# autonomousvision/unimatch

Measured on AMD Instinct MI355X. Metric: image_pairs_per_sec, higher is better.
Workload: dtype f16x2

## Files before the change

include/unimatch_hip.h:

```cpp
#ifndef UNIMATCH_HIP_H
#define UNIMATCH_HIP_H

#include <stddef.h>
#include <stdint.h>

#ifdef __cplusplus
extern "C" {
#endif

#define UM_VERSION 220

#define UM_MODE_EXACT 0
#define UM_MODE_FAST 1

#define UM_ERR_BAD_ARG (-1)
#define UM_ERR_BAD_GEOMETRY (-2)
#define UM_ERR_WORKSPACE (-3)
#define UM_ERR_UNSUPPORTED (-4)
#define UM_ERR_COLLECTIVE (-5)

int um_version(void);
const char* um_last_error_string(void);

#define UM_RANGE_PLANES 1u
#define UM_RANGE_ATTN_TOKENS 2u
#define UM_RANGE_ATTN_QUERY 4u
#define UM_RANGE_ATTN_OUTPUT 8u
#define UM_RANGE_FFN_TOKENS 16u
#define UM_RANGE_FFN_HIDDEN 32u
#define UM_RANGE_KV_TOKENS 64u
#define UM_RANGE_LINEAR 128u
int um_range_flags(unsigned* flags_out, int reset);

#define UM_K_WINDOW_ATTN 0
#define UM_K_GLOBAL_SOFTMAX 1
#define UM_K_SPLIT_PLANES 2
#define UM_K_LOCAL_CORR 3
#define UM_K_COST_VOLUME 4
#define UM_K_PROP_LOCAL 5
#define UM_K_DEPTH_CORR 6
#define UM_K_LINEAR 7
#define UM_K_INSTANCE_NORM 8
#define UM_K_CONVEX_UPSAMPLE 9
#define UM_K_FFN 10
#define UM_K_CONV 11
#define UM_K_COUNT 12
#define UM_V_WATTN_TILE 0
#define UM_V_WATTN_KSPLIT 1
#define UM_V_FFN_TILE 2
#define UM_V_FFN_HSPLIT 3
#define UM_V_GSV4 4
#define UM_V_GSV3 5
#define UM_V_K4_MFMA 6
#define UM_V_K4_VALU 7
#define UM_V_K3_MFMA 8
#define UM_V_K3_VALU 9
#define UM_V_CONV_PATCH 10
#define UM_V_CONV_ROWS 11
#define UM_V_CONV_GENERIC 12
#define UM_V_WATTN_W8 13
#define UM_V_CONV_PATCH_NORM 14
#define UM_V_COUNT 15
int um_census_enable(int on);
long um_census_count(int variant);
int um_window_attn_tile_census(int enable, unsigned long long* counts4);
double um_probe_mfma_flops(int iters);
int um_probe_mfma(float* sink, int iters, void* stream);
int um_probe_copy(const void* src, void* dst, size_t bytes, void* stream);
int um_probe_chase(const unsigned* ring, unsigned* out, int hops, void* stream);
int um_timing_enable(int kernel_mask);
int um_timing_collect(int kernel_id, double* total_ms, int* launches);

size_t um_window_attn_workspace_bytes(int streams, int tokens, int channels, int mode);
int um_window_attn_fwd(const float* q, const float* k, const float* v, float* out,
                       int streams, int h, int w, int channels,
                       int win_h, int win_w, int shift_h, int shift_w,
                       int mode, void* workspace, size_t workspace_bytes, void* stream);

int um_window_attn_planes_fwd(const void* q_planes, const void* k_planes, const void* v_planes, float* out,
                              int streams, int h, int w, int channels, int ldq, int ldkv,
                              long q_plane_stride, long kv_plane_stride,
                              int win_h, int win_w, int shift_h, int shift_w, int kv_rotate, int mode, void* stream);

int um_window_attn_merge_fwd(const void* q_planes, const void* k_planes, const void* v_planes, const void* wm_planes,
                             const float* gamma, const float* beta, const float* residual, float eps, int wshift, float* out,
                             int streams, int h, int w, int channels, int ldq, int ldkv, long q_plane_stride,
                             long kv_plane_stride, int win_h, int win_w, int shift_h, int shift_w, int kv_rotate, int mode,
                             void* stream);

size_t um_window_attn_ksplit_workspace_bytes(int streams, int h, int w, int win_h, int win_w);
int um_window_attn_plan(int streams, int h, int w, int win_h, int win_w, int* full_tiles, int* split_tiles, int* parts);
int um_window_attn_qproj_merge_fwd(const float* x, const void* wq_planes, const void* k_planes, const void* v_planes,
                                   const void* wm_planes, const float* gamma, const float* beta, const float* residual, float eps,
                                   int wshift, float* out, int streams, int h, int w, int channels, int ldkv,
                                   long kv_plane_stride, int win_h, int win_w, int shift_h, int shift_w, int kv_rotate, int mode,
                                   void* workspace, size_t workspace_bytes, void* stream);

#define UM_EPI_PLANES 0
#define UM_EPI_LN 1
#define UM_EPI_GELU_PLANES 2
size_t um_planes_bytes(long rows, int cols, int mode);
int um_weight_planes(const float* w, void* planes, int n, int k, int wshift, int mode, void* stream);
int um_linear_fwd(const float* a0, const float* a1, const void* a_planes, const void* w_planes,
                  int m, int n, int k, int wshift, int epilogue, void* out,
                  const float* gamma, const float* beta, const float* residual, float eps,
                  int mode, void* stream);

int um_linear_bias_fwd(const float* a0, const void* a_planes, const void* w_planes, const float* bias, int m, int n, int k,
                       int wshift, float out_mul, float bias_mul, void* out_planes, float* out_f32, int mode, void* stream);

int um_ffn_fwd(const float* x, const float* y, const void* w1_planes, const void* w2_planes, int m, int hidden,
               int wshift, const float* gamma, const float* beta, float eps, float* out, int mode, void* stream);
size_t um_ffn_split_workspace_bytes(int m, int hidden);
int um_ffn_ws_fwd(const float* x, const float* y, const void* w1_planes, const void* w2_planes, int m, int hidden,
                  int wshift, const float* gamma, const float* beta, float eps, float* out, int mode, void* workspace,
                  size_t workspace_bytes, void* stream);

int um_kv4_fwd(const float* x, const void* wc_planes, int m, int wshift, void* out_planes, int mode, void* stream);
int um_ffn_kv_fwd(const float* x, const float* y, const void* w1_planes, const void* w2_planes, int m, int hidden, int wshift,
                  const float* gamma, const float* beta, float eps, float* out, const void* wc_planes, void* kv_planes, int mode,
                  void* workspace, size_t workspace_bytes, void* stream);

int um_conv2d_fwd(const void* a_planes, const void* w_planes, const float* bias, float* out, float* stats_out, int batch,
                  int hi, int wi, int cin, int cout, int kh, int kw, int stride, int pad_h, int pad_w, int relu, int wshift,
                  int mode, void* stream);
int um_conv2d_ex(const void* a_planes, int a_ld, int a_coff, long a_rows, const void* w_planes, const float* bias, float* out,
                 int out_ld, int out_coff, void* out_planes, int outp_ld, int outp_coff, long outp_rows, float* stats_out,
                 int batch, int hi, int wi, int cin, int cout, int kh, int kw, int stride, int pad_h, int pad_w, int act,
                 int wshift, int mode, void* stream);
int um_conv2d_gru_fwd(int gate, const void* a_planes, int a_ld, int a_coff, long a_rows, const void* w_planes, const float* bias,
                      float* hidden, const float* z, int z_ld, float* z_out, int z_out_ld, void* out_planes, int outp_ld,
                      int outp_coff, long outp_rows, int batch, int hi, int wi, int cin, int channels, int kh, int kw, int pad_h,
                      int pad_w, int wshift, int mode, void* stream);
int um_conv2d_gru_add_fwd(int gate, const void* a_planes, int a_ld, int a_coff, long a_rows, const void* w_planes, const float* bias,
                          const float* addend, int addend_ld, float* hidden, const float* z, int z_ld, float* z_out, int z_out_ld,
                          void* out_planes, int outp_ld, int outp_coff, long outp_rows, int batch, int hi, int wi, int cin,
                          int channels, int kh, int kw, int pad_h, int pad_w, int wshift, int mode, void* stream);
int um_conv_stats_parts(int hi, int wi, int cout, int kh, int kw, int stride, int pad_h, int pad_w);
size_t um_conv_stats_bytes(int batch, int parts, int channels);

size_t um_stem_planes_bytes(int batch, int h, int w);
size_t um_conv7_planes_bytes(int batch, int h, int w, int stride);
int um_conv7_fwd(const float* image, int channels, int normalize, const float* mean3, const float* std3, void* image_planes,
                 const void* w_planes, const float* bias, float* out, int out_ld, int out_coff, void* out_planes, int outp_ld,
                 int outp_coff, long outp_rows, float* stats_out, int batch, int h, int w, int cout, int stride, int act,
                 int wshift, void* stream);
int um_stem_conv_fwd(const float* image, int normalize, const float* mean3, const float* std3, void* image_planes,
                     const void* w_planes, float* out, float* stats_out, int batch, int h, int w, int cout, int wshift,
                     void* stream);

size_t um_nhwc_norm_workspace_bytes(int batch, int pixels, int channels);
int um_nhwc_instance_norm(const float* x, const float* shortcut, const void* shortcut_planes, void* planes_out, float* f32_out,
                          int batch, int pixels, int channels, float eps, int normalize, int relu, const float* conv_stats,
                          int conv_stats_parts, void* workspace, size_t workspace_bytes, int mode, void* stream);

int um_nhwc_stats_finalize(const float* conv_stats, int conv_stats_parts, float* stats_out, int batch, int pixels, int channels,
                           float eps, void* stream);
int um_conv2d_norm_supported(int hi, int wi, int cin, int cout, int kh, int kw, int stride, int pad_h, int pad_w, int mode);
int um_conv2d_norm_fwd(const float* x, const float* norm_stats, int norm_relu, const void* w_planes, const float* bias, float* out,
                       float* stats_out, int batch, int hi, int wi, int cin, int cout, int kh, int kw, int stride, int pad_h,
                       int pad_w, int relu, int wshift, int mode, void* stream);

int um_nhwc_gate(int mode, const float* src, int src_ld, const float* zr, float* hbuf, void* planes_out, int ld, int coff,
                 long plane_rows, long rows, int channels, void* stream);

int um_nchw_to_nhwc(const float* x, void* planes_out, float* f32_out, int batch, int channels, int pixels, int mode,
                    void* stream);

size_t um_global_corr_workspace_bytes(int batch, int tokens, int channels, int mode);
int um_global_corr_softmax_flow(const float* f0, const float* f1, float* flow,
                                int batch, int h, int w, int channels, int bidir,
                                int mode, void* workspace, size_t workspace_bytes, void* stream);

int um_global_corr_softmax_stereo(const float* f0, const float* f1, float* disp,
                                  int batch, int h, int w, int channels,
                                  int mode, void* workspace, size_t workspace_bytes, void* stream);

int um_prop_global_attn(const float* q, const float* k, const float* value, float* out,
                        int batch, int h, int w, int channels, int value_channels,
                        int mode, void* workspace, size_t workspace_bytes, void* stream);
float um_global_corr_plane_scale(int channels);
int um_prop_global_attn_planes(const void* q_planes, const void* k_planes, const float* value, float* out, int batch, int h,
                               int w, int channels, int value_channels, int mode, void* workspace, size_t workspace_bytes,
                               void* stream);


int um_local_corr_softmax(const float* f0, const float* f1, float* out,
                          int batch, int h, int w, int channels, int radius, int one_d, void* stream);

int um_local_corr_with_flow(const float* f0, const float* f1, const float* flow, float* cost,
                            int batch, int h, int w, int channels, int radius, void* stream);
int um_local_corr_with_flow_dilated(const float* f0, const float* f1, const float* flow, float* cost,
                                    int batch, int h, int w, int channels, int radius, int dilation, void* stream);
int um_local_corr_with_flow_planes(const float* f0, const float* f1, const float* flow, void* planes_out, int ld, long plane_rows,
                                   int batch, int h, int w, int channels, int radius, void* stream);

size_t um_local_corr_feat_planes_bytes(int batch, int h, int w, int channels);
int um_local_corr_feat_planes(const float* f0, const float* f1, void* feat_planes, int batch, int h, int w, int channels,
                              void* stream);
int um_local_corr_with_flow_feat_supported(int h, int w, int channels, int radius);
int um_local_corr_softmax_mfma(const float* f0, const float* f1, float* out, int batch, int h, int w, int channels, int radius,
                               void* workspace, size_t workspace_bytes, void* stream);
int um_local_corr_with_flow_feat(const float* f0, const float* f1, const void* feat_planes, const float* flow, float* cost,
                                 void* planes_out, int ld, long plane_rows, int batch, int h, int w, int channels, int radius,
                                 int flags, unsigned* stats ,
                                 void* stream);

int um_prop_local_attn(const float* q, const float* k, const float* value, float* out,
                       int batch, int h, int w, int channels, int value_channels, int radius,
                       void* stream);

int um_depth_corr_softmax(const float* f0, const float* f1, const float* cam, const float* candidates,
                          float* out, int batch, int h, int w, int channels, int num_candidates,
                          int from_argmax, void* stream);

int um_convex_upsample(const float* flow, const float* mask, float* up, int batch, int channels, int h, int w,
                       int factor, int is_depth, int mask_nhwc, void* stream);

int um_flow_warp(const float* feature_tokens, const float* flow, float* out_tokens, int batch, int h, int w, int channels,
                 void* stream);

int um_fwd_bwd_occlusion(const float* fwd, const float* bwd, float* occ_fwd, float* occ_bwd, int batch, int h, int w, float alpha,
                         float beta, void* stream);
size_t um_flow_to_rgb_workspace_bytes(int batch, int h, int w);
int um_flow_to_rgb(const float* flow, unsigned char* rgb, int batch, int h, int w, void* workspace, size_t ws_bytes, void* stream);

#define UM_FLOW_METRICS_K 16
#define UM_DISP_METRICS_K 8
#define UM_DEPTH_METRICS_K 8
size_t um_flow_metrics_workspace_bytes(int batch, int h, int w);
int um_flow_metrics(const float* pred, const float* gt, const float* valid, const float* noc_valid, double* rows, int batch, int hp,
                    int wp, int h, int w, int top, int left, void* workspace, size_t ws_bytes, void* stream);
size_t um_disp_metrics_workspace_bytes(int batch, int h, int w);
int um_disp_metrics(const float* pred, const float* gt, double* rows, int batch, int hp, int wp, int h, int w, int top, int left,
                    float max_disp, void* workspace, size_t ws_bytes, void* stream);
size_t um_depth_metrics_workspace_bytes(int batch, int h, int w);
int um_depth_metrics(const float* pred, const float* gt, const float* valid, double* rows, int batch, int hp, int wp, int h, int w,
                     int top, int left, float lo, float hi, void* workspace, size_t ws_bytes, void* stream);

#define UM_PREPOST_MAX_DIM 262140
#define UM_IMG_F32_NCHW 0
#define UM_IMG_U8_NHWC 1
#define UM_SIZE_PAD 0
#define UM_SIZE_RESIZE 1
#define UM_PRED_FLOW 0
#define UM_PRED_DISPARITY 1
#define UM_PRED_DEPTH 2
int um_image_prepare(const void* src, int src_layout, float* dst, int batch, int h, int w, int transpose, const float* mean,
                     const float* std, int mode, int hp, int wp, int top, int left, void* stream);
int um_pred_restore(const float* pred, float* out, int batch, int channels, int hp, int wp, int mode, int top, int left, int h, int w,
                    int kind, int transpose, void* stream);

int um_flow_upsample2x(const float* flow, float* out, int batch, int channels, int h, int w, float mult, void* stream);
int um_depth_cam_pack(const float* intrinsics, const float* pose, float* cam, int batch, float stride_div, int bidir, void* stream);
int um_rigid_flow(const float* inv_depth, const float* cam, float* flow, int batch, int h, int w, void* stream);

int um_instance_norm_fwd(const float* x, const float* shortcut, float* y, long planes, int hw, float eps,
                         int relu, void* stream);

#define UM_COMM_ID_BYTES 128
int um_comm_unique_id(void* id_out );
int um_comm_init_rank(void** comm_out, const void* id , int rank, int world);
int um_comm_init_file(void** comm_out, const char* path, int rank, int world, int timeout_seconds);
int um_comm_init_file_nonce(void** comm_out, const char* path, int rank, int world, int timeout_seconds, int nonce);
int um_comm_world(void* comm);
int um_comm_destroy(void* comm);
int um_allgather_preds(void* comm, const float* send, float* recv, size_t count_per_rank, void* stream);

int um_swin_attn_fwd(const float* q, const float* k, const float* v, float* out, int streams, int h, int w, int channels,
                     int win_h, int win_w, int shift_h, int shift_w, int mode, void* workspace, size_t workspace_bytes,
                     void* stream);
int um_attn1d_fwd(const float* q, const float* k, const float* v, float* out, int streams, int h, int w, int channels,
                  int win_w, int shift_w, int mode, void* workspace, size_t workspace_bytes, void* stream);
int um_local_corr_softmax_1d(const float* f0, const float* f1, float* out, int batch, int h, int w, int channels, int radius,
                             void* stream);
size_t um_workspace_bytes_swin_attn_fwd(int streams, int h, int w, int channels, int mode);
size_t um_workspace_bytes_attn1d_fwd(int streams, int h, int w, int channels, int mode);
size_t um_workspace_bytes_global_corr_softmax_flow(int batch, int h, int w, int channels, int mode);
size_t um_workspace_bytes_global_corr_softmax_stereo(int batch, int h, int w, int channels, int mode);
size_t um_workspace_bytes_prop_global_attn(int batch, int h, int w, int channels, int mode);
size_t um_workspace_bytes_local_corr_softmax(int batch, int h, int w, int channels, int mode);
size_t um_workspace_bytes_local_corr_softmax_1d(int batch, int h, int w, int channels, int mode);
size_t um_workspace_bytes_local_corr_with_flow(int batch, int h, int w, int channels, int mode);
size_t um_workspace_bytes_prop_local_attn(int batch, int h, int w, int channels, int mode);
size_t um_workspace_bytes_depth_corr_softmax(int batch, int h, int w, int channels, int mode);
size_t um_workspace_bytes_allgather_preds(int batch, int h, int w, int channels, int mode);

#ifdef UM_DIAGNOSTIC_BUILD
int um_debug_mfma_peak(float* sink, int iters, int random_operands, void* stream);
int um_debug_mfma_ticks(unsigned long long* ticks, float* sink, int iters, int random_operands, int waves, int chain, void* stream);
int um_debug_mfma_lds(unsigned long long* ticks, float* sink, int tiles, int mode, void* stream);
#endif

#ifdef __cplusplus
}
#endif
#endif
```

unimatch_amd/_abi.py:

```python
import ctypes
import os

_HERE = os.path.dirname(os.path.abspath(__file__))
LIB_PATH = os.environ.get('UM_LIB') or os.path.join(_HERE, 'libunimatch_hip.so')

MODE_EXACT = 0
MODE_FAST = 1

CENSUS = {'wattn_tile': 0, 'wattn_ksplit': 1, 'ffn_tile': 2, 'ffn_hsplit': 3, 'gsv4': 4, 'gsv3': 5, 'k4_mfma': 6, 'k4_valu': 7,
          'k3_mfma': 8, 'k3_valu': 9, 'conv_patch': 10, 'conv_rows': 11, 'conv_generic': 12, 'wattn_w8': 13, 'conv_patch_norm': 14}

_c_int, _c_size_t, _c_void_p = ctypes.c_int, ctypes.c_size_t, ctypes.c_void_p

SIGNATURES = {
    'um_version': (_c_int, []),
    'um_last_error_string': (ctypes.c_char_p, []),
    'um_range_flags': (_c_int, [ctypes.POINTER(ctypes.c_uint), _c_int]),
    'um_timing_enable': (_c_int, [_c_int]),
    'um_timing_collect': (_c_int, [_c_int, ctypes.POINTER(ctypes.c_double), ctypes.POINTER(_c_int)]),
    'um_window_attn_workspace_bytes': (_c_size_t, [_c_int] * 4),
    'um_window_attn_fwd': (_c_int, [_c_void_p] * 4 + [_c_int] * 9 + [_c_void_p, _c_size_t, _c_void_p]),
    'um_window_attn_planes_fwd': (_c_int, [_c_void_p] * 4 + [_c_int] * 6 + [ctypes.c_long] * 2 + [_c_int] * 6 + [_c_void_p]),
    'um_window_attn_merge_fwd': (_c_int, [_c_void_p] * 7 + [ctypes.c_float, _c_int, _c_void_p] + [_c_int] * 6 + [ctypes.c_long] * 2 +
                                 [_c_int] * 6 + [_c_void_p]),
    'um_window_attn_qproj_merge_fwd': (_c_int, [_c_void_p] * 8 + [ctypes.c_float, _c_int, _c_void_p] + [_c_int] * 5 + [ctypes.c_long] +
                                       [_c_int] * 6 + [_c_void_p, _c_size_t, _c_void_p]),
    'um_window_attn_ksplit_workspace_bytes': (_c_size_t, [_c_int] * 5),
    'um_window_attn_plan': (_c_int, [_c_int] * 5 + [ctypes.POINTER(_c_int)] * 3),
    'um_planes_bytes': (_c_size_t, [ctypes.c_long, _c_int, _c_int]),
    'um_weight_planes': (_c_int, [_c_void_p] * 2 + [_c_int] * 4 + [_c_void_p]),
    'um_linear_fwd': (_c_int, [_c_void_p] * 4 + [_c_int] * 5 + [_c_void_p] * 4 + [ctypes.c_float, _c_int, _c_void_p]),
    'um_linear_bias_fwd': (_c_int, [_c_void_p] * 4 + [_c_int] * 4 + [ctypes.c_float] * 2 + [_c_void_p] * 2 + [_c_int, _c_void_p]),
    'um_ffn_fwd': (_c_int, [_c_void_p] * 4 + [_c_int] * 3 + [_c_void_p] * 2 + [ctypes.c_float, _c_void_p, _c_int, _c_void_p]),
    'um_ffn_ws_fwd': (_c_int, [_c_void_p] * 4 + [_c_int] * 3 + [_c_void_p] * 2 + [ctypes.c_float, _c_void_p, _c_int, _c_void_p, _c_size_t,
                                _c_void_p]),
    'um_ffn_split_workspace_bytes': (_c_size_t, [_c_int] * 2),
    'um_ffn_kv_fwd': (_c_int, [_c_void_p] * 4 + [_c_int] * 3 + [_c_void_p] * 2 + [ctypes.c_float, _c_void_p, _c_void_p, _c_void_p, _c_int, _c_void_p,
                                _c_size_t, _c_void_p]),
    'um_kv4_fwd': (_c_int, [_c_void_p, _c_void_p, _c_int, _c_int, _c_void_p, _c_int, _c_void_p]),
    'um_conv2d_fwd': (_c_int, [_c_void_p] * 5 + [_c_int] * 13 + [_c_void_p]),
    'um_conv2d_ex': (_c_int, [_c_void_p, _c_int, _c_int, ctypes.c_long, _c_void_p, _c_void_p, _c_void_p, _c_int, _c_int, _c_void_p,
                              _c_int, _c_int, ctypes.c_long, _c_void_p] + [_c_int] * 13 + [_c_void_p]),
    'um_nhwc_gate': (_c_int, [_c_int, _c_void_p, _c_int, _c_void_p, _c_void_p, _c_void_p, _c_int, _c_int, ctypes.c_long, ctypes.c_long,
                              _c_int, _c_void_p]),
    'um_local_corr_with_flow_planes': (_c_int, [_c_void_p] * 4 + [_c_int, ctypes.c_long] + [_c_int] * 5 + [_c_void_p]),
    'um_conv2d_gru_fwd': (_c_int, [_c_int, _c_void_p, _c_int, _c_int, ctypes.c_long, _c_void_p, _c_void_p, _c_void_p, _c_void_p, _c_int,
                                   _c_void_p, _c_int, _c_void_p, _c_int, _c_int, ctypes.c_long] + [_c_int] * 11 + [_c_void_p]),
    'um_conv2d_gru_add_fwd': (_c_int, [_c_int, _c_void_p, _c_int, _c_int, ctypes.c_long, _c_void_p, _c_void_p, _c_void_p, _c_int, _c_void_p, _c_void_p,
                                        _c_int, _c_void_p, _c_int, _c_void_p, _c_int, _c_int, ctypes.c_long] + [_c_int] * 11 + [_c_void_p]),
    'um_conv2d_norm_supported': (_c_int, [_c_int] * 10),
    'um_conv2d_norm_fwd': (_c_int, [_c_void_p, _c_void_p, _c_int] + [_c_void_p] * 4 + [_c_int] * 13 + [_c_void_p]),
    'um_nhwc_stats_finalize': (_c_int, [_c_void_p, _c_int, _c_void_p] + [_c_int] * 3 + [ctypes.c_float, _c_void_p]),
    'um_conv_stats_bytes': (_c_size_t, [_c_int] * 3),
    'um_conv_stats_parts': (_c_int, [_c_int] * 8),
    'um_stem_planes_bytes': (_c_size_t, [_c_int] * 3),
    'um_conv7_planes_bytes': (_c_size_t, [_c_int] * 4),
    'um_conv7_fwd': (_c_int, [_c_void_p, _c_int, _c_int] + [_c_void_p] * 6 + [_c_int, _c_int, _c_void_p, _c_int, _c_int, ctypes.c_long,
                              _c_void_p] + [_c_int] * 7 + [_c_void_p]),
    'um_stem_conv_fwd': (_c_int, [_c_void_p, _c_int] + [_c_void_p] * 6 + [_c_int] * 5 + [_c_void_p]),
    'um_nhwc_norm_workspace_bytes': (_c_size_t, [_c_int] * 3),
    'um_nhwc_instance_norm': (_c_int, [_c_void_p] * 5 + [_c_int] * 3 + [ctypes.c_float, _c_int, _c_int, _c_void_p, _c_int, _c_void_p,
                                       _c_size_t, _c_int, _c_void_p]),
    'um_nchw_to_nhwc': (_c_int, [_c_void_p] * 3 + [_c_int] * 4 + [_c_void_p]),
    'um_flow_warp': (_c_int, [_c_void_p] * 3 + [_c_int] * 4 + [_c_void_p]),
    'um_fwd_bwd_occlusion': (_c_int, [_c_void_p] * 4 + [_c_int] * 3 + [ctypes.c_float] * 2 + [_c_void_p]),
    'um_flow_to_rgb_workspace_bytes': (_c_size_t, [_c_int] * 3),
    'um_flow_to_rgb': (_c_int, [_c_void_p] * 2 + [_c_int] * 3 + [_c_void_p, _c_size_t, _c_void_p]),
    'um_flow_metrics_workspace_bytes': (_c_size_t, [_c_int] * 3),
    'um_flow_metrics': (_c_int, [_c_void_p] * 5 + [_c_int] * 7 + [_c_void_p, _c_size_t, _c_void_p]),
    'um_disp_metrics_workspace_bytes': (_c_size_t, [_c_int] * 3),
    'um_disp_metrics': (_c_int, [_c_void_p] * 3 + [_c_int] * 7 + [ctypes.c_float, _c_void_p, _c_size_t, _c_void_p]),
    'um_depth_metrics_workspace_bytes': (_c_size_t, [_c_int] * 3),
    'um_depth_metrics': (_c_int, [_c_void_p] * 4 + [_c_int] * 7 + [ctypes.c_float] * 2 + [_c_void_p, _c_size_t, _c_void_p]),
    'um_image_prepare': (_c_int, [_c_void_p, _c_int, _c_void_p] + [_c_int] * 4 + [ctypes.POINTER(ctypes.c_float)] * 2 + [_c_int] * 5 +
                         [_c_void_p]),
    'um_pred_restore': (_c_int, [_c_void_p] * 2 + [_c_int] * 11 + [_c_void_p]),
    'um_convex_upsample': (_c_int, [_c_void_p] * 3 + [_c_int] * 7 + [_c_void_p]),
    'um_flow_upsample2x': (_c_int, [_c_void_p] * 2 + [_c_int] * 4 + [ctypes.c_float, _c_void_p]),
    'um_depth_cam_pack': (_c_int, [_c_void_p] * 3 + [_c_int, ctypes.c_float, _c_int, _c_void_p]),
    'um_rigid_flow': (_c_int, [_c_void_p] * 3 + [_c_int] * 3 + [_c_void_p]),
    'um_instance_norm_fwd': (_c_int, [_c_void_p] * 3 + [ctypes.c_long, _c_int, ctypes.c_float, _c_int, _c_void_p]),
    'um_global_corr_workspace_bytes': (_c_size_t, [_c_int] * 4),
    'um_global_corr_softmax_flow': (_c_int, [_c_void_p] * 3 + [_c_int] * 6 + [_c_void_p, _c_size_t, _c_void_p]),
    'um_global_corr_softmax_stereo': (_c_int, [_c_void_p] * 3 + [_c_int] * 5 + [_c_void_p, _c_size_t, _c_void_p]),
    'um_prop_global_attn': (_c_int, [_c_void_p] * 4 + [_c_int] * 6 + [_c_void_p, _c_size_t, _c_void_p]),
    'um_global_corr_plane_scale': (ctypes.c_float, [_c_int]),
    'um_prop_global_attn_planes': (_c_int, [_c_void_p] * 4 + [_c_int] * 6 + [_c_void_p, _c_size_t, _c_void_p]),
    'um_local_corr_softmax': (_c_int, [_c_void_p] * 3 + [_c_int] * 6 + [_c_void_p]),
    'um_local_corr_with_flow': (_c_int, [_c_void_p] * 4 + [_c_int] * 5 + [_c_void_p]),
    'um_local_corr_with_flow_dilated': (_c_int, [_c_void_p] * 4 + [_c_int] * 6 + [_c_void_p]),
    'um_local_corr_feat_planes_bytes': (ctypes.c_size_t, [_c_int] * 4),
    'um_local_corr_feat_planes': (_c_int, [_c_void_p] * 3 + [_c_int] * 4 + [_c_void_p]),
    'um_local_corr_with_flow_feat_supported': (_c_int, [_c_int] * 4),
    'um_local_corr_softmax_mfma': (_c_int, [_c_void_p] * 3 + [_c_int] * 5 + [_c_void_p, ctypes.c_size_t, _c_void_p]),
    'um_local_corr_with_flow_feat': (_c_int, [_c_void_p] * 6 + [_c_int, ctypes.c_long] + [_c_int] * 6 + [_c_void_p, _c_void_p]),
    'um_prop_local_attn': (_c_int, [_c_void_p] * 4 + [_c_int] * 6 + [_c_void_p]),
    'um_depth_corr_softmax': (_c_int, [_c_void_p] * 5 + [_c_int] * 6 + [_c_void_p]),
    'um_census_enable': (_c_int, [_c_int]),
    'um_census_count': (ctypes.c_long, [_c_int]),
    'um_window_attn_tile_census': (_c_int, [_c_int, ctypes.POINTER(ctypes.c_ulonglong)]),
    'um_probe_mfma_flops': (ctypes.c_double, [_c_int]),
    'um_probe_mfma': (_c_int, [_c_void_p, _c_int, _c_void_p]),
    'um_probe_copy': (_c_int, [_c_void_p, _c_void_p, _c_size_t, _c_void_p]),
    'um_probe_chase': (_c_int, [_c_void_p, _c_void_p, _c_int, _c_void_p]),
    'um_swin_attn_fwd': (_c_int, [_c_void_p] * 4 + [_c_int] * 9 + [_c_void_p, _c_size_t, _c_void_p]),
    'um_attn1d_fwd': (_c_int, [_c_void_p] * 4 + [_c_int] * 7 + [_c_void_p, _c_size_t, _c_void_p]),
    'um_local_corr_softmax_1d': (_c_int, [_c_void_p] * 3 + [_c_int] * 5 + [_c_void_p]),
    **{f'um_workspace_bytes_{op}': (_c_size_t, [_c_int] * 5) for op in (
        'swin_attn_fwd', 'attn1d_fwd', 'global_corr_softmax_flow', 'global_corr_softmax_stereo', 'prop_global_attn',
        'local_corr_softmax', 'local_corr_softmax_1d', 'local_corr_with_flow', 'prop_local_attn', 'depth_corr_softmax',
        'allgather_preds')},
    'um_comm_unique_id': (_c_int, [_c_void_p]),
    'um_comm_init_rank': (_c_int, [ctypes.POINTER(_c_void_p), _c_void_p, _c_int, _c_int]),
    'um_comm_init_file': (_c_int, [ctypes.POINTER(_c_void_p), ctypes.c_char_p, _c_int, _c_int, _c_int]),
    'um_comm_init_file_nonce': (_c_int, [ctypes.POINTER(_c_void_p), ctypes.c_char_p, _c_int, _c_int, _c_int, _c_int]),
    'um_comm_world': (_c_int, [_c_void_p]),
    'um_comm_destroy': (_c_int, [_c_void_p]),
    'um_allgather_preds': (_c_int, [_c_void_p, _c_void_p, _c_void_p, _c_size_t, _c_void_p]),
}
COMM_ID_BYTES = 128
DIAG_SIGNATURES = {
    'um_debug_mfma_peak': (_c_int, [_c_void_p, _c_int, _c_int, _c_void_p]),
    'um_debug_mfma_lds': (_c_int, [_c_void_p, _c_void_p, _c_int, _c_int, _c_void_p]),
    'um_debug_mfma_ticks': (_c_int, [_c_void_p, _c_void_p, _c_int, _c_int, _c_int, _c_int, _c_void_p]),
}

RANGE_ROLES = {1: 'a tensor converted to operand planes (q / k / v / features)', 2: 'attention source tokens', 4: 'projected queries',
               8: 'attention output (input of the merge Linear)', 16: 'FFN input [x | y]', 32: 'FFN hidden activations',
               64: 'tokens / projected keys and values of the k | v projection', 128: 'inputs / plane outputs of a Linear'}

_lib = None


class HipExtensionError(RuntimeError):
    pass


def load():
    global _lib
    if _lib is not None:
        return _lib
    if not os.path.exists(LIB_PATH):
        raise HipExtensionError(
            f'{LIB_PATH} is missing: build it with `python -m unimatch_amd.build` '
            '(hipcc --offload-arch=gfx950).  There is no CPU / PyTorch fallback for the hot path.')
    try:
        lib = ctypes.CDLL(LIB_PATH)
    except OSError as exc:
        raise HipExtensionError(f'cannot load {LIB_PATH}: {exc}') from exc
    for name, (res, args) in SIGNATURES.items():
        try:
            fn = getattr(lib, name)
        except AttributeError as exc:
            raise HipExtensionError(f'{LIB_PATH} does not export {name}') from exc
        fn.restype = res
        fn.argtypes = args
    for name, (res, args) in DIAG_SIGNATURES.items():
        fn = getattr(lib, name, None)
        if fn is not None:
            fn.restype = res
            fn.argtypes = args
    _lib = lib
    return lib


def load_diagnostic():
    lib = load()
    if not hasattr(lib, 'um_debug_mfma_peak'):
        raise HipExtensionError('the shipped library carries no um_debug_* symbol: build a diagnostic variant '
                                '(`python -m unimatch_amd.build --variant diag`) and set UM_LIB=unimatch_amd/_variants/libdiag.so')
    return lib


def census(lib=None):
    lib = lib or load()
    return {k: int(lib.um_census_count(v)) for k, v in CENSUS.items()}


def attn_tile_census(enable):
    out = (ctypes.c_ulonglong * 4)()
    check(load().um_window_attn_tile_census(1 if enable else 0, out), 'um_window_attn_tile_census')
    return dict(zip(('full', 'probed', 'probed_then_computed', 'workgroups'), (int(v) for v in out)))


def check(code, what):
    if code == 0:
        return
    msg = load().um_last_error_string().decode('utf-8', 'replace')
    if code < 0:
        raise ValueError(f'{what}: {msg} (code {code})')
    raise RuntimeError(f'{what}: HIP error {code}')


class OperandRangeError(FloatingPointError):
    """An activation reached fp16's largest finite value (65504) on its way into an exact-mode MFMA operand."""


def range_flags(reset=False):
    out = ctypes.c_uint(0)
    check(load().um_range_flags(ctypes.byref(out), 1 if reset else 0), 'um_range_flags')
    return out.value


def check_operand_range(where=''):
# ... 8 lines not shown
```

unimatch_amd/build.py:

```python
import os
import shutil
import subprocess
import sys

HERE = os.path.dirname(os.path.abspath(__file__))
CSRC = os.path.join(HERE, 'csrc')
LIB = os.path.join(HERE, 'libunimatch_hip.so')
SOURCES = ['capi.hip', 'global_match.hip', 'window_attn.hip', 'local_ops.hip', 'linear.hip', 'ffn.hip', 'conv.hip', 'nhwc_ops.hip', 'norm_ops.hip', 'upsample.hip',
           'rccl_gather.hip', 'local_corr_mfma.hip', 'aliases.hip', 'probe.hip', 'video.hip', 'metrics.hip', 'prepost.hip']
DIAG_SOURCES = ['microbench.hip']
HEADERS = ['common.h', 'planes.h', 'timing.h', os.path.join('..', '..', 'include', 'unimatch_hip.h')]
EXTRA_FLAGS = {'ffn.hip': ['-fno-slp-vectorize'], 'global_match.hip': ['-fno-slp-vectorize', '-mllvm', '-amdgpu-mfma-vgpr-form', '-Wno-inline-asm'], 'window_attn.hip': ['-fno-slp-vectorize'],
               'linear.hip': ['-fno-slp-vectorize'],
               'video.hip': ['-ffp-contract=off'],
               'metrics.hip': ['-ffp-contract=off', '-fhip-fp32-correctly-rounded-divide-sqrt'],
               'prepost.hip': ['-ffp-contract=off', '-fhip-fp32-correctly-rounded-divide-sqrt']}
FLAGS = ['--offload-arch=gfx950', '-O3', '-std=c++17', '-fPIC', '-fno-gpu-rdc', '-Wno-unused-result']


def find_hipcc():
    for cand in (os.environ.get('HIPCC'), shutil.which('hipcc'), '/opt/rocm/bin/hipcc'):
        if cand and os.path.exists(cand):
            return cand
    raise RuntimeError('hipcc not found: the HIP extension cannot be built')


def _stale(target, deps):
    if not os.path.exists(target):
        return True
    t = os.path.getmtime(target)
    return any(os.path.getmtime(d) > t for d in deps)


def build(force=False, verbose=False):
    hipcc = find_hipcc()
    objdir = os.path.join(HERE, '_obj')
    os.makedirs(objdir, exist_ok=True)
    hdrs = [os.path.normpath(os.path.join(CSRC, h)) for h in HEADERS] + [os.path.abspath(__file__)]
    objs = []
    for src in SOURCES:
        s = os.path.join(CSRC, src)
        o = os.path.join(objdir, src.replace('.hip', '.o'))
        if force or _stale(o, [s] + hdrs):
            cmd = [hipcc] + FLAGS + EXTRA_FLAGS.get(src, []) + ['-c', s, '-o', o]
            if verbose:
                print(' '.join(cmd))
            subprocess.run(cmd, check=True, cwd=CSRC)
        objs.append(o)
    if force or _stale(LIB, objs):
        cmd = [hipcc, '--offload-arch=gfx950', '-shared', '-fPIC', '-o', LIB] + objs + ['-ldl']
        if verbose:
            print(' '.join(cmd))
        subprocess.run(cmd, check=True)
    return LIB


def build_variant(name, defines, verbose=False, only=None):
    hipcc = find_hipcc()
    objdir = os.path.join(HERE, '_variants', '_obj_' + name)
    os.makedirs(objdir, exist_ok=True)
    objs = []
    defines = list(defines) + ['-DUM_DIAGNOSTIC_BUILD']
    if only:
        build(verbose=verbose)
    for src in SOURCES + DIAG_SOURCES:
        if only and src not in only and src not in DIAG_SOURCES:
            objs.append(os.path.join(HERE, '_obj', src.replace('.hip', '.o')))
            continue
        o = os.path.join(objdir, src.replace('.hip', '.o'))
        cmd = [hipcc] + FLAGS + EXTRA_FLAGS.get(src, []) + list(defines) + ['-c', os.path.join(CSRC, src), '-o', o]
        if verbose:
            print(' '.join(cmd))
        subprocess.run(cmd, check=True, cwd=CSRC)
        objs.append(o)
    lib = os.path.join(HERE, '_variants', f'lib{name}.so')
    subprocess.run([hipcc, '--offload-arch=gfx950', '-shared', '-fPIC', '-o', lib] + objs + ['-ldl'], check=True)
    shutil.rmtree(objdir, ignore_errors=True)
    return lib


if __name__ == '__main__':
    if '--variant' in sys.argv:
        i = sys.argv.index('--variant')
        only = sys.argv[sys.argv.index('--only') + 1].split(',') if '--only' in sys.argv else None
        print(build_variant(sys.argv[i + 1], [a for a in sys.argv[i + 2:] if a.startswith('-D')], verbose=True, only=only))
    else:
        print(build(force='--force' in sys.argv, verbose=True))
```

unimatch_amd/csrc/conv.hip:

```cpp
#include <cstdlib>
#include <cstring>
#ifndef UM_CONV_2P
#define UM_CONV_2P 0
#endif
#include "common.h"
#include "planes.h"

struct ConvArgs {
    const unsigned short* ap;
    long a_plane_stride;
    unsigned row_stride;
    unsigned zero_row;
    const unsigned short* wp;
    long w_plane_stride;
    const float* bias;
    float* out;
    unsigned short* outp;
    long outp_plane_stride;
    int out_ld, out_coff, outp_ld, outp_coff;
    int act;
    int gate, gate_c, gate_zld;
    float* gate_h;
    const float* gate_z;
    float* gate_hout;
// ... 89 lines not shown
    };
    auto to_lds_b = [&](auto act_tag) {
        if (a.bias) to_lds(act_tag, IntC<1>{});
        else to_lds(act_tag, IntC<0>{});
    };
    switch (a.addend ? 0 : a.act) {
        case 0: to_lds_b(IntC<0>{}); break;
        case 1: to_lds_b(IntC<1>{}); break;
        case 2: to_lds_b(IntC<2>{}); break;
        default: to_lds_b(IntC<3>{}); break;
    }
    __builtin_amdgcn_wave_barrier();
    if (a.stats) {
        constexpr int RG = 64 / CPR >= 8 ? 8 : 64 / CPR >= 4 ? 4 : 2;
        constexpr int RPG = 32 / RG;
        const int nv = nvalid;
        const int c = lane % CPR, rg = lane / CPR;
        const f32x4 k = *reinterpret_cast<const f32x4*>(stg + (c << 4));
        f32x4 s1 = {0.f, 0.f, 0.f, 0.f}, s2 = {0.f, 0.f, 0.f, 0.f};
        if (rg < RG) {
            if (nv == 32) {
#pragma unroll
                for (int j = 0; j < RPG; ++j) {
                    const int r = rg * RPG + j;
                    const f32x4 d = *reinterpret_cast<const f32x4*>(stg + r * ROWB + ((c ^ (r & 7)) << 4)) - k;
                    s1 = s1 + d;
                    s2 = s2 + d * d;
                }
            } else {
#pragma unroll
                for (int j = 0; j < RPG; ++j) {
                    const int r = rg * RPG + j;
                    f32x4 d = *reinterpret_cast<const f32x4*>(stg + r * ROWB + ((c ^ (r & 7)) << 4)) - k;
                    if (r >= nv) d = f32x4{0.f, 0.f, 0.f, 0.f};
                    s1 = s1 + d;
                    s2 = s2 + d * d;
                }
            }
        }
#pragma unroll
        for (int step = CPR * RG / 2; step >= CPR; step >>= 1)
#pragma unroll
            for (int i = 0; i < 4; ++i) {
                s1[i] += __shfl_down(s1[i], step, 64);
                s2[i] += __shfl_down(s2[i], step, 64);
            }
        float* ws = reinterpret_cast<float*>(scratch) + wave * (2 * 32 * NT) + 32 * NT0;
        float* cnt = reinterpret_cast<float*>(scratch) + 8 * (2 * 32 * NT);
        if (lane == 0) cnt[wave] = (float)nv;
        if (lane < CPR) {
            const float inv = nv > 0 ? 1.0f / (float)nv : 0.f;
            *reinterpret_cast<f32x4*>(ws + 4 * c) = k + s1 * inv;
            *reinterpret_cast<f32x4*>(ws + 32 * NT + 4 * c) = s2 - s1 * s1 * inv;
        }
        __syncthreads();
        const int grp = tid >> 8, gt = tid & 255;
        if (gt < 32 * NTP && nb + gt < a.Cout && (cnt[4 * grp] > 0.f || dense_parts)) {
            const float* w0 = reinterpret_cast<const float*>(scratch) + grp * 4 * (2 * 32 * NT) + 32 * NT0;
            float mean = w0[gt], m2 = w0[32 * NT + gt];
            float n = cnt[4 * grp];
#pragma unroll
            for (int wv = 1; wv < 4; ++wv) {
                const float nw = cnt[4 * grp + wv];
                if (nw > 0.f) {
                    const float mw = w0[wv * (2 * 32 * NT) + gt], m2w = w0[wv * (2 * 32 * NT) + 32 * NT + gt];
                    const float delta = mw - mean, nn = n + nw;
                    mean += delta * (nw / nn);
                    m2 += m2w + delta * delta * (n * nw / nn);
                    n = nn;
                }
            }
            float* pr = a.stats + ((long)(part0 + grp) * 3) * a.Cout + nb + gt;
            pr[0] = n > 0.f ? mean : 0.f;
            pr[a.Cout] = n;
            pr[2 * a.Cout] = n > 0.f ? m2 : 0.f;
        }
    }
    auto store_rows = [&](auto gate_tag, auto add_tag) {
        constexpr int GATE = decltype(gate_tag)::value;
        constexpr bool ADD = decltype(add_tag)::value != 0;
        float* obase = a.out ? a.out + rowbase * a.out_ld + a.out_coff : nullptr;
        unsigned short* pbase = a.outp ? a.outp + rowbase * a.outp_ld + a.outp_coff : nullptr;
#pragma unroll
        for (int b = 0; b < NBATCH; ++b) {
            const int slot = NSIDE == 2 ? (b & 1) : 0;
            if ((ADD || GATE != 0) && NSIDE == 2 && b + 1 < NBATCH) preload(b + 1, (b + 1) & 1);
            if ((ADD || GATE != 0) && NSIDE == 1 && b > 0) preload(b, 0);
#pragma unroll
            for (int j = 0; j < BATCH; ++j) {
                const int idx = (b * BATCH + j) * 64 + lane;
                const int r = idx / CPR, c = idx - r * CPR;
                f32x4 d = *reinterpret_cast<const f32x4*>(stg + r * ROWB + ((c ^ (r & 7)) << 4));
                int col = nb + 4 * c;
                if (r < nrows && col < a.Cout) {
                    if (ADD) {
                        d = d + ad[slot][j];
#pragma unroll
                        for (int i = 0; i < 4; ++i) {
                            if (a.act == 1) d[i] = fmaxf(d[i], 0.f);
                            else if (a.act == 2) d[i] = 1.0f / (1.0f + __expf(-d[i]));
                            else if (a.act == 3) d[i] = tanhf(d[i]);
                        }
                    }
                    bool to_out = obase != nullptr, to_planes = pbase != nullptr;
                    if (GATE == 1) {
                        if (col >= a.gate_c) {
                            col -= a.gate_c;
                            d = d * gh[slot][j];
                            to_out = false;
                        } else {
                            to_planes = false;
                        }
                    } else if (GATE == 2) {
#pragma unroll
                        for (int i = 0; i < 4; ++i) d[i] = (1.0f - gz[slot][j][i]) * gh[slot][j][i] + gz[slot][j][i] * d[i];
                        *reinterpret_cast<f32x4*>(hobase + (unsigned)(r * a.gate_hout_ld + col)) = d;
                    }
                    if (to_out) __builtin_nontemporal_store(d, reinterpret_cast<f32x4*>(obase + (unsigned)(r * a.out_ld + col)));
                    if (to_planes) {
                        unsigned short* dst = pbase + (unsigned)(r * a.outp_ld + col);
                        const unsigned h0 = T::pack2(d[0], d[1]), h1 = T::pack2(d[2], d[3]);
                        *reinterpret_cast<u32x2*>(dst) = u32x2{h0, h1};
                        if (NS == 2) {
                            const f32x2 u0 = T::unpack2(h0), u1 = T::unpack2(h1);
                            const u32x2 lo = u32x2{T::pack2(d[0] - u0[0], d[1] - u0[1]), T::pack2(d[2] - u1[0], d[3] - u1[1])};
                            *reinterpret_cast<u32x2*>(dst + a.outp_plane_stride) = lo;
                        }
                    }
                }
            }
        }
    };
    auto store_rows_g = [&](auto gate_tag) {
        if (a.addend) store_rows(gate_tag, IntC<1>{});
        else store_rows(gate_tag, IntC<0>{});
    };
    if (a.gate == 0) store_rows_g(IntC<0>{});
    else if (a.gate == 1) store_rows_g(IntC<1>{});
    else store_rows_g(IntC<2>{});
}

template <typename T, int NS, int NT, int NTE = NT>
__device__ __forceinline__ void conv_epilogue(const ConvArgs& a, f32x16 (&acc)[NT], unsigned char* lds, unsigned char* scratch,
                                              int bt, int rloc0, int nvalid, int part0, bool dense_parts, int n0, int tid, int wave,
                                              int lane, int half) {
    constexpr int NP = NTE < NT ? NTE : NT;
    constexpr int WSTRIDE = 32 * (32 * NP * 4);
    conv_epilogue_pass<T, NS, NT, 0, NP, WSTRIDE>(a, acc, lds, scratch, bt, rloc0, nvalid, part0, dense_parts, n0, tid, wave, lane, half);
    if constexpr (NTE < NT)
        conv_epilogue_pass<T, NS, NT, NTE, NT - NTE, WSTRIDE>(a, acc, lds, scratch, bt, rloc0, nvalid, part0, dense_parts, n0, tid, wave,
                                                              lane, half);
}

template <typename T, int NS, int NT>
__global__ __launch_bounds__(256, 2) void conv_kernel(ConvArgs a) {
    constexpr int TILE = 128 * 64;
    constexpr int WTILE = 32 * NT * 64;
    constexpr int STAGE = NS * (TILE + WTILE);
    constexpr int EPI = 4 * 32 * (32 * NT * 4);
    constexpr int RING = (2 * STAGE > EPI) ? 2 * STAGE : EPI;
    __shared__ __attribute__((aligned(16))) unsigned char lds[RING + 8 * 2 * 32 * NT * 4 + 64];

    const int tid = threadIdx.x, lane = tid & 63;
    const int wave = __builtin_amdgcn_readfirstlane(tid >> 6);
    const int half = lane >> 5;
    const int P = a.Ho * a.Wo, tpi = (P + 127) / 128;
    const int ny = (a.Cout + 32 * NT - 1) / (32 * NT);
    const int wg = a.xcd ? xcd_remap(blockIdx.x, gridDim.x) : blockIdx.x;
    const int tile = wg / ny;
    const int bt = tile / tpi, pl0 = (tile - bt * tpi) * 128;
    const int n0 = (wg - tile * ny) * (32 * NT);
    const int cpt = a.Cin >> 5;
    const int nstage = a.KH * a.KW * cpt;
    const int ktot = a.KH * a.KW * a.Cin;

    const int dcp = lane & 3;
    int py[2], px[2], pbase[2];
    bool pok[2];
#pragma unroll
    for (int i = 0; i < 2; ++i) {
        const int p = pl0 + 32 * wave + 16 * i + (lane >> 2);
        pok[i] = p < P;
        const int rem = pok[i] ? p : 0;
        const int y = rem / a.Wo, x = rem - y * a.Wo;
        py[i] = y * a.stride - a.pad_h;
        px[i] = x * a.stride - a.pad_w;
        pbase[i] = bt * a.Hi * a.Wi;
    }
    const unsigned zero_row = a.zero_row;
    unsigned rowoff[2];
    auto set_tap = [&](int ky, int kx) {
#pragma unroll
        for (int i = 0; i < 2; ++i) {
            const int iy = py[i] + ky, ix = px[i] + kx;
            const bool ok = pok[i] && (unsigned)iy < (unsigned)a.Hi && (unsigned)ix < (unsigned)a.Wi;
            const unsigned row = ok ? (unsigned)(pbase[i] + iy * a.Wi + ix) : zero_row;
            rowoff[i] = row * a.row_stride;
        }
    };
    int ky = 0, kx = 0, cc = 0;
    auto stage_async = [&](int c0, int kglob, unsigned char* buf) {
#pragma unroll
        for (int i = 0; i < 2; ++i) {
            const int r = 32 * wave + 16 * i + (lane >> 2);
            const int sc = dcp ^ ((r >> 2) & 3);
            const unsigned off = rowoff[i] + (unsigned)((c0 + 8 * sc) * 2);
#pragma unroll
            for (int pl = 0; pl < NS; ++pl) conv_dma16(a.ap + pl * a.a_plane_stride, off, buf + pl * TILE + (32 * wave + 16 * i) * 64);
        }
#pragma unroll
        for (int i = 0; i < (2 * NT + 3) / 4; ++i) {
            const int j = wave + 4 * i;
            if (j < 2 * NT) {
                const int r = 16 * j + (lane >> 2);
                const int sc = dcp ^ ((r >> 2) & 3);
                const int n = min(n0 + r, a.Cout - 1);
                const unsigned off = (unsigned)(((long)n * ktot + kglob + 8 * sc) * 2);
#pragma unroll
                for (int pl = 0; pl < NS; ++pl)
                    conv_dma16(a.wp + pl * a.w_plane_stride, off, buf + NS * TILE + pl * WTILE + (16 * j) * 64);
            }
        }
    };

    f32x16 acc[NT];
#pragma unroll
    for (int nt = 0; nt < NT; ++nt)
#pragma unroll
        for (int r = 0; r < 16; ++r) acc[nt][r] = 0.f;

    const int fr = lane & 31;
    int foff[2];
#pragma unroll
    for (int ks = 0; ks < 2; ++ks) foff[ks] = fr * 64 + (((2 * ks + half) ^ ((fr >> 2) & 3)) << 4);

    set_tap(0, 0);
    stage_async(0, 0, lds);
    auto advance = [&]() {
        if (++cc == cpt) {
            cc = 0;
            if (++kx == a.KW) {
                kx = 0;
                ++ky;
            }
            set_tap(ky, kx);
        }
    };
    advance();
    asm volatile("s_waitcnt vmcnt(0)" ::: "memory");
    __syncthreads();

    for (int s = 0; s < nstage; ++s) {
        unsigned char* cur = lds + (s & 1) * STAGE;
        unsigned char* nxt = lds + ((s & 1) ^ 1) * STAGE;
        if (s + 1 < nstage) {
            stage_async(cc * 32, (s + 1) * 32, nxt);
            advance();
        }
        const unsigned char* at = cur + 32 * wave * 64;
        const unsigned char* wt = cur + NS * TILE;
        __builtin_amdgcn_s_setprio(1);
#pragma unroll
        for (int ks = 0; ks < 2; ++ks) {
            const i16x8 bh = *reinterpret_cast<const i16x8*>(at + foff[ks]);
            i16x8 bl;
            if (NS == 2) bl = *reinterpret_cast<const i16x8*>(at + TILE + foff[ks]);
#pragma unroll
            for (int nt = 0; nt < NT; ++nt) {
                const i16x8 wh = *reinterpret_cast<const i16x8*>(wt + nt * 32 * 64 + foff[ks]);
                if (NS == 2) {
                    const i16x8 wl = *reinterpret_cast<const i16x8*>(wt + WTILE + nt * 32 * 64 + foff[ks]);
                    if (UM_CONV_2P != 1) acc[nt] = T::mfma(wl, bh, acc[nt]);
                    if (UM_CONV_2P != 2) acc[nt] = T::mfma(wh, bl, acc[nt]);
                }
                acc[nt] = T::mfma(wh, bh, acc[nt]);
            }
        }
        __builtin_amdgcn_s_setprio(0);
        asm volatile("s_waitcnt vmcnt(0)" ::: "memory");
        __syncthreads();
    }

    {
        const int rloc0 = pl0 + 32 * wave;
        conv_epilogue<T, NS, NT>(a, acc, lds, lds + RING, bt, rloc0, min(32, max(0, P - rloc0)), bt * ((P + 127) / 128) + pl0 / 128, false,
                                 n0, tid, wave, lane, half);
    }
}

template <int NS, int NT, int KW, int NSLOT>
struct ConvRowsLds {
    static constexpr int NTE = NT < 2 ? NT : 2;
    static constexpr int ATILE = 288 * 32;
    static constexpr int WTILE = 32 * NT * 32;
    static constexpr int STAGE = NS * (ATILE + KW * WTILE);
    static constexpr int EPI = 8 * 32 * (32 * NTE * 4);
    static constexpr int RING = (NSLOT * STAGE > EPI) ? NSLOT * STAGE : EPI;
    static constexpr int TOTAL = RING + 8 * 2 * 32 * NT * 4 + 64;
};

__device__ __forceinline__ void conv_wait_vm(int n) {
    switch (n) {
        case 0: asm volatile("s_waitcnt vmcnt(0)" ::: "memory"); break;
        case 1: asm volatile("s_waitcnt vmcnt(1)" ::: "memory"); break;
        case 2: asm volatile("s_waitcnt vmcnt(2)" ::: "memory"); break;
        case 3: asm volatile("s_waitcnt vmcnt(3)" ::: "memory"); break;
        case 4: asm volatile("s_waitcnt vmcnt(4)" ::: "memory"); break;
        case 6: asm volatile("s_waitcnt vmcnt(6)" ::: "memory"); break;
        case 8: asm volatile("s_waitcnt vmcnt(8)" ::: "memory"); break;
        case 9: asm volatile("s_waitcnt vmcnt(9)" ::: "memory"); break;
        case 12: asm volatile("s_waitcnt vmcnt(12)" ::: "memory"); break;
        case 16: asm volatile("s_waitcnt vmcnt(16)" ::: "memory"); break;
        case 18: asm volatile("s_waitcnt vmcnt(18)" ::: "memory"); break;
        case 24: asm volatile("s_waitcnt vmcnt(24)" ::: "memory"); break;
        default: asm volatile("s_waitcnt vmcnt(0)" ::: "memory"); break;
    }
}

template <typename T, int NS, int NT, int KW, int NSLOT>
__global__ __launch_bounds__(512, (NSLOT == 2 && NT < 4 ? 2 : 1)) void conv_rows_kernel(ConvArgs a) {
    using L = ConvRowsLds<NS, NT, KW, NSLOT>;
    constexpr int ATILE = L::ATILE, WTILE = L::WTILE, STAGE = L::STAGE, RING = L::RING;
    extern __shared__ __attribute__((aligned(16))) unsigned char lds[];

    const int tid = threadIdx.x, lane = tid & 63;
    const int wave = __builtin_amdgcn_readfirstlane(tid >> 6);
    const int half = lane >> 5, fr = lane & 31;
    const int P = a.Ho * a.Wo, tpi = (P + 255) / 256;
    const int ny = (a.Cout + 32 * NT - 1) / (32 * NT);
    const int wg = a.xcd ? xcd_remap(blockIdx.x, gridDim.x) : blockIdx.x;
    const int tile = wg / ny;
    const int bt = tile / tpi, pl0 = (tile - bt * tpi) * 256;
    const int n0 = (wg - tile * ny) * (32 * NT);
    const int cpt = a.Cin >> 4;
    const int nstage = a.KH * cpt;
    const int ktot = a.KH * KW * a.Cin;

    const int dcp = lane & 1;
    int wy[2];
    long wflat[2];
    bool wok[2];
#pragma unroll
    for (int i = 0; i < 2; ++i) {
        const int jr = i == 0 ? wave : 8;
        const int j = 32 * jr + (lane >> 1);
        const int p = pl0 + j - a.pad_w;
        wok[i] = (i == 0 || wave == 7) && p >= 0 && p < P;
        const int rem = wok[i] ? p : 0;
        wy[i] = rem / a.Wo - a.pad_h;
        wflat[i] = (long)bt * P + rem - (long)a.pad_h * a.Wi;
    }
    unsigned rowoff[2];
    auto set_ky = [&](int ky) {
#pragma unroll
        for (int i = 0; i < 2; ++i) {
            const int iy = wy[i] + ky;
            const bool ok = wok[i] && (unsigned)iy < (unsigned)a.Hi;
            const unsigned row = ok ? (unsigned)(wflat[i] + (long)ky * a.Wi) : a.zero_row;
            rowoff[i] = row * a.row_stride;
        }
    };
    constexpr int NPIECE = 2 + (KW * NT + 7) / 8;
    auto stage_piece = [&](int k, int ky, int cc, unsigned char* buf) {
        if (k < 2) {
            const int jr = k == 0 ? wave : 8;
            if (k == 0 || wave == 7) {
                const int r = 32 * jr + (lane >> 1);
                const int sc = dcp ^ ((r >> 3) & 1);
                const unsigned off = rowoff[k] + (unsigned)((cc * 16 + 8 * sc) * 2);
#pragma unroll
                for (int pl = 0; pl < NS; ++pl) conv_dma16(a.ap + pl * a.a_plane_stride, off, buf + pl * ATILE + (32 * jr) * 32);
            }
        } else {
            const int q = wave + 8 * (k - 2);
            if (q < KW * NT) {
                const int kx = q / NT, jb = q - kx * NT;
                const int r = 32 * jb + (lane >> 1);
                const int sc = dcp ^ ((r >> 3) & 1);
                const int n = min(n0 + r, a.Cout - 1);
                const unsigned off = (unsigned)(((long)n * ktot + (ky * KW + kx) * a.Cin + cc * 16 + 8 * sc) * 2);
#pragma unroll
                for (int pl = 0; pl < NS; ++pl)
                    conv_dma16(a.wp + pl * a.w_plane_stride, off, buf + NS * ATILE + (kx * NS + pl) * WTILE + (32 * jb) * 32);
            }
        }
    };

    bool tap_ok[KW];
    bool any_masked = false;
    {
        const int p = pl0 + 32 * wave + fr;
        const bool pok = p < P;
        const int x = (pok ? p : 0) % a.Wo;
#pragma unroll
        for (int kx = 0; kx < KW; ++kx) {
            tap_ok[kx] = pok && (unsigned)(x + kx - a.pad_w) < (unsigned)a.Wi;
            any_masked |= !tap_ok[kx];
        }
    }
    const bool wave_masked = __any(any_masked);

    f32x16 acc[NT];
#pragma unroll
    for (int nt = 0; nt < NT; ++nt)
#pragma unroll
        for (int r = 0; r < 16; ++r) acc[nt][r] = 0.f;

    const int foffw = fr * 32 + ((half ^ ((fr >> 3) & 1)) << 4);
    int foffa[KW];
#pragma unroll
    for (int kx = 0; kx < KW; ++kx) {
        const int r = 32 * wave + fr + kx;
        foffa[kx] = r * 32 + ((half ^ ((r >> 3) & 1)) << 4);
    }

    int cnt = NS * (1 + (wave == 7 ? 1 : 0));
#pragma unroll
    for (int k = 2; k < NPIECE; ++k) cnt += (wave + 8 * (k - 2) < KW * NT) ? NS : 0;
    constexpr int D = NSLOT - 1;

    int ky = 0, cc = 0;
    set_ky(0);
    auto advance = [&]() {
        if (++cc == cpt) {
            cc = 0;
            ++ky;
            set_ky(ky);
        }
    };
#pragma unroll
    for (int d = 0; d < D; ++d)
        if (d < nstage) {
#pragma unroll
            for (int k = 0; k < NPIECE; ++k) stage_piece(k, ky, cc, lds + d * STAGE);
            advance();
        }
    conv_wait_vm(nstage >= D ? cnt * (D - 1) : 0);
    __syncthreads();

    int cur_off = 0, nxt_off = D * STAGE;
// ... 123 lines not shown
        float v[8];
#pragma unroll
        for (int k = 0; k < 8; ++k) {
            const float m = nsc ? mu[8 + k] : mu[k], r = nsc ? rs[8 + k] : rs[k];
            v[k] = ((k < 4 ? nx0[k & 3] : nx1[k & 3]) - m) * r;
        }
        if (a.norm_relu) {
#pragma unroll
            for (int k = 0; k < 8; ++k) v[k] = fmaxf(v[k], 0.f);
        }
        const bool ok = rowoff[i] != ~0u;
        u32x4 h = {T::pack2(v[0], v[1]), T::pack2(v[2], v[3]), T::pack2(v[4], v[5]), T::pack2(v[6], v[7])};
        unsigned char* dst = buf + (32 * (wave + 8 * i)) * 32 + lane * 16;
        if (NS == 2) {
            u32x4 l;
#pragma unroll
            for (int k = 0; k < 4; ++k) {
                const f32x2 u = T::unpack2(h[k]);
                l[k] = ok ? T::pack2(v[2 * k] - u[0], v[2 * k + 1] - u[1]) : 0u;
            }
            *reinterpret_cast<u32x4*>(dst + ATILE) = l;
        }
#pragma unroll
        for (int k = 0; k < 4; ++k) h[k] = ok ? h[k] : 0u;
        *reinterpret_cast<u32x4*>(dst) = h;
    };
    auto stage_w = [&](int cc, int ky, unsigned char* buf) {
#pragma unroll
        for (int k = 0; k < (3 * NT + 7) / 8; ++k) {
            const int q = wave + 8 * k;
            if (q < 3 * NT) {
                const int kx = q / NT, jb = q - kx * NT;
                const int r = 32 * jb + (lane >> 1);
                const int sc = dcp ^ ((r >> 3) & 1);
                const int n = min(n0 + r, a.Cout - 1);
                const unsigned off = (unsigned)(((long)n * ktot + (ky * 3 + kx) * a.Cin + cc * 16 + 8 * sc) * 2);
#pragma unroll
                for (int pl = 0; pl < NS; ++pl)
                    conv_dma16(a.wp + pl * a.w_plane_stride, off, buf + (kx * NS + pl) * WTILE + (32 * jb) * 32);
            }
        }
    };

    f32x16 acc[NT];
#pragma unroll
    for (int nt = 0; nt < NT; ++nt)
#pragma unroll
        for (int r = 0; r < 16; ++r) acc[nt][r] = 0.f;

    const int foffw = fr * 32 + ((half ^ ((fr >> 3) & 1)) << 4);
    int foffa[3][3];
#pragma unroll
    for (int ky = 0; ky < 3; ++ky)
#pragma unroll
        for (int kx = 0; kx < 3; ++kx) {
            const int r = (wave + ky) * PW + kx + fr;
            foffa[ky][kx] = r * 32 + ((half ^ ((r >> 3) & 1)) << 4);
        }

    if constexpr (NORM) {
        stage_w(0, 0, lds + WBASE);
        norm_load(0, 0);
        norm_store(0, 0, lds);
        if (wave < 3) {
            norm_load(0, 1);
            norm_store(0, 1, lds);
        }
    } else {
        stage_patch(0, lds);
        stage_w(0, 0, lds + WBASE);
    }
    asm volatile("s_waitcnt vmcnt(0)" ::: "memory");
    __syncthreads();

    for (int cc = 0; cc < cpt; ++cc) {
        const int a_cur = (cc & 1) * ASLOT, a_nxt = ASLOT - a_cur;
#pragma unroll
        for (int ky = 0; ky < 3; ++ky) {
            const int w_par = (cc + ky) & 1;
            const int w_cur = WBASE + w_par * WSLOT, w_nxt = WBASE + (w_par ^ 1) * WSLOT;
            const bool last = ky == 2 && cc + 1 == cpt;
            __builtin_amdgcn_s_setprio(1);
#pragma unroll
            for (int kx = 0; kx < 3; ++kx) {
                if (kx == 0 && !last) stage_w(ky == 2 ? cc + 1 : cc, ky == 2 ? 0 : ky + 1, lds + w_nxt);
                if constexpr (NORM) {
                    if (kx == 1 && cc + 1 < cpt) {
                        if (ky == 0) norm_load(cc + 1, 0);
                        if (ky == 1) {
                            norm_store(cc + 1, 0, lds + a_nxt);
                            if (wave < 3) norm_load(cc + 1, 1);
                        }
                        if (ky == 2 && wave < 3) norm_store(cc + 1, 1, lds + a_nxt);
                    }
                } else {
                    if (kx == 1 && ky == 0 && cc + 1 < cpt) stage_patch(cc + 1, lds + a_nxt);
                }
                const i16x8 bh = *reinterpret_cast<const i16x8*>(lds + a_cur + foffa[ky][kx]);
                i16x8 bl;
                if (NS == 2) bl = *reinterpret_cast<const i16x8*>(lds + a_cur + ATILE + foffa[ky][kx]);
                const unsigned char* wt = lds + w_cur + kx * NS * WTILE;
#pragma unroll
                for (int nt = 0; nt < NT; ++nt) {
                    const i16x8 wh = *reinterpret_cast<const i16x8*>(wt + nt * 32 * 32 + foffw);
                    if (NS == 2) {
                        const i16x8 wl = *reinterpret_cast<const i16x8*>(wt + WTILE + nt * 32 * 32 + foffw);
                        if (UM_CONV_2P != 1) acc[nt] = T::mfma(wl, bh, acc[nt]);
                        if (UM_CONV_2P != 2) acc[nt] = T::mfma(wh, bl, acc[nt]);
                    }
                    acc[nt] = T::mfma(wh, bh, acc[nt]);
                }
            }
            __builtin_amdgcn_s_setprio(0);
            asm volatile("s_waitcnt vmcnt(0)" ::: "memory");
            __syncthreads();
        }
    }
    const int nvalid = y0 + wave < a.Ho ? min(32, a.Wo - x0) : 0;
    conv_epilogue<T, NS, NT, L::NTE>(a, acc, lds, lds + L::EPI, bt, (y0 + wave) * a.Wo + x0, nvalid, (bt * tpi + tt) * 2, true, n0, tid,
                                     wave, lane, half);
}

template <typename T, int NS, int NT>
__global__ __launch_bounds__(512, (NT < 4 ? 2 : 1)) void conv_patch_kernel(ConvArgs a) {
    extern __shared__ __attribute__((aligned(16))) unsigned char lds[];
    conv_patch_body<T, NS, NT, false>(a, lds);
}

template <typename T, int NS, int NT>
__global__ __launch_bounds__(512, (NT < 4 ? 2 : 1)) void conv_patch_norm_kernel(ConvArgs a) {
    extern __shared__ __attribute__((aligned(16))) unsigned char lds[];
    conv_patch_body<T, NS, NT, true>(a, lds);
}

extern void um_set_error(const char* fmt, ...);

static int conv_xcd_enabled() {
    static const int on = um_debug_env("UM_CONV_NO_XCD") == nullptr;
    return on;
}

template <int NT>
static hipError_t launch_conv(const ConvArgs& a, int mode, hipStream_t stream) {
    dim3 grid(a.B * ((a.Ho * a.Wo + 127) / 128) * ((a.Cout + 32 * NT - 1) / (32 * NT))), block(256);
    ScopedKernelTimer timer(UM_K_CONV, stream);
    um_census_hit(UM_V_CONV_GENERIC);
    if (mode == 0)
        hipLaunchKernelGGL((conv_kernel<Fp16, 2, NT>), grid, block, 0, stream, a);
    else
        hipLaunchKernelGGL((conv_kernel<Bf16, 1, NT>), grid, block, 0, stream, a);
    return hipGetLastError();
}

template <int NT, int KW, int NSLOT>
static hipError_t launch_conv_rows(const ConvArgs& a, int mode, hipStream_t stream) {
    static bool configured[2] = {false, false};
    dim3 grid(a.B * ((a.Ho * a.Wo + 255) / 256) * ((a.Cout + 32 * NT - 1) / (32 * NT))), block(512);
    constexpr int LDS2 = ConvRowsLds<2, NT, KW, NSLOT>::TOTAL, LDS1 = ConvRowsLds<1, NT, KW, NSLOT>::TOTAL;
    static_assert(LDS2 <= 160 * 1024 && LDS1 <= 160 * 1024, "ring beyond the CU's LDS");
    ScopedKernelTimer timer(UM_K_CONV, stream);
    um_census_hit(UM_V_CONV_ROWS);
    if (mode == 0) {
        if (!configured[0]) {
            hipError_t e = hipFuncSetAttribute(reinterpret_cast<const void*>(&conv_rows_kernel<Fp16, 2, NT, KW, NSLOT>),
                                               hipFuncAttributeMaxDynamicSharedMemorySize, LDS2);
            if (e != hipSuccess) return e;
            configured[0] = true;
        }
        hipLaunchKernelGGL((conv_rows_kernel<Fp16, 2, NT, KW, NSLOT>), grid, block, LDS2, stream, a);
    } else {
        if (!configured[1]) {
            hipError_t e = hipFuncSetAttribute(reinterpret_cast<const void*>(&conv_rows_kernel<Bf16, 1, NT, KW, NSLOT>),
                                               hipFuncAttributeMaxDynamicSharedMemorySize, LDS1);
            if (e != hipSuccess) return e;
            configured[1] = true;
        }
        hipLaunchKernelGGL((conv_rows_kernel<Bf16, 1, NT, KW, NSLOT>), grid, block, LDS1, stream, a);
    }
    return hipGetLastError();
}

template <int NT, bool NORM = false>
static hipError_t launch_conv_patch(const ConvArgs& a, int mode, hipStream_t stream) {
    static bool configured[2] = {false, false};
    dim3 grid(a.B * ((a.Ho + 7) / 8) * ((a.Wo + 31) / 32) * ((a.Cout + 32 * NT - 1) / (32 * NT))), block(512);
    constexpr int LDS2 = ConvPatchLds<2, NT>::TOTAL, LDS1 = ConvPatchLds<1, NT>::TOTAL;
    static_assert(LDS2 <= 160 * 1024 && LDS1 <= 160 * 1024, "ring beyond the CU's LDS");
    ScopedKernelTimer timer(UM_K_CONV, stream);
    um_census_hit(UM_V_CONV_PATCH);
    if (NORM) um_census_hit(UM_V_CONV_PATCH_NORM);
    void (*k2)(ConvArgs), (*k1)(ConvArgs);
    if constexpr (NORM) {
        k2 = conv_patch_norm_kernel<Fp16, 2, NT>;
        k1 = conv_patch_norm_kernel<Bf16, 1, NT>;
    } else {
        k2 = conv_patch_kernel<Fp16, 2, NT>;
        k1 = conv_patch_kernel<Bf16, 1, NT>;
    }
    if (mode == 0) {
        if (!configured[0]) {
            hipError_t e = hipFuncSetAttribute(reinterpret_cast<const void*>(k2), hipFuncAttributeMaxDynamicSharedMemorySize, LDS2);
            if (e != hipSuccess) return e;
            configured[0] = true;
        }
        hipLaunchKernelGGL(k2, grid, block, LDS2, stream, a);
    } else {
        if (!configured[1]) {
            hipError_t e = hipFuncSetAttribute(reinterpret_cast<const void*>(k1), hipFuncAttributeMaxDynamicSharedMemorySize, LDS1);
            if (e != hipSuccess) return e;
            configured[1] = true;
        }
        hipLaunchKernelGGL(k1, grid, block, LDS1, stream, a);
    }
    return hipGetLastError();
}

enum ConvKind { CONV_GENERIC = 0, CONV_ROWS = 1, CONV_PATCH = 2 };

static ConvKind conv_pick(int hi, int wi, int ho, int wo, int cout, int kh, int kw, int stride, int pad_h, int pad_w, int* nt_out) {
    const int nt = (cout % 128 == 0 || cout > 192) ? 4 : (cout % 96 == 0) ? 3 : (cout <= 64 || cout % 64 == 0) ? 2 : 4;
    *nt_out = nt;
    static const bool rows_enabled = um_debug_env("UM_CONV_NO_ROWS") == nullptr;
    static const char* patch_env = um_debug_env("UM_CONV_PATCH");
    static const char* patch_nts = patch_env ? patch_env : "234";
    const bool same = stride == 1 && ho == hi && wo == wi && (long)ho * wo >= 256 && rows_enabled;
    const bool rows3 = same && kw == 3 && pad_w == 1, rows5 = same && kw == 5 && pad_w == 2 && nt == 4;
    const long tiled = (long)((ho + 7) / 8 * 8) * ((wo + 31) / 32 * 32);
    if (rows3 && kh == 3 && pad_h == 1 && 4L * ho * wo >= 3 * tiled && strchr(patch_nts, '0' + nt) != nullptr) {
        if (cout <= 32) *nt_out = 1;
        return CONV_PATCH;
    }
    return rows3 || rows5 ? CONV_ROWS : CONV_GENERIC;
}

static constexpr bool kNormOnLoad[5] = {false, false, true, true, true};

extern "C" int um_conv2d_norm_supported(int hi, int wi, int cin, int cout, int kh, int kw, int stride, int pad_h, int pad_w, int mode) {
    if (hi <= 0 || wi <= 0 || cin <= 0 || cin % 32 != 0 || cout <= 0 || cout % 4 != 0 || kh <= 0 || kw <= 0 || stride <= 0 || pad_h < 0 ||
        pad_w < 0 || (mode != 0 && mode != 1))
        return 0;
    const int ho = (hi + 2 * pad_h - kh) / stride + 1, wo = (wi + 2 * pad_w - kw) / stride + 1;
    if (ho <= 0 || wo <= 0) return 0;
    int nt;
    if (conv_pick(hi, wi, ho, wo, cout, kh, kw, stride, pad_h, pad_w, &nt) != CONV_PATCH) return 0;
    return nt >= 2 && nt <= 4 && kNormOnLoad[nt] ? 1 : 0;
}

extern "C" int um_conv_stats_parts(int hi, int wi, int cout, int kh, int kw, int stride, int pad_h, int pad_w) {
    if (hi <= 0 || wi <= 0 || cout <= 0 || kh <= 0 || kw <= 0 || stride <= 0 || pad_h < 0 || pad_w < 0) return -1;
    const int ho = (hi + 2 * pad_h - kh) / stride + 1, wo = (wi + 2 * pad_w - kw) / stride + 1;
    if (ho <= 0 || wo <= 0) return -1;
    int nt;
    if (conv_pick(hi, wi, ho, wo, cout, kh, kw, stride, pad_h, pad_w, &nt) == CONV_PATCH) return 2 * ((ho + 7) / 8) * ((wo + 31) / 32);
    return (int)(((long)ho * wo + 127) / 128);
}

static int conv2d_impl(const void* a_planes, int a_ld, int a_coff, long a_rows, const void* w_planes, const float* bias,
                       float* out, int out_ld, int out_coff, void* out_planes, int outp_ld, int outp_coff, long outp_rows,
                       float* stats_out, int batch, int hi, int wi, int cin, int cout, int kh, int kw, int stride,
                       int pad_h, int pad_w, int act, int wshift, int mode, void* stream_, int gate, float* gate_h,
                       const float* gate_z, int gate_zld, const float* addend = nullptr, int addend_ld = 0, float* gate_hout = nullptr,
                       int gate_hout_ld = 0, const float* norm_x = nullptr, const float* norm_stats = nullptr, int norm_relu = 0) {
    const bool norm = norm_x != nullptr;
    if (gate_hout && (gate != 2 || gate_hout_ld < cout || gate_hout_ld % 4 != 0 || ((unsigned long)gate_hout & 15) != 0)) {
        um_set_error("um_conv2d: a separate new-state tensor goes with gate 2 only: 16-byte aligned fp32 [M][ld >= channels, ld %% 4 == 0]");
        return -1;
    }
    if (addend && (addend_ld < cout || addend_ld % 4 != 0 || ((unsigned long)addend & 15) != 0 || stats_out)) {
        um_set_error("um_conv2d: the addend must be 16-byte aligned fp32 [M][ld >= cout, ld %% 4 == 0] (and excludes fused statistics)");
        return -1;
    }
    if ((!a_planes && !norm) || !w_planes || (!out && !out_planes) || batch <= 0 || hi <= 0 || wi <= 0 || cin <= 0 || cin % 32 != 0 ||
        cout <= 0 || cout % 4 != 0 || kh <= 0 || kw <= 0 || stride <= 0 || pad_h < 0 || pad_w < 0 || (mode != 0 && mode != 1) ||
        wshift < 0 || wshift > 14 || act < 0 || act > 3) {
        um_set_error("um_conv2d: bad argument (batch=%d hi=%d wi=%d cin=%d cout=%d k=%dx%d stride=%d pad=%d,%d act=%d; cin must "
                     "be a multiple of 32, cout of 4)", batch, hi, wi, cin, cout, kh, kw, stride, pad_h, pad_w, act);
        return -1;
    }
    const int ho = (hi + 2 * pad_h - kh) / stride + 1, wo = (wi + 2 * pad_w - kw) / stride + 1;
    if (ho <= 0 || wo <= 0) {
        um_set_error("um_conv2d: empty output (%d x %d)", ho, wo);
        return -1;
    }
    const long rows_in = (long)batch * hi * wi, m = (long)batch * ho * wo;
    if (a_ld < a_coff + cin || a_ld % 8 != 0 || a_coff % 8 != 0 || a_rows < rows_in + 1 ||
        (out && (out_ld < out_coff + cout || out_ld % 4 != 0 || out_coff % 4 != 0)) ||
        (out_planes && (outp_ld < outp_coff + (gate == 1 ? cout / 2 : cout) || outp_ld % 4 != 0 || outp_coff % 4 != 0 ||
                        outp_rows < m))) {
        um_set_error("um_conv2d: inconsistent leading dimensions / offsets / row counts");
        return -1;
    }
    if (stats_out && !out) {
        um_set_error("um_conv2d: fused statistics need the fp32 output");
        return -1;
    }
    if (bias && ((unsigned long)bias & 15) != 0) {
        um_set_error("um_conv2d: bias must be 16-byte aligned");
        return -1;
    }
    if (a_rows * a_ld * 2 >= (1L << 32) || (long)cout * kh * kw * cin * 2 >= (1L << 32) || m >= (1L << 31)) {
        um_set_error("um_conv2d: operand planes beyond 4 GiB are not addressable by this kernel");
        return -4;
    }
    if (norm) {
        if (!norm_stats || ((unsigned long)norm_x & 15) != 0 || ((unsigned long)norm_stats & 3) != 0) {
            um_set_error("um_conv2d_norm_fwd: the fp32 input must be 16-byte aligned and comes with its statistics [batch][2][cin]");
            return -1;
        }
        if (!um_conv2d_norm_supported(hi, wi, cin, cout, kh, kw, stride, pad_h, pad_w, mode)) {
            um_set_error("um_conv2d_norm_fwd: no on-load kernel for this geometry (hi=%d wi=%d cin=%d cout=%d k=%dx%d stride=%d pad=%d,%d): "
                         "ask um_conv2d_norm_supported() first", hi, wi, cin, cout, kh, kw, stride, pad_h, pad_w);
            return -2;
        }
        if (rows_in * cin * 4 >= (1L << 32) - 1) {
            um_set_error("um_conv2d_norm_fwd: an fp32 input beyond 4 GiB is not addressable by this kernel");
            return -4;
        }
    }
    ConvArgs a;
    a.xf = norm_x;
    a.nstats = norm_stats;
    a.norm_relu = norm_relu;
    a.ap = (const unsigned short*)a_planes + a_coff;
    a.a_plane_stride = a_rows * a_ld;
    a.row_stride = (unsigned)a_ld * 2;
    a.zero_row = (unsigned)(a_rows - 1);
    a.wp = (const unsigned short*)w_planes;
    a.w_plane_stride = (long)cout * kh * kw * cin;
    a.bias = bias;
    a.out = out;
    a.out_ld = out_ld;
    a.out_coff = out_coff;
    a.outp = (unsigned short*)out_planes;
    a.outp_ld = outp_ld;
    a.outp_coff = outp_coff;
    a.outp_plane_stride = outp_rows * outp_ld;
    a.stats = stats_out;
    a.addend = addend;
    a.addend_ld = addend_ld;
    a.B = batch;
    a.Hi = hi;
    a.Wi = wi;
    a.Cin = cin;
    a.Ho = ho;
    a.Wo = wo;
    a.Cout = cout;
    a.KH = kh;
    a.KW = kw;
    a.stride = stride;
    a.pad_h = pad_h;
    a.pad_w = pad_w;
    a.M = (int)m;
    a.act = act;
    a.gate = gate;
    a.gate_c = gate == 1 ? cout / 2 : cout;
    a.gate_h = gate_h;
    a.gate_z = gate_z;
    a.gate_zld = gate_zld;
    a.gate_hout = gate_hout ? gate_hout : gate_h;
    a.gate_hout_ld = gate_hout ? gate_hout_ld : a.gate_c;
    a.out_scale = ldexpf(1.f, -wshift);
    a.xcd = conv_xcd_enabled();
    hipError_t e;
    int nt;
    const ConvKind kind = conv_pick(hi, wi, ho, wo, cout, kh, kw, stride, pad_h, pad_w, &nt);
    hipStream_t st = (hipStream_t)stream_;
    if (norm)
        e = nt == 2 ? launch_conv_patch<2, true>(a, mode, st) : nt == 3 ? launch_conv_patch<3, true>(a, mode, st) : launch_conv_patch<4, true>(a, mode, st);
    else if (kind == CONV_PATCH)
        e = nt == 1 ? launch_conv_patch<1>(a, mode, st) : nt == 2 ? launch_conv_patch<2>(a, mode, st) : nt == 3 ? launch_conv_patch<3>(a, mode, st)
                                                                                                          : launch_conv_patch<4>(a, mode, st);
    else if (kind == CONV_ROWS && kw == 5) e = launch_conv_rows<4, 5, 2>(a, mode, st);
    else if (kind == CONV_ROWS) e = nt == 2 ? launch_conv_rows<2, 3, 2>(a, mode, st) : nt == 3 ? launch_conv_rows<3, 3, 2>(a, mode, st) : launch_conv_rows<4, 3, 2>(a, mode, st);
    else e = nt == 2 ? launch_conv<2>(a, mode, st) : nt == 3 ? launch_conv<3>(a, mode, st) : launch_conv<4>(a, mode, st);
    if (e != hipSuccess) {
        um_set_error("um_conv2d: launch failed: %s", hipGetErrorString(e));
        return (int)e;
    }
    return 0;
}

extern "C" int um_conv2d_ex(const void* a_planes, int a_ld, int a_coff, long a_rows, const void* w_planes, const float* bias,
                            float* out, int out_ld, int out_coff, void* out_planes, int outp_ld, int outp_coff, long outp_rows,
                            float* stats_out, int batch, int hi, int wi, int cin, int cout, int kh, int kw, int stride,
                            int pad_h, int pad_w, int act, int wshift, int mode, void* stream_) {
    return conv2d_impl(a_planes, a_ld, a_coff, a_rows, w_planes, bias, out, out_ld, out_coff, out_planes, outp_ld, outp_coff,
                       outp_rows, stats_out, batch, hi, wi, cin, cout, kh, kw, stride, pad_h, pad_w, act, wshift, mode, stream_, 0,
                       nullptr, nullptr, 0);
}

extern "C" int um_conv2d_gru_fwd(int gate, const void* a_planes, int a_ld, int a_coff, long a_rows, const void* w_planes,
                                 const float* bias, float* hidden, const float* z, int z_ld, float* z_out, int z_out_ld,
                                 void* out_planes, int outp_ld, int outp_coff, long outp_rows, int batch, int hi, int wi, int cin,
                                 int channels, int kh, int kw, int pad_h, int pad_w, int wshift, int mode, void* stream_) {
    if ((gate != 1 && gate != 2) || !hidden || !out_planes || channels <= 0 || channels % 4 != 0 || (gate == 1 && !z_out) ||
        (gate == 2 && !z)) {
        um_set_error("um_conv2d_gru_fwd: bad argument (gate=%d channels=%d)", gate, channels);
        return -1;
    }
    if (gate == 1)
        return conv2d_impl(a_planes, a_ld, a_coff, a_rows, w_planes, bias, z_out, z_out_ld, 0, out_planes, outp_ld, outp_coff,
                           outp_rows, nullptr, batch, hi, wi, cin, 2 * channels, kh, kw, 1, pad_h, pad_w, 2, wshift, mode, stream_,
                           1, hidden, nullptr, 0);
    return conv2d_impl(a_planes, a_ld, a_coff, a_rows, w_planes, bias, nullptr, 0, 0, out_planes, outp_ld, outp_coff, outp_rows,
                       nullptr, batch, hi, wi, cin, channels, kh, kw, 1, pad_h, pad_w, 3, wshift, mode, stream_, 2, hidden, z, z_ld);
}

extern "C" int um_conv2d_gru_add_fwd(int gate, const void* a_planes, int a_ld, int a_coff, long a_rows, const void* w_planes,
                                     const float* bias, const float* addend, int addend_ld, float* hidden, const float* z, int z_ld,
                                     float* z_out, int z_out_ld, void* out_planes, int outp_ld, int outp_coff, long outp_rows,
                                     int batch, int hi, int wi, int cin, int channels, int kh, int kw, int pad_h, int pad_w,
                                     int wshift, int mode, void* stream_) {
    if ((gate != 1 && gate != 2) || !hidden || !out_planes || !addend || channels <= 0 || channels % 4 != 0 || (gate == 1 && !z_out) ||
        (gate == 2 && !z)) {
        um_set_error("um_conv2d_gru_add_fwd: bad argument (gate=%d channels=%d)", gate, channels);
        return -1;
    }
    if (gate == 1)
        return conv2d_impl(a_planes, a_ld, a_coff, a_rows, w_planes, bias, z_out, z_out_ld, 0, out_planes, outp_ld, outp_coff,
                           outp_rows, nullptr, batch, hi, wi, cin, 2 * channels, kh, kw, 1, pad_h, pad_w, 2, wshift, mode, stream_,
                           1, hidden, nullptr, 0, addend, addend_ld);
    return conv2d_impl(a_planes, a_ld, a_coff, a_rows, w_planes, bias, nullptr, 0, 0, out_planes, outp_ld, outp_coff, outp_rows,
                       nullptr, batch, hi, wi, cin, channels, kh, kw, 1, pad_h, pad_w, 3, wshift, mode, stream_, 2, hidden, z, z_ld,
                       addend, addend_ld, z_out, z_out_ld);
}

extern "C" int um_conv2d_fwd(const void* a_planes, const void* w_planes, const float* bias, float* out, float* stats_out,
                             int batch, int hi, int wi, int cin, int cout, int kh, int kw, int stride, int pad_h, int pad_w,
                             int relu, int wshift, int mode, void* stream_) {
    const long rows_in = (long)batch * hi * wi;
    return um_conv2d_ex(a_planes, cin, 0, rows_in + 1, w_planes, bias, out, cout, 0, nullptr, 0, 0, 0, stats_out, batch, hi, wi,
                        cin, cout, kh, kw, stride, pad_h, pad_w, relu ? 1 : 0, wshift, mode, stream_);
}

extern "C" int um_conv2d_norm_fwd(const float* x, const float* norm_stats, int norm_relu, const void* w_planes, const float* bias, float* out,
                                  float* stats_out, int batch, int hi, int wi, int cin, int cout, int kh, int kw, int stride, int pad_h,
                                  int pad_w, int relu, int wshift, int mode, void* stream_) {
    if (!x) {
        um_set_error("um_conv2d_norm_fwd: no input");
        return -1;
    }
    const long rows_in = (long)batch * hi * wi;
    return conv2d_impl(nullptr, cin, 0, rows_in + 1, w_planes, bias, out, cout, 0, nullptr, 0, 0, 0, stats_out, batch, hi, wi, cin, cout, kh,
                       kw, stride, pad_h, pad_w, relu ? 1 : 0, wshift, mode, stream_, 0, nullptr, nullptr, 0, nullptr, 0, nullptr, 0, x,
                       norm_stats, norm_relu ? 1 : 0);
}

template <int CPP>
__global__ __launch_bounds__(256) void pack7_kernel(const float* img, unsigned short* planes, long plane_stride, int B, int C,
                                                    int H, int W, int Hp, int Wp, int normalize, float m0, float m1, float m2,
                                                    float s0, float s1, float s2) {
    const long idx = (long)blockIdx.x * 256 + threadIdx.x;
    const long total = (long)B * Hp * Wp;
    if (idx >= total) return;
    const int xp = (int)(idx % Wp);
    const long t = idx / Wp;
    const int yp = (int)(t % Hp), b = (int)(t / Hp);
    const int y = yp - 3, x = xp - 3;
    float v[CPP];
#pragma unroll
    for (int c = 0; c < CPP; ++c) v[c] = 0.f;
    if ((unsigned)y < (unsigned)H && (unsigned)x < (unsigned)W) {
        const float mean[3] = {m0, m1, m2}, sd[3] = {s0, s1, s2};
#pragma unroll
        for (int c = 0; c < CPP; ++c) {
            if (c < C) {
                float p = img[(((long)b * C + c) * H + y) * W + x];
                if (normalize && c < 3) p = (p / 255.0f - mean[c]) / sd[c];
                v[c] = p;
            }
        }
    }
#pragma unroll
    for (int c = 0; c < CPP; c += 4) {
        const unsigned h0 = Fp16::pack2(v[c], v[c + 1]), h1 = Fp16::pack2(v[c + 2], v[c + 3]);
        *reinterpret_cast<u32x2*>(planes + idx * CPP + c) = u32x2{h0, h1};
        const f32x2 u0 = Fp16::unpack2(h0), u1 = Fp16::unpack2(h1);
        *reinterpret_cast<u32x2*>(planes + plane_stride + idx * CPP + c) =
            u32x2{Fp16::pack2(v[c] - u0[0], v[c + 1] - u0[1]), Fp16::pack2(v[c + 2] - u1[0], v[c + 3] - u1[1])};
    }
}

static int conv7_wp(int w) { return (w + 8 + 1) & ~1; }

extern "C" size_t um_conv7_planes_bytes(int batch, int h, int w, int stride) {
    if (batch <= 0 || h <= 0 || w <= 0 || (stride != 1 && stride != 2)) return 0;
    const long cpp = stride == 2 ? 4 : 8;
    return (size_t)(2 * ((long)batch * (h + 6) * conv7_wp(w) + 8) * cpp * 2);
}

extern "C" int um_conv7_fwd(const float* image, int channels, int normalize, const float* mean3, const float* std3,
                            void* image_planes, const void* w_planes, const float* bias, float* out, int out_ld, int out_coff,
                            void* out_planes, int outp_ld, int outp_coff, long outp_rows, float* stats_out, int batch, int h,
                            int w, int cout, int stride, int act, int wshift, void* stream_) {
    hipStream_t stream = (hipStream_t)stream_;
    const int cpp = stride == 2 ? 4 : 8;
    if (!image || !image_planes || !w_planes || (!out && !out_planes) || batch <= 0 || h < 7 || w < 7 || cout <= 0 || cout % 4 != 0 ||
        wshift < 0 || wshift > 14 || (stride != 1 && stride != 2) || channels <= 0 || channels > (stride == 2 ? 3 : 8) ||
        (normalize && (!mean3 || !std3)) || act < 0 || act > 3) {
        um_set_error("um_conv7_fwd: bad argument (batch=%d channels=%d h=%d w=%d cout=%d stride=%d)", batch, channels, h, w, cout, stride);
        return -1;
    }
    const int hp = h + 6, wp = conv7_wp(w);
    const int ho = (h - 1) / stride + 1, wo = (w - 1) / stride + 1;
    const long rows = (long)batch * hp * wp, m = (long)batch * ho * wo;
    if ((out && (out_ld < out_coff + cout || out_ld % 4 != 0 || out_coff % 4 != 0)) ||
        (out_planes && (outp_ld < outp_coff + cout || outp_ld % 4 != 0 || outp_coff % 4 != 0 || outp_rows < m))) {
        um_set_error("um_conv7_fwd: inconsistent leading dimensions / offsets / row counts");
        return -1;
    }
    if (stats_out && !out) {
        um_set_error("um_conv7_fwd: fused statistics need the fp32 output");
        return -1;
    }
    if (bias && ((unsigned long)bias & 15) != 0) {
        um_set_error("um_conv7_fwd: bias must be 16-byte aligned");
        return -1;
    }
    if ((rows + 8) * cpp * 2 >= (1L << 32) || m >= (1L << 31)) {
        um_set_error("um_conv7_fwd: image batch beyond the 32-bit addressing of this kernel");
        return -4;
    }
    const long plane_stride = (rows + 8) * cpp;
    {
        ScopedKernelTimer timer(UM_K_CONV, stream);
        const float mm[3] = {normalize ? mean3[0] : 0.f, normalize ? mean3[1] : 0.f, normalize ? mean3[2] : 0.f};
        const float ss[3] = {normalize ? std3[0] : 1.f, normalize ? std3[1] : 1.f, normalize ? std3[2] : 1.f};
        const dim3 grid((unsigned)((rows + 255) / 256));
        if (cpp == 4)
            hipLaunchKernelGGL((pack7_kernel<4>), grid, dim3(256), 0, stream, image, (unsigned short*)image_planes, plane_stride,
                               batch, channels, h, w, hp, wp, normalize, mm[0], mm[1], mm[2], ss[0], ss[1], ss[2]);
        else
            hipLaunchKernelGGL((pack7_kernel<8>), grid, dim3(256), 0, stream, image, (unsigned short*)image_planes, plane_stride,
                               batch, channels, h, w, hp, wp, normalize, mm[0], mm[1], mm[2], ss[0], ss[1], ss[2]);
    }
    ConvArgs a;
    a.ap = (const unsigned short*)image_planes;
    a.a_plane_stride = plane_stride;
    a.row_stride = (unsigned)cpp * 2;
    a.zero_row = 0;
    a.wp = (const unsigned short*)w_planes;
    a.w_plane_stride = (long)cout * 7 * 8 * cpp;
    a.bias = bias;
    a.out = out;
    a.out_ld = out_ld;
    a.out_coff = out_coff;
    a.outp = (unsigned short*)out_planes;
    a.outp_ld = outp_ld;
    a.outp_coff = outp_coff;
    a.outp_plane_stride = outp_rows * outp_ld;
    a.stats = stats_out;
    a.addend = nullptr;
    a.addend_ld = 0;
    a.B = batch;
    a.Hi = hp;
    a.Wi = wp;
    a.Cin = 8 * cpp;
    a.Ho = ho;
    a.Wo = wo;
    a.Cout = cout;
    a.KH = 7;
    a.KW = 1;
    a.stride = stride;
    a.pad_h = 0;
    a.pad_w = 0;
    a.M = (int)m;
    a.act = act;
    a.gate = 0;
    a.gate_c = a.gate_zld = 0;
    a.gate_h = nullptr;
    a.gate_z = nullptr;
    a.out_scale = ldexpf(1.f, -wshift);
    a.xcd = conv_xcd_enabled();
    a.xf = a.nstats = nullptr;
    a.norm_relu = 0;
    hipError_t e;
    if (cout % 128 == 0 || cout > 192) e = launch_conv<4>(a, 0, stream);
    else if (cout % 96 == 0) e = launch_conv<3>(a, 0, stream);
    else e = launch_conv<2>(a, 0, stream);
    if (e != hipSuccess) {
        um_set_error("um_conv7_fwd: launch failed: %s", hipGetErrorString(e));
        return (int)e;
    }
    return 0;
}

extern "C" size_t um_stem_planes_bytes(int batch, int h, int w) { return um_conv7_planes_bytes(batch, h, w, 2); }

extern "C" int um_stem_conv_fwd(const float* image, int normalize, const float* mean3, const float* std3, void* image_planes,
                                const void* w_planes, float* out, float* stats_out, int batch, int h, int w, int cout,
                                int wshift, void* stream_) {
    return um_conv7_fwd(image, 3, normalize, mean3, std3, image_planes, w_planes, nullptr, out, cout, 0, nullptr, 0, 0, 0, stats_out,
                        batch, h, w, cout, 2, 0, wshift, stream_);
}
```

unimatch_amd/csrc/nhwc_ops.hip:

```cpp
#include "common.h"
#include "planes.h"

#define NHWC_CHUNK_ROWS 256

__global__ __launch_bounds__(256) void nhwc_stats_kernel(const float* x, float* partial, int P, int C, int nchunk) {
    __shared__ float red[2][256 * 4];
    const int b = blockIdx.y, ch = blockIdx.x;
    const int quads = C >> 2, rl_n = 256 / quads;
    const int q = threadIdx.x % quads, rl = threadIdx.x / quads;
    const int r0 = ch * NHWC_CHUNK_ROWS, r1 = min(P, r0 + NHWC_CHUNK_ROWS);
    const float* xb = x + ((long)b * P) * C + 4 * q;
    f32x4 s1 = {0.f, 0.f, 0.f, 0.f}, s2 = s1;
    if (rl < rl_n) {
        const f32x4 k = *reinterpret_cast<const f32x4*>(xb + (long)r0 * C);
        for (int r = r0 + rl; r < r1; r += rl_n) {
            const f32x4 v = *reinterpret_cast<const f32x4*>(xb + (long)r * C) - k;
            s1 += v;
            s2 += v * v;
        }
    }
#pragma unroll
    for (int i = 0; i < 4; ++i) {
        red[0][threadIdx.x * 4 + i] = s1[i];
        red[1][threadIdx.x * 4 + i] = s2[i];
    }
    __syncthreads();
    if ((int)threadIdx.x < C) {
        const int c = threadIdx.x, cq = c >> 2, ci = c & 3;
        float a1 = 0.f, a2 = 0.f;
        for (int l = 0; l < rl_n; ++l) {
            a1 += red[0][(l * quads + cq) * 4 + ci];
            a2 += red[1][(l * quads + cq) * 4 + ci];
        }
        float* pr = partial + (((long)b * nchunk + ch) * 3) * C;
        pr[c] = x[((long)b * P + r0) * C + c];
        pr[C + c] = a1;
        pr[2 * C + c] = a2;
    }
}

__global__ __launch_bounds__(256) void nhwc_stats_finalize_kernel(const float* partial, float* stats, int P, int C, int nparts,
                                                                  int rpp, float eps) {
    __shared__ double red[256];
    __shared__ double bc[8];
    const int b = blockIdx.y;
    const int ch = threadIdx.x & 7, c = blockIdx.x * 8 + ch, ln = threadIdx.x >> 3;
    const bool counted = rpp == 0;
    const int tail = counted ? 1 : P - (nparts - 1) * rpp;
    const double inv_full = counted ? 0.0 : 1.0 / (double)rpp, inv_tail = 1.0 / (double)tail;
    const float* base = partial + ((long)b * nparts * 3) * C + c;
    constexpr int NB = 32;
    const bool in_regs = nparts <= 32 * NB;
    float rk[NB], r1[NB], r2[NB];
    double sx = 0.0;
    if (in_regs) {
#pragma unroll
        for (int j = 0; j < NB; ++j) {
            const int pt = ln + 32 * j;
            rk[j] = r1[j] = r2[j] = 0.f;
            if (pt < nparts) {
                const float* pr = base + (long)pt * 3 * C;
                rk[j] = pr[0];
                r1[j] = pr[C];
                r2[j] = pr[2 * C];
            }
        }
#pragma unroll
        for (int j = 0; j < NB; ++j) {
            const int pt = ln + 32 * j;
            if (pt < nparts)
                sx += counted ? (double)r1[j] * (double)rk[j]
                              : (pt == nparts - 1 ? (double)tail : (double)rpp) * (double)rk[j] + (double)r1[j];
        }
    } else {
#pragma unroll 8
        for (int pt = ln; pt < nparts; pt += 32) {
            const float* pr = base + (long)pt * 3 * C;
            sx += counted ? (double)pr[C] * (double)pr[0]
                          : (pt == nparts - 1 ? (double)tail : (double)rpp) * (double)pr[0] + (double)pr[C];
        }
    }
    red[threadIdx.x] = sx;
    __syncthreads();
    if (ln == 0) {
        double t = 0.0;
        for (int l = 0; l < 32; ++l) t += red[l * 8 + ch];
        bc[ch] = t / (double)P;
    }
    __syncthreads();
    const double mean = bc[ch];
    double m2 = 0.0;
    auto add_part = [&](int pt, double k, double s1, double s2) {
        if (counted) {
            const double d = k - mean;
            m2 += s2 + s1 * d * d;
            return;
        }
        const bool last = pt == nparts - 1;
        const double n = last ? (double)tail : (double)rpp, inv = last ? inv_tail : inv_full;
        const double d = k + s1 * inv - mean;
        m2 += (s2 - s1 * s1 * inv) + n * d * d;
    };
    if (in_regs) {
#pragma unroll
        for (int j = 0; j < NB; ++j) {
            const int pt = ln + 32 * j;
            if (pt < nparts) add_part(pt, rk[j], r1[j], r2[j]);
        }
    } else {
#pragma unroll 8
        for (int pt = ln; pt < nparts; pt += 32) {
            const float* pr = base + (long)pt * 3 * C;
            add_part(pt, pr[0], pr[C], pr[2 * C]);
        }
    }
    red[threadIdx.x] = m2;
    __syncthreads();
    if (ln == 0) {
        double t = 0.0;
        for (int l = 0; l < 32; ++l) t += red[l * 8 + ch];
        const double var = t / (double)P;
        stats[((long)b * 2) * C + c] = (float)mean;
        stats[((long)b * 2 + 1) * C + c] = (float)(1.0 / sqrt((var > 0.0 ? var : 0.0) + (double)eps));
    }
}

template <typename T, int NS>
__global__ __launch_bounds__(256) void nhwc_apply_kernel(const float* x, const float* stats, const float* shortcut,
                                                         const unsigned short* shortcut_planes, unsigned short* planes,
                                                         float* outf, long rows, int P, int C, int relu) {
    const int c8n = C >> 3;
    const long idx = (long)blockIdx.x * 256 + threadIdx.x;
    const long total = (rows + (planes ? 1 : 0)) * c8n;
    if (idx >= total) return;
    const long row = idx / c8n;
    const int c = (int)(idx - row * c8n) * 8;
    const long plane_stride = (rows + 1) * C;
    if (row == rows) {
        const u32x4 z = {0u, 0u, 0u, 0u};
#pragma unroll
        for (int pl = 0; pl < NS; ++pl) *reinterpret_cast<u32x4*>(planes + pl * plane_stride + row * C + c) = z;
        return;
    }
    float v[8];
    {
        const f32x4 a0 = __builtin_nontemporal_load(reinterpret_cast<const f32x4*>(x + row * C + c));
        const f32x4 a1 = __builtin_nontemporal_load(reinterpret_cast<const f32x4*>(x + row * C + c + 4));
#pragma unroll
        for (int i = 0; i < 4; ++i) {
            v[i] = a0[i];
            v[4 + i] = a1[i];
        }
    }
    if (stats) {
        const int b = (int)(row / P);
        const float* mu = stats + ((long)b * 2) * C + c;
        const float* rs = mu + C;
#pragma unroll
        for (int i = 0; i < 8; ++i) v[i] = (v[i] - mu[i]) * rs[i];
    }
    if (relu) {
#pragma unroll
        for (int i = 0; i < 8; ++i) v[i] = fmaxf(v[i], 0.f);
    }
    if (shortcut) {
        const f32x4 s0 = *reinterpret_cast<const f32x4*>(shortcut + row * C + c);
        const f32x4 s1 = *reinterpret_cast<const f32x4*>(shortcut + row * C + c + 4);
#pragma unroll
        for (int i = 0; i < 4; ++i) {
            v[i] = fmaxf(v[i] + s0[i], 0.f);
            v[4 + i] = fmaxf(v[4 + i] + s1[i], 0.f);
        }
    } else if (shortcut_planes) {
        const u32x4 sh = *reinterpret_cast<const u32x4*>(shortcut_planes + row * C + c);
        u32x4 sl = {0u, 0u, 0u, 0u};
        if (NS == 2) sl = *reinterpret_cast<const u32x4*>(shortcut_planes + plane_stride + row * C + c);
#pragma unroll
        for (int i = 0; i < 4; ++i) {
            const f32x2 uh = T::unpack2(sh[i]);
            f32x2 ul = {0.f, 0.f};
            if (NS == 2) ul = T::unpack2(sl[i]);
            v[2 * i] = fmaxf(v[2 * i] + (uh[0] + ul[0]), 0.f);
            v[2 * i + 1] = fmaxf(v[2 * i + 1] + (uh[1] + ul[1]), 0.f);
        }
    }
    if (outf) {
        *reinterpret_cast<f32x4*>(outf + row * C + c) = f32x4{v[0], v[1], v[2], v[3]};
        *reinterpret_cast<f32x4*>(outf + row * C + c + 4) = f32x4{v[4], v[5], v[6], v[7]};
    }
    if (planes) {
        const u32x4 h = {T::pack2(v[0], v[1]), T::pack2(v[2], v[3]), T::pack2(v[4], v[5]), T::pack2(v[6], v[7])};
        *reinterpret_cast<u32x4*>(planes + row * C + c) = h;
        if (NS == 2) {
            u32x4 l;
#pragma unroll
            for (int i = 0; i < 4; ++i) {
                const f32x2 u = T::unpack2(h[i]);
                l[i] = T::pack2(v[2 * i] - u[0], v[2 * i + 1] - u[1]);
            }
            *reinterpret_cast<u32x4*>(planes + plane_stride + row * C + c) = l;
        }
    }
}

template <typename T, int NS>
__global__ __launch_bounds__(256) void nchw_to_nhwc_kernel(const float* x, unsigned short* planes, float* outf, int P, int C,
                                                           long rows) {
    __shared__ float tile[256 * 65];
    const int b = blockIdx.y, p0 = blockIdx.x * 64;
    const int px = threadIdx.x & 63;
    for (int c = threadIdx.x >> 6; c < C; c += 4) {
        const int p = min(p0 + px, P - 1);
        tile[c * 65 + px] = x[((long)b * C + c) * P + p];
    }
    __syncthreads();
    const int c8n = C >> 3;
    const long plane_stride = (rows + 1) * C;
    for (int it = threadIdx.x; it < 64 * c8n; it += 256) {
        const int pl_px = it / c8n, c = (it - pl_px * c8n) * 8;
        if (p0 + pl_px >= P) continue;
        const long row = (long)b * P + p0 + pl_px;
        float v[8];
#pragma unroll
        for (int i = 0; i < 8; ++i) v[i] = tile[(c + i) * 65 + pl_px];
        if (outf) {
            *reinterpret_cast<f32x4*>(outf + row * C + c) = f32x4{v[0], v[1], v[2], v[3]};
            *reinterpret_cast<f32x4*>(outf + row * C + c + 4) = f32x4{v[4], v[5], v[6], v[7]};
        }
        if (planes) {
            const u32x4 h = {T::pack2(v[0], v[1]), T::pack2(v[2], v[3]), T::pack2(v[4], v[5]), T::pack2(v[6], v[7])};
            *reinterpret_cast<u32x4*>(planes + row * C + c) = h;
            if (NS == 2) {
                u32x4 l;
#pragma unroll
                for (int i = 0; i < 4; ++i) {
                    const f32x2 u = T::unpack2(h[i]);
                    l[i] = T::pack2(v[2 * i] - u[0], v[2 * i + 1] - u[1]);
                }
                *reinterpret_cast<u32x4*>(planes + plane_stride + row * C + c) = l;
            }
        }
    }
    if (planes && blockIdx.x == 0 && b == 0) {
        for (int c = threadIdx.x; c < C; c += 256)
#pragma unroll
            for (int pl = 0; pl < NS; ++pl) planes[pl * plane_stride + rows * C + c] = 0;
    }
}

__global__ __launch_bounds__(256) void nhwc_gate_kernel(int mode, const float* src, int src_ld, const float* zr, float* hbuf,
                                                        unsigned short* planes, long plane_stride, int ld, int coff, long rows,
                                                        int C) {
    const int c4n = (C + 3) >> 2;
    const long idx = (long)blockIdx.x * 256 + threadIdx.x;
    if (idx >= rows * c4n) return;
    const long row = idx / c4n;
    const int c = (int)(idx - row * c4n) * 4;
    float v[4];
#pragma unroll
    for (int i = 0; i < 4; ++i) {
        const int ci = c + i;
        float x = 0.f;
        if (ci < C) {
            if (mode == 0) x = src[row * src_ld + ci];
            else if (mode == 1) x = zr[row * (2 * C) + C + ci] * hbuf[row * C + ci];
            else {
                const float z = zr[row * (2 * C) + ci];
                x = (1.0f - z) * hbuf[row * C + ci] + z * src[row * src_ld + ci];
                hbuf[row * C + ci] = x;
            }
        }
        v[i] = x;
    }
    if (!planes) return;
    const unsigned h0 = Fp16::pack2(v[0], v[1]), h1 = Fp16::pack2(v[2], v[3]);
    const f32x2 u0 = Fp16::unpack2(h0), u1 = Fp16::unpack2(h1);
    const unsigned l0 = Fp16::pack2(v[0] - u0[0], v[1] - u0[1]), l1 = Fp16::pack2(v[2] - u1[0], v[3] - u1[1]);
    unsigned short* d = planes + row * ld + coff + c;
    if (c + 4 <= C) {
        *reinterpret_cast<u32x2*>(d) = u32x2{h0, h1};
        *reinterpret_cast<u32x2*>(d + plane_stride) = u32x2{l0, l1};
    } else {
        const unsigned hh[2] = {h0, h1}, ll[2] = {l0, l1};
        for (int i = 0; c + i < C; ++i) {
            d[i] = (unsigned short)(hh[i >> 1] >> (16 * (i & 1)));
            d[plane_stride + i] = (unsigned short)(ll[i >> 1] >> (16 * (i & 1)));
        }
    }
}

extern void um_set_error(const char* fmt, ...);

extern "C" size_t um_nhwc_norm_workspace_bytes(int batch, int pixels, int channels) {
    if (batch <= 0 || pixels <= 0 || channels <= 0) return 0;
    const long nchunk = (pixels + NHWC_CHUNK_ROWS - 1) / NHWC_CHUNK_ROWS;
    return (size_t)((long)batch * nchunk * 3 * channels + (long)batch * 2 * channels) * sizeof(float);
}

extern "C" size_t um_conv_stats_bytes(int batch, int parts, int channels) {
    if (batch <= 0 || parts <= 0 || channels <= 0) return 0;
    return (size_t)((long)batch * parts * 3 * channels) * sizeof(float);
}

static bool nhwc_channels_ok(int c) { return c > 0 && c % 8 == 0 && c <= 256; }

extern "C" int um_nhwc_instance_norm(const float* x, const float* shortcut, const void* shortcut_planes, void* planes_out, float* f32_out, int batch,
                                     int pixels, int channels, float eps, int normalize, int relu, const float* conv_stats, int conv_stats_parts,
                                     void* workspace, size_t workspace_bytes, int mode, void* stream_) {
    hipStream_t stream = (hipStream_t)stream_;
    if (!x || (!planes_out && !f32_out) || batch <= 0 || pixels <= 0 || !nhwc_channels_ok(channels) || (mode != 0 && mode != 1)) {
        um_set_error("um_nhwc_instance_norm: bad argument (batch=%d pixels=%d channels=%d: channels must be a multiple of 8, <= 256)",
                     batch, pixels, channels);
        return -1;
    }
    const long rows = (long)batch * pixels;
    const int nchunk = (pixels + NHWC_CHUNK_ROWS - 1) / NHWC_CHUNK_ROWS;
    float* partial = (float*)workspace;
    float* stats = nullptr;
    ScopedKernelTimer timer(UM_K_INSTANCE_NORM, stream);
    if (normalize) {
        if (!workspace || workspace_bytes < um_nhwc_norm_workspace_bytes(batch, pixels, channels)) {
            um_set_error("um_nhwc_instance_norm: workspace too small");
            return -3;
        }
        stats = partial + (long)batch * nchunk * 3 * channels;
        if (conv_stats) {
            if (conv_stats_parts <= 0) {
                um_set_error("um_nhwc_instance_norm: conv_stats needs conv_stats_parts = um_conv_stats_parts() of the convolution");
                return -1;
            }
            hipLaunchKernelGGL(nhwc_stats_finalize_kernel, dim3(channels / 8, batch), dim3(256), 0, stream, conv_stats, stats, pixels, channels,
                               conv_stats_parts, 0, eps);
        } else {
            hipLaunchKernelGGL(nhwc_stats_kernel, dim3(nchunk, batch), dim3(256), 0, stream, x, partial, pixels, channels, nchunk);
            hipLaunchKernelGGL(nhwc_stats_finalize_kernel, dim3(channels / 8, batch), dim3(256), 0, stream, partial, stats, pixels, channels,
                               nchunk, NHWC_CHUNK_ROWS, eps);
        }
    }
    const long total = (rows + (planes_out ? 1 : 0)) * (channels / 8);
    const dim3 grid((unsigned)((total + 255) / 256));
    if (mode == 0)
        hipLaunchKernelGGL((nhwc_apply_kernel<Fp16, 2>), grid, dim3(256), 0, stream, x, stats, shortcut,
                           (const unsigned short*)shortcut_planes, (unsigned short*)planes_out, f32_out, rows, pixels, channels, relu);
    else
        hipLaunchKernelGGL((nhwc_apply_kernel<Bf16, 1>), grid, dim3(256), 0, stream, x, stats, shortcut,
                           (const unsigned short*)shortcut_planes, (unsigned short*)planes_out, f32_out, rows, pixels, channels, relu);
    const hipError_t e = hipGetLastError();
    if (e != hipSuccess) {
        um_set_error("um_nhwc_instance_norm: launch failed: %s", hipGetErrorString(e));
        return (int)e;
    }
    return 0;
}

extern "C" int um_nhwc_stats_finalize(const float* conv_stats, int conv_stats_parts, float* stats_out, int batch, int pixels, int channels,
                                      float eps, void* stream_) {
    hipStream_t stream = (hipStream_t)stream_;
    if (!conv_stats || conv_stats_parts <= 0 || !stats_out || batch <= 0 || pixels <= 0 || !nhwc_channels_ok(channels)) {
        um_set_error("um_nhwc_stats_finalize: bad argument (parts=%d batch=%d pixels=%d channels=%d: channels must be a multiple of 8, "
                     "<= 256)", conv_stats_parts, batch, pixels, channels);
        return -1;
    }
    ScopedKernelTimer timer(UM_K_INSTANCE_NORM, stream);
    hipLaunchKernelGGL(nhwc_stats_finalize_kernel, dim3(channels / 8, batch), dim3(256), 0, stream, conv_stats, stats_out, pixels, channels,
                       conv_stats_parts, 0, eps);
    const hipError_t e = hipGetLastError();
    if (e != hipSuccess) {
        um_set_error("um_nhwc_stats_finalize: launch failed: %s", hipGetErrorString(e));
        return (int)e;
    }
    return 0;
}

extern "C" int um_nchw_to_nhwc(const float* x, void* planes_out, float* f32_out, int batch, int channels, int pixels, int mode,
                               void* stream_) {
    hipStream_t stream = (hipStream_t)stream_;
    if (!x || (!planes_out && !f32_out) || batch <= 0 || pixels <= 0 || channels <= 0 || channels % 8 != 0 || channels > 256 ||
        (mode != 0 && mode != 1)) {
        um_set_error("um_nchw_to_nhwc: bad argument (batch=%d channels=%d pixels=%d: channels must be a multiple of 8, <= 256)",
                     batch, channels, pixels);
        return -1;
    }
    const long rows = (long)batch * pixels;
    const dim3 grid((pixels + 63) / 64, batch);
    ScopedKernelTimer timer(UM_K_INSTANCE_NORM, stream);
    if (mode == 0)
        hipLaunchKernelGGL((nchw_to_nhwc_kernel<Fp16, 2>), grid, dim3(256), 0, stream, x, (unsigned short*)planes_out, f32_out,
                           pixels, channels, rows);
    else
        hipLaunchKernelGGL((nchw_to_nhwc_kernel<Bf16, 1>), grid, dim3(256), 0, stream, x, (unsigned short*)planes_out, f32_out,
                           pixels, channels, rows);
    const hipError_t e = hipGetLastError();
    if (e != hipSuccess) {
        um_set_error("um_nchw_to_nhwc: launch failed: %s", hipGetErrorString(e));
        return (int)e;
    }
    return 0;
}

extern "C" int um_nhwc_gate(int mode, const float* src, int src_ld, const float* zr, float* hbuf, void* planes_out, int ld, int coff,
                            long plane_rows, long rows, int channels, void* stream_) {
    hipStream_t stream = (hipStream_t)stream_;
    const bool ok = rows > 0 && channels > 0 && mode >= 0 && mode <= 2 && (mode == 1 || src) && (mode == 0 || (zr && hbuf)) &&
                    (mode == 2 || planes_out) &&
                    (!planes_out || (ld >= coff + channels && plane_rows >= rows && (channels % 4 != 0 || coff % 4 == 0)));
    if (!ok) {
        um_set_error("um_nhwc_gate: bad argument (mode=%d rows=%ld channels=%d ld=%d coff=%d)", mode, rows, channels, ld, coff);
        return -1;
    }
    const long total = rows * ((channels + 3) / 4);
    ScopedKernelTimer timer(UM_K_INSTANCE_NORM, stream);
    hipLaunchKernelGGL(nhwc_gate_kernel, dim3((unsigned)((total + 255) / 256)), dim3(256), 0, stream, mode, src, src_ld, zr, hbuf,
                       (unsigned short*)planes_out, plane_rows * ld, ld, coff, rows, channels);
    const hipError_t e = hipGetLastError();
    if (e != hipSuccess) {
        um_set_error("um_nhwc_gate: launch failed: %s", hipGetErrorString(e));
        return (int)e;
    }
    return 0;
}
```

unimatch_amd/csrc/planes.h:

```cpp
#pragma once
#include "common.h"
#include "timing.h"

template <class T, int NS>
__global__ __launch_bounds__(256) void split_planes_kernel(const float* __restrict__ src,
                                                           unsigned short* __restrict__ dst,
                                                           long n8, float scale, long plane_stride, unsigned* range_flag) {
    long i = (long)blockIdx.x * blockDim.x + threadIdx.x;
    const long step = (long)gridDim.x * blockDim.x;
    float mx = 0.f;
    for (; i < n8; i += step) {
        const f32x4* s4 = reinterpret_cast<const f32x4*>(src) + 2 * i;
        f32x4 a = s4[0], b = s4[1];
        float x[8] = {a[0], a[1], a[2], a[3], b[0], b[1], b[2], b[3]};
        float y[8];
        u32x4 hi;
#pragma unroll
        for (int j = 0; j < 8; ++j) {
            y[j] = x[j] * scale;
            mx = fmaxf(mx, __builtin_fabsf(y[j]));
        }
#pragma unroll
        for (int j = 0; j < 4; ++j) hi[j] = T::pack2(y[2 * j], y[2 * j + 1]);
        *reinterpret_cast<u32x4*>(dst + 8 * i) = hi;
        if (NS == 2) {
            u32x4 lo;
#pragma unroll
            for (int j = 0; j < 4; ++j) {
                f32x2 h = T::unpack2(hi[j]);
                lo[j] = T::pack2(y[2 * j] - h[0], y[2 * j + 1] - h[1]);
            }
            *reinterpret_cast<u32x4*>(dst + plane_stride + 8 * i) = lo;
        }
    }
    um_range_note<T>(range_flag, mx, UM_RANGE_PLANES);
}

static inline hipError_t launch_split_elems(const float* src, unsigned short* dst, long n_elems, float scale,
                                            int mode, hipStream_t stream);

static inline hipError_t launch_split_planes(const float* src, unsigned short* dst, long rows, float scale,
                                             int mode, hipStream_t stream) {
    return launch_split_elems(src, dst, rows * UM_CHANNELS, scale, mode, stream);
}

static inline hipError_t launch_split_elems(const float* src, unsigned short* dst, long n_elems, float scale,
                                            int mode, hipStream_t stream) {
    const long n8 = n_elems / 8;
    long blocks = (n8 + 255) / 256;
    if (blocks > 8192) blocks = 8192;
    if (blocks < 1) blocks = 1;
    const long plane_stride = n_elems;
    ScopedKernelTimer timer(UM_K_SPLIT_PLANES, stream);
    if (mode == 0)
        hipLaunchKernelGGL((split_planes_kernel<Fp16, 2>), dim3((unsigned)blocks), dim3(256), 0, stream, src, dst, n8,
                           scale, plane_stride, um_range_flag_dev());
    else
        hipLaunchKernelGGL((split_planes_kernel<Bf16, 1>), dim3((unsigned)blocks), dim3(256), 0, stream, src, dst, n8,
                           scale, plane_stride, (unsigned*)nullptr);
    return hipGetLastError();
}

static inline size_t planes_bytes(long rows, int mode) {
    return (size_t)rows * UM_CHANNELS * 2 * (mode == 0 ? 2 : 1);
}
```

unimatch_amd/encoder.py:

```python

import torch
import torch.nn as nn
import torch.nn.functional as F


def _conv3(cin, cout, stride=1):
    return nn.Conv2d(cin, cout, 3, stride=stride, padding=1, bias=False)


class _Residual(nn.Module):

    def __init__(self, cin, cout, stride):
        super().__init__()
        self.conv1, self.conv2 = _conv3(cin, cout, stride), _conv3(cout, cout)
        self.norm1, self.norm2 = nn.InstanceNorm2d(cout), nn.InstanceNorm2d(cout)
        self.downsample = None
        if stride != 1 or cin != cout:
            self.norm3 = nn.InstanceNorm2d(cout)
            self.downsample = nn.Sequential(nn.Conv2d(cin, cout, 1, stride=stride), self.norm3)

    def forward(self, x, ops=None):
        if ops is not None:
            y = ops.instance_norm(self.conv1(x), relu=True)
            sc = x if self.downsample is None else ops.instance_norm(self.downsample[0](x), relu=False)
            return ops.instance_norm(self.conv2(y), relu=True, shortcut=sc.contiguous())
        y = F.relu(self.norm1(self.conv1(x)))
        y = F.relu(self.norm2(self.conv2(y)))
        return F.relu((x if self.downsample is None else self.downsample(x)) + y)


    def forward_nhwc(self, act, ops, want_f32):
        planes, f32, b, h, w, c = act
        stride = self.conv1.stride[0]
        cout = self.conv1.out_channels
        t, ho, wo = ops.conv2d_nhwc((planes, b, h, w, c), self.conv1.weight, None, stride, (1, 1), stats=True)
        if getattr(ops, 'norm_on_load', False) and ops.conv2d_norm_supported(ho, wo, cout, self.conv2.weight):
            u, _, _ = ops.conv2d_nhwc_normed(t, ops.last_conv_stats, (b, ho, wo, cout), self.conv2.weight, stats=True)
        else:
            tp, _ = ops.nhwc_norm(t, b, ho * wo, relu=True, want_planes=True, conv_stats=ops.last_conv_stats)
            u, _, _ = ops.conv2d_nhwc((tp, b, ho, wo, cout), self.conv2.weight, None, 1, (1, 1), stats=True)
        ustats = ops.last_conv_stats
        sc = scp = None
        if self.downsample is None:
            sc, scp = (f32, None) if f32 is not None else (None, planes)
        else:
            proj = self.downsample[0]
            d, _, _ = ops.conv2d_nhwc((planes, b, h, w, c), proj.weight, proj.bias, stride, (0, 0), stats=True)
            _, sc = ops.nhwc_norm(d, b, ho * wo, relu=False, want_planes=False, want_f32=True, conv_stats=ops.last_conv_stats)
        op, of = ops.nhwc_norm(u, b, ho * wo, relu=True, shortcut=sc, shortcut_planes=scp, want_planes=True, want_f32=want_f32,
                               conv_stats=ustats)
        return op, of, b, ho, wo, cout


class _SharedStridedConv(nn.Module):

    def __init__(self, channels, num_branch):
        super().__init__()
        self.num_branch = num_branch
        self.weight = nn.Parameter(torch.empty(channels, channels, 3, 3))
        nn.init.kaiming_uniform_(self.weight, nonlinearity='relu')

    def forward(self, x):
        return [F.conv2d(x, self.weight, None, stride=2 ** i, padding=1) for i in range(self.num_branch)]

    def forward_nhwc(self, act, ops):
        planes, _, b, h, w, c = act
        outs = []
        for i in range(self.num_branch):
            o, ho, wo = ops.conv2d_nhwc((planes, b, h, w, c), self.weight, None, 2 ** i, (1, 1))
            outs.append(o.view(b, ho, wo, -1).permute(0, 3, 1, 2))
        return outs


class CNNEncoder(nn.Module):

    def __init__(self, output_dim=128, num_output_scales=1):
        super().__init__()
        self.num_branch = num_output_scales
        d0, d1, d2 = 64, 96, 128
        self.conv1 = nn.Conv2d(3, d0, 7, stride=2, padding=3, bias=False)
        self.norm1 = nn.InstanceNorm2d(d0)
        self.layer1 = nn.Sequential(_Residual(d0, d0, 1), _Residual(d0, d0, 1))
        self.layer2 = nn.Sequential(_Residual(d0, d1, 2), _Residual(d1, d1, 1))
        self.layer3 = nn.Sequential(_Residual(d1, d2, 2 if num_output_scales == 1 else 1), _Residual(d2, d2, 1))
        self.conv2 = nn.Conv2d(d2, output_dim, 1)
        if num_output_scales > 1:
            if num_output_scales > 4:
                raise ValueError('at most 4 output scales')
            self.trident_conv = _SharedStridedConv(output_dim, num_output_scales)
        for m in self.modules():
            if isinstance(m, nn.Conv2d):
                nn.init.kaiming_normal_(m.weight, mode='fan_out', nonlinearity='relu')

    @staticmethod
    def takes_raw_images(ops, x):
        return ops is not None and getattr(ops, 'fused_conv', False) and x.is_cuda

    def forward(self, x, ops=None, input_norm=None):
        if self.takes_raw_images(ops, x):
            return self._forward_nhwc(x, ops, input_norm)
        assert input_norm is None
        if ops is not None and getattr(ops, 'fused_tail', False) and x.is_cuda:
            x = ops.instance_norm(self.conv1(x), relu=True)
            for layer in (self.layer1, self.layer2, self.layer3):
                for block in layer:
                    x = block(x, ops)
            x = self.conv2(x)
        else:
            x = F.relu(self.norm1(self.conv1(x)))
            x = self.conv2(self.layer3(self.layer2(self.layer1(x))))
        return self.trident_conv(x) if self.num_branch > 1 else [x]


    shortcut_f32 = False

    def _forward_nhwc(self, x, ops, input_norm=None):
        b = x.shape[0]
        y, h, w = ops.stem_conv(x.contiguous(), self.conv1.weight, input_norm, stats=True)
        c = y.shape[1]
        keep_f32 = self.shortcut_f32
        planes, f32 = ops.nhwc_norm(y, b, h * w, relu=True, want_planes=True, want_f32=keep_f32, conv_stats=ops.last_conv_stats)
        act = (planes, f32, b, h, w, c)
        blocks = [blk for layer in (self.layer1, self.layer2, self.layer3) for blk in layer]
        for i, blk in enumerate(blocks):
            nxt = blocks[i + 1] if i + 1 < len(blocks) else None
            act = blk.forward_nhwc(act, ops, want_f32=keep_f32 and nxt is not None and nxt.downsample is None)
        planes, _, b, h, w, c = act
        out, _, _ = ops.conv2d_nhwc((planes, b, h, w, c), self.conv2.weight, self.conv2.bias, 1, (0, 0))
        if self.num_branch == 1:
            return [out.view(b, h, w, -1).permute(0, 3, 1, 2)]
        tp, _ = ops.nhwc_norm(out, b, h * w, normalize=False, relu=False, want_planes=True)
        return self.trident_conv.forward_nhwc((tp, None, b, h, w, out.shape[1]), ops)
```

unimatch_amd/ops.py:

```python
import contextlib
import ctypes
import threading
import weakref
from collections import namedtuple

import torch

from . import _abi

PRECISIONS = {'exact': _abi.MODE_EXACT, 'fast': _abi.MODE_FAST}


class KernelTimer:

    def __init__(self):
        self.records = []

    def summary(self):
        torch.cuda.synchronize()
        out = {}
        for name, s, e, meta in self.records:
            d = out.setdefault(name, {'calls': 0, 'ms': 0.0, 'meta': meta})
            d['calls'] += 1
            d['ms'] += s.elapsed_time(e)
        return out


def _ptr(t):
    return t.data_ptr()


def _stream():
    return torch.cuda.current_stream().cuda_stream


def _check_tokens(name, t, n=None, tokens=None):
    if not (t.is_cuda and t.dtype == torch.float32 and t.dim() == 3 and t.is_contiguous()):
        raise ValueError(f'{name}: expected a contiguous CUDA float32 [N, L, C] tensor, got '
                         f'{tuple(t.shape)} {t.dtype} {t.device} contiguous={t.is_contiguous()}')
    if n is not None and t.shape[0] != n or tokens is not None and t.shape[1] != tokens:
        raise ValueError(f'{name}: shape {tuple(t.shape)} does not match N={n}, L={tokens}')


def _check_map(name, t, n, h, w):
    if not (t.is_cuda and t.dtype == torch.float32 and t.dim() == 4 and t.is_contiguous()
            and t.shape[0] == n and t.shape[2] == h and t.shape[3] == w):
        raise ValueError(f'{name}: expected a contiguous CUDA float32 [{n}, V, {h}, {w}] tensor, got '
                         f'{tuple(t.shape)} {t.dtype}')


def pack_kv4_weights(weights):
    w4 = torch.cat([w.detach().float() for w in weights], 0)
    perm = torch.arange(32, device=w4.device) ^ 16
    cross = w4[256:].view(8, 32, 128)[:, perm].reshape(256, 128)
    return torch.cat([w4[:256], cross], 1).contiguous()


WorkspaceKey = namedtuple('WorkspaceKey', 'kind geometry device owner')


class _Scope(threading.local):
    token = None
    lane = 0


class WorkspaceRegistry:

    GEOMETRIES = 8

    def __init__(self, stream=None, capturing=None):
        self._entries = {}
        self._scope = _Scope()
        self._stream_handle = stream or _stream
        self._capturing = capturing or torch.cuda.is_current_stream_capturing

    @contextlib.contextmanager
    def graph_scope(self, token):
        prev, self._scope.token = self._scope.token, token
        owned = {}
        try:
            yield owned
        finally:
            self._scope.token = prev
            for k in [k for k in self._entries if isinstance(k.owner, tuple) and k.owner[0] is token]:
                owned[k] = self._entries.pop(k)

    @contextlib.contextmanager
    def part_scope(self, lane):
        prev, self._scope.lane = self._scope.lane, lane
        try:
            yield
        finally:
            self._scope.lane = prev

    def workspace_scope(self):
        return self._scope.token, self._scope.lane

    def workspace_entries(self):
        return list(self._entries.items())

    def _workspace(self, kind, geometry, nbytes, device, keep):
        scope = self._scope
        owner = self._stream_handle() if scope.token is None else (scope.token, scope.lane)
        buf = self._entries.get((kind, geometry, device, owner))
        if buf is None:
            if self._capturing():
                return torch.zeros(nbytes, dtype=torch.uint8, device=device)
            group = [k for k in self._entries if (k.kind, k.device, k.owner) == (kind, device, owner)]
            for k in group[:max(0, len(group) + 1 - keep)]:
                del self._entries[k]
            buf = self._entries[WorkspaceKey(kind, geometry, device, owner)] = torch.zeros(nbytes, dtype=torch.uint8, device=device)
        return buf

    def release_cached_planes(self):
        for k in [k for k in self._entries if isinstance(k.kind, tuple)]:
            del self._entries[k]


class HipOps(WorkspaceRegistry):

    fused_tail = True
    fused_ffn = True
    fused_merge = True
    fused_qproj = True
    block_kv = True
    refine_hoist = True
    fused_kv = True
    fused_conv = True
    norm_on_load = True
    CONV_MODE = 0
    WSHIFT = 10

    def __init__(self, precision='exact'):
        if precision not in PRECISIONS:
            raise ValueError(f'precision must be one of {sorted(PRECISIONS)}')
        self.lib = _abi.load()
        if not torch.cuda.is_available():
            raise _abi.HipExtensionError('no GPU visible: the UniMatch hot path only runs on the HIP extension')
        self.precision = precision
        self.mode = PRECISIONS[precision]
        self.timer = None
        self.nplanes = 2 if precision == 'exact' else 1
        self._wcache = {}
        self.cache_generation = 0
        WorkspaceRegistry.__init__(self)

    def _ws(self, nbytes, device):
        return torch.empty(max(int(nbytes), 256), dtype=torch.uint8, device=device)

    def _launch(self, name, fn, meta=None):
        if self.timer is None:
            return fn()
        s, e = torch.cuda.Event(enable_timing=True), torch.cuda.Event(enable_timing=True)
        s.record()
        r = fn()
        e.record()
        self.timer.records.append((name, s, e, meta))
        return r

    def window_attention(self, q, k, v, h, w, win_h, win_w, shift_h=0, shift_w=0):
        s, l, c = q.shape
        _check_tokens('q', q, tokens=h * w)
        _check_tokens('k', k, s, l)
        _check_tokens('v', v, s, l)
        out = torch.empty_like(q)
        nbytes = self.lib.um_window_attn_workspace_bytes(s, l, c, self.mode)
        ws = self._ws(nbytes, q.device)
        n = win_h * win_w
        meta = {'flops': 4.0 * s * l * n * c, 'bytes': 4.0 * 4 * s * l * c}
        code = self._launch('window_attn', lambda: self.lib.um_window_attn_fwd(
            _ptr(q), _ptr(k), _ptr(v), _ptr(out), s, h, w, c, win_h, win_w, shift_h, shift_w,
            self.mode, _ptr(ws), ws.numel(), _stream()), meta)
        _abi.check(code, 'um_window_attn_fwd')
        return out

    def _cache_get(self, tag, tensors):
        key = (tag,) + tuple((id(t), t._version, t.data_ptr(), str(t.device), t.dtype) for t in tensors)
        hit = self._wcache.get(key)
        if hit is not None and all(r() is t for r, t in zip(hit[0], tensors)):
            return key, hit[1]
        return key, None

    def invalidate_weights(self):
        self._wcache.clear()
        self._entries.clear()
        self.cache_generation += 1

    def _cache_put(self, key, tensors, value):
        if len(self._wcache) > 256:
            self._wcache = {k: v for k, v in self._wcache.items() if all(r() is not None for r in v[0])}
            if len(self._wcache) > 256:
                self._wcache.clear()
        self._wcache[key] = (tuple(weakref.ref(t) for t in tensors), value)
        self.cache_generation += 1
        return value

    def weight_planes(self, weights):
        key, hit = self._cache_get('lin', weights)
        if hit is not None:
            return hit
        w = (weights[0] if len(weights) == 1 else torch.cat(list(weights), 0)).detach().float().contiguous()
        n, k = w.shape
        self._check_weight_range(w, self.WSHIFT if self.mode == 0 else 0, 'Linear weight')
        planes = torch.empty(self.lib.um_planes_bytes(n, k, self.mode), dtype=torch.uint8, device=w.device)
        _abi.check(self.lib.um_weight_planes(_ptr(w), _ptr(planes), n, k, self.WSHIFT, self.mode, _stream()),
                   'um_weight_planes')
        return self._cache_put(key, weights, (planes, n, k))

    @staticmethod
    def _check_weight_range(w, shift, what):
        limit = 65504.0 / float(1 << shift)
        amax = float(w.abs().max()) if w.numel() else 0.0
        if not amax < limit:
            raise ValueError(f'{what}: max |w| = {amax:.4g} does not fit the fp16 operand planes (|w| < {limit:.4g} at the '
                             f'2^{shift} pre-scale; see include/unimatch_hip.h, "Operand range")')

    def _check_rows(self, name, t, k):
        if not (t.is_cuda and t.dtype == torch.float32 and t.dim() == 2 and t.is_contiguous() and t.shape[1] == k):
            raise ValueError(f'{name}: expected a contiguous CUDA float32 [M, {k}] tensor, got {tuple(t.shape)} {t.dtype}')

    def linear_planes(self, a, weights, a1=None, gelu=False, a_planes_k=None):
        wp, n, k = self.weight_planes(weights)
        if a_planes_k is not None:
            m = a.numel() // (2 * self.nplanes * a_planes_k)
            args = (None, None, _ptr(a))
        else:
            m = a.shape[0]
            self._check_rows('a', a, k // 2 if a1 is not None else k)
            if a1 is not None:
                self._check_rows('a1', a1, k // 2)
            args = (_ptr(a), _ptr(a1) if a1 is not None else None, None)
        out = torch.empty(self.lib.um_planes_bytes(m, n, self.mode), dtype=torch.uint8, device=a.device)
        meta = {'flops': 2.0 * m * n * k}
        code = self._launch('linear', lambda: self.lib.um_linear_fwd(
            args[0], args[1], args[2], _ptr(wp), m, n, k, self.WSHIFT, 2 if gelu else 0, _ptr(out),
            None, None, None, 0.0, self.mode, _stream()), meta)
        _abi.check(code, 'um_linear_fwd')
        return out, m, n

    def linear_ln(self, a, weights, norm, residual=None, a_planes_k=None):
        wp, n, k = self.weight_planes(weights)
        if a_planes_k is not None:
            m = a.numel() // (2 * self.nplanes * a_planes_k)
            args = (None, None, _ptr(a))
        else:
            m = a.shape[0]
            self._check_rows('a', a, k)
            args = (_ptr(a), None, None)
        if residual is not None:
            self._check_rows('residual', residual, n)
        out = torch.empty((m, n), dtype=torch.float32, device=a.device)
        code = self._launch('linear', lambda: self.lib.um_linear_fwd(
            args[0], args[1], args[2], _ptr(wp), m, n, k, self.WSHIFT, 1, _ptr(out),
            _ptr(norm.weight), _ptr(norm.bias), _ptr(residual) if residual is not None else None,
            float(norm.eps), self.mode, _stream()), {'flops': 2.0 * m * n * k})
        _abi.check(code, 'um_linear_fwd')
        return out

    def ffn_ln(self, x, y, w1, w2, norm):
        w1p, hid, k1 = self.weight_planes((w1,))
        w2p, n2, k2 = self.weight_planes((w2,))
        if (k1, n2, k2) != (256, 128, hid):
            raise ValueError(f'ffn_ln: expected W1 [hidden, 256] and W2 [128, hidden], got {tuple(w1.shape)} {tuple(w2.shape)}')
        self._check_rows('x', x, 128)
        self._check_rows('y', y, 128)
        m = x.shape[0]
        if y.shape[0] != m:
            raise ValueError('ffn_ln: x and y must have the same number of rows')
        out = torch.empty((m, 128), dtype=torch.float32, device=x.device)
        ws = self._split_workspace('ffn_hsplit', (m, hid), x.device)
        code = self._launch('ffn', lambda: self.lib.um_ffn_ws_fwd(
            _ptr(x), _ptr(y), _ptr(w1p), _ptr(w2p), m, hid, self.WSHIFT, _ptr(norm.weight), _ptr(norm.bias),
            float(norm.eps), _ptr(out), self.mode, _ptr(ws) if ws is not None else None, ws.numel() if ws is not None else 0,
            _stream()), {'flops': 2.0 * m * hid * (256 + 128)})
        _abi.check(code, 'um_ffn_ws_fwd')
        return out

    def ffn_ln_kv(self, x, y, w1, w2, norm, kv_weights):
        w1p, hid, k1 = self.weight_planes((w1,))
        w2p, n2, k2 = self.weight_planes((w2,))
        if (k1, n2, k2) != (256, 128, hid):
            raise ValueError(f'ffn_ln_kv: expected W1 [hidden, 256] and W2 [128, hidden], got {tuple(w1.shape)} {tuple(w2.shape)}')
# ... 211 lines not shown
              and pred.dim() == want and gt.dim() == want and gt.shape[0] == pred.shape[0]
              and (not channels or (pred.shape[1] == channels and gt.shape[1] == channels)))
        if not ok:
            raise ValueError(f'{name}: expected CUDA float32 pred / gt of {want} dimensions and one batch, got {tuple(pred.shape)} '
                             f'{pred.dtype} and {tuple(gt.shape)} {gt.dtype}')
        b, (hp, wp), (h, w) = pred.shape[0], pred.shape[-2:], gt.shape[-2:]
        top, left = (int(crop[0]), int(crop[1])) if crop is not None else (0, 0)
        if top < 0 or left < 0 or top + h > hp or left + w > wp:
            raise ValueError(f'{name}: the crop {h}x{w} at ({top}, {left}) leaves the prediction {hp}x{wp}')
        out = []
        for m in masks:
            if m is not None:
                if not (m.is_cuda and m.device == pred.device and tuple(m.shape) == (b, h, w)):
                    raise ValueError(f'{name}: expected a CUDA mask [{b}, {h}, {w}], got {tuple(m.shape)} on {m.device}')
                m = m.float().contiguous()
            out.append(m)
        return pred.contiguous(), gt.contiguous(), out, (b, hp, wp, h, w, top, left)

    def flow_metrics(self, pred, gt, valid=None, noc_valid=None, crop=None):
        pred, gt, (valid, noc_valid), (b, hp, wp, h, w, top, left) = self._metric_args('flow_metrics', pred, gt, 2, crop, (valid, noc_valid))
        rows = torch.empty((b, 16), dtype=torch.float64, device=pred.device)
        ws = self._ws(self.lib.um_flow_metrics_workspace_bytes(b, h, w), pred.device)
        code = self._launch('flow_metrics', lambda: self.lib.um_flow_metrics(
            _ptr(pred), _ptr(gt), _ptr(valid) if valid is not None else None, _ptr(noc_valid) if noc_valid is not None else None,
            _ptr(rows), b, hp, wp, h, w, top, left, _ptr(ws), ws.numel(), _stream()))
        _abi.check(code, 'um_flow_metrics')
        return rows

    def disp_metrics(self, pred, gt, max_disp=0.0, crop=None):
        pred, gt, _, (b, hp, wp, h, w, top, left) = self._metric_args('disp_metrics', pred, gt, 0, crop, ())
        rows = torch.empty((b, 8), dtype=torch.float64, device=pred.device)
        ws = self._ws(self.lib.um_disp_metrics_workspace_bytes(b, h, w), pred.device)
        code = self._launch('disp_metrics', lambda: self.lib.um_disp_metrics(
            _ptr(pred), _ptr(gt), _ptr(rows), b, hp, wp, h, w, top, left, float(max_disp), _ptr(ws), ws.numel(), _stream()))
        _abi.check(code, 'um_disp_metrics')
        return rows

    def depth_metrics(self, pred, gt, valid=None, lo=0.0, hi=float('inf'), crop=None):
        pred, gt, (valid,), (b, hp, wp, h, w, top, left) = self._metric_args('depth_metrics', pred, gt, 0, crop, (valid,))
        rows = torch.empty((b, 8), dtype=torch.float64, device=pred.device)
        ws = self._ws(self.lib.um_depth_metrics_workspace_bytes(b, h, w), pred.device)
        code = self._launch('depth_metrics', lambda: self.lib.um_depth_metrics(
            _ptr(pred), _ptr(gt), _ptr(valid) if valid is not None else None, _ptr(rows), b, hp, wp, h, w, top, left, float(lo),
            float(hi), _ptr(ws), ws.numel(), _stream()))
        _abi.check(code, 'um_depth_metrics')
        return rows

    def flow_upsample2x(self, flow, mult=2.0):
        if not (flow.is_cuda and flow.dtype == torch.float32 and flow.dim() == 4):
            raise ValueError('flow_upsample2x: expected a CUDA float32 [B, V, h, w] tensor')
        flow = flow.contiguous()
        b, v, h, w = flow.shape
        out = torch.empty((b, v, 2 * h, 2 * w), dtype=torch.float32, device=flow.device)
        _abi.check(self.lib.um_flow_upsample2x(_ptr(flow), _ptr(out), b, v, h, w, float(mult), _stream()), 'um_flow_upsample2x')
        return out

    def depth_cam(self, intrinsics, pose, stride_div, bidir=False):
        b = intrinsics.shape[0]
        if not (tuple(intrinsics.shape) == (b, 3, 3) and tuple(pose.shape) == (b, 4, 4) and intrinsics.is_cuda and pose.is_cuda):
            raise ValueError('depth_cam: expected CUDA intrinsics [B,3,3] and pose [B,4,4]')
        k, p = intrinsics.float().contiguous(), pose.float().contiguous()
        cam = torch.empty((2 * b if bidir else b, 30), dtype=torch.float32, device=k.device)
        _abi.check(self.lib.um_depth_cam_pack(_ptr(k), _ptr(p), _ptr(cam), b, float(stride_div), int(bool(bidir)), _stream()),
                   'um_depth_cam_pack')
        return cam

    def rigid_flow(self, inv_depth, cam):
        b, _, h, w = inv_depth.shape
        if not (inv_depth.is_cuda and inv_depth.dtype == torch.float32 and tuple(cam.shape) == (b, 30)):
            raise ValueError('rigid_flow: expected CUDA float32 inv_depth [B,1,h,w] and cam [B,30]')
        inv_depth = inv_depth.contiguous()
        out = torch.empty((b, 2, h, w), dtype=torch.float32, device=inv_depth.device)
        _abi.check(self.lib.um_rigid_flow(_ptr(inv_depth), _ptr(cam), _ptr(out), b, h, w, _stream()), 'um_rigid_flow')
        return out

    def instance_norm(self, x, relu=True, shortcut=None, eps=1e-5):
        if not (x.is_cuda and x.dtype == torch.float32 and x.dim() == 4 and x.is_contiguous()):
            raise ValueError('instance_norm: expected a contiguous CUDA float32 NCHW tensor')
        if shortcut is not None and not (shortcut.shape == x.shape and shortcut.is_contiguous()
                                         and shortcut.dtype == torch.float32):
            raise ValueError('instance_norm: shortcut must match x')
        n, c, h, w = x.shape
        y = torch.empty_like(x)
        code = self._launch('instance_norm', lambda: self.lib.um_instance_norm_fwd(
            _ptr(x), _ptr(shortcut) if shortcut is not None else None, _ptr(y), n * c, h * w, float(eps),
            int(bool(relu)), _stream()))
        _abi.check(code, 'um_instance_norm_fwd')
        return y

    def conv_weight_planes(self, weight):
        key, hit = self._cache_get('conv', (weight,))
        if hit is not None:
            return hit
        cout, cin, kh, kw = weight.shape
        w2 = weight.detach().float().permute(0, 2, 3, 1).reshape(cout, kh * kw * cin).contiguous()
        planes = torch.empty(self.lib.um_planes_bytes(cout, kh * kw * cin, self.CONV_MODE), dtype=torch.uint8, device=w2.device)
        self._check_weight_range(w2, self.WSHIFT, 'convolution weight')
        _abi.check(self.lib.um_weight_planes(_ptr(w2), _ptr(planes), cout, kh * kw * cin, self.WSHIFT, self.CONV_MODE, _stream()),
                   'um_weight_planes')
        return self._cache_put(key, (weight,), (planes, cout, cin, kh, kw))

    def conv2d_nhwc(self, act, weight, bias=None, stride=1, padding=(1, 1), relu=False, stats=False):
        planes, b, h, w, cin = act
        wp, cout, wcin, kh, kw = self.conv_weight_planes(weight)
        if wcin != cin:
            raise ValueError(f'conv2d_nhwc: weight expects {wcin} input channels, activation has {cin}')
        ph, pw = (padding, padding) if isinstance(padding, int) else padding
        ho, wo = (h + 2 * ph - kh) // stride + 1, (w + 2 * pw - kw) // stride + 1
        out = torch.empty((b * ho * wo, cout), dtype=torch.float32, device=planes.device)
        self.last_conv_stats = None
        if stats:
            parts = self.lib.um_conv_stats_parts(h, w, cout, kh, kw, stride, ph, pw)
            self.last_conv_stats = (torch.empty(self.lib.um_conv_stats_bytes(b, parts, cout) // 4, dtype=torch.float32,
                                                device=planes.device), parts)
        st = self.last_conv_stats[0] if self.last_conv_stats is not None else None
        meta = {'flops': 2.0 * b * ho * wo * cout * kh * kw * cin}
        code = self._launch('conv', lambda: self.lib.um_conv2d_fwd(
            _ptr(planes), _ptr(wp), _ptr(bias) if bias is not None else None, _ptr(out), _ptr(st) if st is not None else None,
            b, h, w, cin, cout, kh, kw,
            stride, ph, pw, int(bool(relu)), self.WSHIFT, self.CONV_MODE, _stream()), meta)
        _abi.check(code, 'um_conv2d_fwd')
        return out, ho, wo

    def conv2d_norm_supported(self, h, w, cin, weight, stride=1, padding=(1, 1)):
        cout, wcin, kh, kw = weight.shape
        ph, pw = (padding, padding) if isinstance(padding, int) else padding
        return wcin == cin and bool(self.lib.um_conv2d_norm_supported(h, w, cin, cout, kh, kw, stride, ph, pw, self.CONV_MODE))

    def conv2d_nhwc_normed(self, x, conv_stats, geom, weight, bias=None, norm_relu=True, relu=False, stats=False, eps=1e-5):
        b, h, w, cin = geom
        self._check_rows('x', x, cin)
        if x.shape[0] != b * h * w:
            raise ValueError('conv2d_nhwc_normed: x must have b * h * w rows')
        wp, cout, wcin, kh, kw = self.conv_weight_planes(weight)
        if wcin != cin:
            raise ValueError(f'conv2d_nhwc_normed: weight expects {wcin} input channels, activation has {cin}')
        nstats = torch.empty((b, 2, cin), dtype=torch.float32, device=x.device)
        _abi.check(self._launch('instance_norm', lambda: self.lib.um_nhwc_stats_finalize(
            _ptr(conv_stats[0]), conv_stats[1], _ptr(nstats), b, h * w, cin, float(eps), _stream())), 'um_nhwc_stats_finalize')
        out = torch.empty((b * h * w, cout), dtype=torch.float32, device=x.device)
        self.last_conv_stats = None
        if stats:
            parts = self.lib.um_conv_stats_parts(h, w, cout, kh, kw, 1, 1, 1)
            self.last_conv_stats = (torch.empty(self.lib.um_conv_stats_bytes(b, parts, cout) // 4, dtype=torch.float32,
                                                device=x.device), parts)
        st = self.last_conv_stats[0] if self.last_conv_stats is not None else None
        meta = {'flops': 2.0 * b * h * w * cout * kh * kw * cin}
        code = self._launch('conv', lambda: self.lib.um_conv2d_norm_fwd(
            _ptr(x), _ptr(nstats), int(bool(norm_relu)), _ptr(wp), _ptr(bias) if bias is not None else None, _ptr(out),
            _ptr(st) if st is not None else None, b, h, w, cin, cout, kh, kw, 1, 1, 1, int(bool(relu)), self.WSHIFT, self.CONV_MODE,
            _stream()), meta)
        _abi.check(code, 'um_conv2d_norm_fwd')
        return out, h, w

    def nhwc_planes_from(self, pieces, pad_to=32):
        rows = pieces[0].shape[0]
        c = sum(p.shape[1] for p in pieces)
        cp = (c + pad_to - 1) // pad_to * pad_to
        if cp != c:
            pieces = list(pieces) + [torch.zeros((rows, cp - c), dtype=torch.float32, device=pieces[0].device)]
        x = pieces[0].contiguous() if len(pieces) == 1 else torch.cat(list(pieces), 1)
        planes, _ = self.nhwc_norm(x, 1, rows, normalize=False, relu=False, want_planes=True)
        return planes, cp

    def conv_weight_padded(self, weight, cin_to):
        key, hit = self._cache_get(('padw', cin_to), (weight,))
        if hit is None:
            cout, cin, kh, kw = weight.shape
            wpad = torch.zeros((cout, cin_to, kh, kw), dtype=torch.float32, device=weight.device)
            wpad[:, :cin] = weight.detach().float()
            hit = self._cache_put(key, (weight,), wpad)
        return hit

    def planes_buffer(self, rows, ld):
        return torch.zeros(2 * (rows + 1) * ld * 2, dtype=torch.uint8, device='cuda')

    def cached_planes_buffer(self, tag, rows, ld, device):
        return self._workspace(('planes', tag), (rows, ld), 2 * (rows + 1) * ld * 2, torch.device(device), 1)

    def conv_weight_planes_from(self, weight):
        cout, cin, kh, kw = weight.shape
        w2 = weight.detach().float().permute(0, 2, 3, 1).reshape(cout, kh * kw * cin).contiguous()
        planes = torch.empty(self.lib.um_planes_bytes(cout, kh * kw * cin, 0), dtype=torch.uint8, device=w2.device)
        self._check_weight_range(w2, self.WSHIFT, 'convolution weight')
        _abi.check(self.lib.um_weight_planes(_ptr(w2), _ptr(planes), cout, kh * kw * cin, self.WSHIFT, 0, _stream()),
                   'um_weight_planes')
        return planes, cout, cin, kh, kw

    def conv_ex(self, src, geom, wb, ksize, stride, pad, act, out=None, outp=None):
        buf, a_ld, a_coff, cin = src
        b, h, w = geom
        (wp, cout, wcin, kh, kw), bias = wb
        if wcin != cin or (kh, kw) != tuple(ksize):
            raise ValueError(f'conv_ex: weight is {cout}x{wcin}x{kh}x{kw}, call wants cin={cin} k={ksize}')
        a_rows = buf.numel() // (4 * a_ld)
        ho, wo = (h + 2 * pad[0] - kh) // stride + 1, (w + 2 * pad[1] - kw) // stride + 1
        o_t, o_ld, o_coff = out if out is not None else (None, 0, 0)
        p_t, p_ld, p_coff = outp if outp is not None else (None, 0, 0)
        p_rows = p_t.numel() // (4 * p_ld) if p_t is not None else 0
        code = self._launch('conv', lambda: self.lib.um_conv2d_ex(
            _ptr(buf), a_ld, a_coff, a_rows, _ptr(wp), _ptr(bias) if bias is not None else None,
            _ptr(o_t) if o_t is not None else None, o_ld, o_coff, _ptr(p_t) if p_t is not None else None, p_ld, p_coff, p_rows,
            None, b, h, w, cin, cout, kh, kw, stride, pad[0], pad[1], act, self.WSHIFT, 0, _stream()),
            {'flops': 2.0 * b * ho * wo * cout * kh * kw * cin})
        _abi.check(code, 'um_conv2d_ex')

    def conv_gru(self, gate, src, geom, wb, ksize, pad, hidden, outp, z=None, z_out=None, addend=None, hidden_out=None):
        buf, a_ld, a_coff, cin = src
        b, h, w = geom
        (wp, cout, wcin, kh, kw), bias = wb
        c = hidden.shape[1]
        if wcin != cin or (kh, kw) != tuple(ksize) or cout != (2 * c if gate == 1 else c):
            raise ValueError('conv_gru: weight / hidden shapes do not match')
        p_t, p_ld, p_coff = outp
        zt = z if gate == 2 else None
        if hidden_out is not None:
            if gate != 2 or addend is None or hidden_out.shape != hidden.shape or hidden_out.dtype != torch.float32 or not hidden_out.is_contiguous():
                raise ValueError('conv_gru: hidden_out goes with gate 2 and an addend, contiguous fp32 of the hidden state\'s shape')
            z_out = hidden_out
        if addend is not None:
            if not (addend.dtype == torch.float32 and addend.is_contiguous() and addend.dim() == 2 and addend.shape[1] == cout
                    and addend.shape[0] == geom[0] * geom[1] * geom[2]):
                raise ValueError(f'conv_gru: addend must be contiguous fp32 [b * h * w = {geom[0] * geom[1] * geom[2]}, cout = {cout}], '
                                 f'got {tuple(addend.shape)}')
            code = self._launch('conv', lambda: self.lib.um_conv2d_gru_add_fwd(
                gate, _ptr(buf), a_ld, a_coff, buf.numel() // (4 * a_ld), _ptr(wp), _ptr(bias) if bias is not None else None,
                _ptr(addend), addend.shape[1], _ptr(hidden), _ptr(zt) if zt is not None else None,
                zt.shape[1] if zt is not None else 0, _ptr(z_out) if z_out is not None else None,
                z_out.shape[1] if z_out is not None else 0, _ptr(p_t), p_ld, p_coff, p_t.numel() // (4 * p_ld), b, h, w, cin, c,
                kh, kw, pad[0], pad[1], self.WSHIFT, 0, _stream()), {'flops': 2.0 * b * h * w * cout * kh * kw * cin})
            _abi.check(code, 'um_conv2d_gru_add_fwd')
            return
        code = self._launch('conv', lambda: self.lib.um_conv2d_gru_fwd(
            gate, _ptr(buf), a_ld, a_coff, buf.numel() // (4 * a_ld), _ptr(wp), _ptr(bias) if bias is not None else None,
            _ptr(hidden), _ptr(zt) if zt is not None else None, zt.shape[1] if zt is not None else 0,
            _ptr(z_out) if z_out is not None else None, z_out.shape[1] if z_out is not None else 0, _ptr(p_t), p_ld, p_coff,
            p_t.numel() // (4 * p_ld), b, h, w, cin, c, kh, kw, pad[0], pad[1], self.WSHIFT, 0, _stream()),
            {'flops': 2.0 * b * h * w * cout * kh * kw * cin})
        _abi.check(code, 'um_conv2d_gru_fwd')

    def conv7(self, image, weight, bias, stride, act, out=None, outp=None):
        b, c, h, w = image.shape
        cout = weight.shape[0]
        cpp = 4 if stride == 2 else 8
        key, hit = self._cache_get(('conv7', stride), (weight,))
        if hit is None:
            wr = torch.zeros((cout, 7, 8, cpp), dtype=torch.float32, device=weight.device)
            wr[:, :, :7, :c] = weight.detach().float().permute(0, 2, 3, 1)
            wr = wr.reshape(cout, 56 * cpp).contiguous()
            wp = torch.empty(self.lib.um_planes_bytes(cout, 56 * cpp, 0), dtype=torch.uint8, device=weight.device)
            self._check_weight_range(wr, self.WSHIFT, 'convolution weight')
            _abi.check(self.lib.um_weight_planes(_ptr(wr), _ptr(wp), cout, 56 * cpp, self.WSHIFT, 0, _stream()), 'um_weight_planes')
            hit = self._cache_put(key, (weight,), wp)
        scratch = torch.empty(self.lib.um_conv7_planes_bytes(b, h, w, stride), dtype=torch.uint8, device=image.device)
        o_t, o_ld, o_coff = out if out is not None else (None, 0, 0)
        p_t, p_ld, p_coff = outp if outp is not None else (None, 0, 0)
        p_rows = p_t.numel() // (4 * p_ld) if p_t is not None else 0
        image = image.contiguous()
        code = self._launch('conv', lambda: self.lib.um_conv7_fwd(
            _ptr(image), c, 0, None, None, _ptr(scratch), _ptr(hit), _ptr(bias) if bias is not None else None,
            _ptr(o_t) if o_t is not None else None, o_ld, o_coff, _ptr(p_t) if p_t is not None else None, p_ld, p_coff, p_rows,
            None, b, h, w, cout, stride, act, self.WSHIFT, _stream()))
        _abi.check(code, 'um_conv7_fwd')

    def nhwc_gate(self, mode, src, dest, ld, coff, rows, channels, zr=None, hbuf=None):
        p_rows = dest.numel() // (4 * ld) if dest is not None else 0
        src_ld = src.shape[1] if src is not None else 0
        code = self._launch('instance_norm', lambda: self.lib.um_nhwc_gate(
            mode, _ptr(src) if src is not None else None, src_ld, _ptr(zr) if zr is not None else None,
            _ptr(hbuf) if hbuf is not None else None, _ptr(dest) if dest is not None else None, ld, coff, p_rows, rows, channels,
            _stream()))
        _abi.check(code, 'um_nhwc_gate')

    def local_corr_with_flow_planes(self, f0, f1, flow, h, w, radius, dest, ld):
        b, l, c = f0.shape
        _check_tokens('f0', f0, tokens=h * w)
        _check_tokens('f1', f1, b, l)
        flow = flow.contiguous()
        feat = self._k4_feat_planes(f0, f1, h, w, radius)
        if feat is not None:
            code = self._launch('local_corr_with_flow', lambda: self.lib.um_local_corr_with_flow_feat(
                _ptr(f0), _ptr(f1), _ptr(feat), _ptr(flow), None, _ptr(dest), ld, dest.numel() // (4 * ld), b, h, w, c, radius,
                self.k4_flags, None, _stream()))
            _abi.check(code, 'um_local_corr_with_flow_feat')
            return
        code = self._launch('local_corr_with_flow', lambda: self.lib.um_local_corr_with_flow_planes(
            _ptr(f0), _ptr(f1), _ptr(flow), _ptr(dest), ld, dest.numel() // (4 * ld), b, h, w, c, radius, _stream()))
        _abi.check(code, 'um_local_corr_with_flow_planes')

    k4_mfma = True
    k4_flags = 0

    def _k4_feat_planes(self, f0, f1, h, w, radius):
        if not self.k4_mfma or not self.lib.um_local_corr_with_flow_feat_supported(h, w, f0.shape[2], radius):
            return None
        key = (id(f0), f0._version, f0.data_ptr(), id(f1), f1._version, f1.data_ptr(), tuple(f0.shape))
        hit = getattr(self, '_k4_feat', None)
        if hit is not None and hit[0] == key and hit[1]() is f0 and hit[2]() is f1:
            return hit[3]
        b, l, c = f0.shape
        feat = torch.empty(self.lib.um_local_corr_feat_planes_bytes(b, h, w, c), dtype=torch.uint8, device=f0.device)
        _abi.check(self.lib.um_local_corr_feat_planes(_ptr(f0), _ptr(f1), _ptr(feat), b, h, w, c, _stream()),
                   'um_local_corr_feat_planes')
        self._k4_feat = (key, weakref.ref(f0), weakref.ref(f1), feat)
        return feat

    def stem_conv(self, image, weight, norm_mean_std=None, stats=True):
        if not (image.is_cuda and image.dtype == torch.float32 and image.dim() == 4 and image.shape[1] == 3
                and image.is_contiguous()):
            raise ValueError('stem_conv: expected a contiguous CUDA float32 [b, 3, h, w] image')
        if tuple(weight.shape[1:]) != (3, 7, 7):
            raise ValueError('stem_conv: expected a [cout, 3, 7, 7] weight')
        b, _, h, w = image.shape
        cout = weight.shape[0]
        key, hit = self._cache_get('stem', (weight,))
        if hit is None:
            wr = torch.zeros((cout, 7, 8, 4), dtype=torch.float32, device=weight.device)
            wr[:, :, :7, :3] = weight.detach().float().permute(0, 2, 3, 1)
            wr = wr.reshape(cout, 224).contiguous()
            wp = torch.empty(self.lib.um_planes_bytes(cout, 224, 0), dtype=torch.uint8, device=weight.device)
            self._check_weight_range(wr, self.WSHIFT, 'convolution weight')
            _abi.check(self.lib.um_weight_planes(_ptr(wr), _ptr(wp), cout, 224, self.WSHIFT, 0, _stream()), 'um_weight_planes')
            hit = self._cache_put(key, (weight,), wp)
        ho, wo = (h - 1) // 2 + 1, (w - 1) // 2 + 1
        scratch = torch.empty(self.lib.um_stem_planes_bytes(b, h, w), dtype=torch.uint8, device=image.device)
        out = torch.empty((b * ho * wo, cout), dtype=torch.float32, device=image.device)
        self.last_conv_stats = None
        if stats:
            parts = self.lib.um_conv_stats_parts(h, w, cout, 7, 7, 2, 3, 3)
            self.last_conv_stats = (torch.empty(self.lib.um_conv_stats_bytes(b, parts, cout) // 4, dtype=torch.float32,
                                                device=image.device), parts)
        st = self.last_conv_stats[0] if self.last_conv_stats is not None else None
        if norm_mean_std is not None:
            mean = (ctypes.c_float * 3)(*[float(v) for v in norm_mean_std[0]])
            std = (ctypes.c_float * 3)(*[float(v) for v in norm_mean_std[1]])
        else:
            mean = std = None
        code = self._launch('conv', lambda: self.lib.um_stem_conv_fwd(
            _ptr(image), int(norm_mean_std is not None), mean, std, _ptr(scratch), _ptr(hit), _ptr(out),
            _ptr(st) if st is not None else None, b, h, w, cout, self.WSHIFT, _stream()),
            {'flops': 2.0 * b * ho * wo * cout * 147})
        _abi.check(code, 'um_stem_conv_fwd')
        return out, ho, wo

    def nhwc_norm(self, x, b, pixels, normalize=True, relu=True, shortcut=None, want_planes=True, want_f32=False, eps=1e-5,
                  conv_stats=None, shortcut_planes=None):
        self._check_rows('x', x, x.shape[1])
        c = x.shape[1]
        if x.shape[0] != b * pixels:
            raise ValueError('nhwc_norm: x must have b * pixels rows')
        if shortcut is not None:
            self._check_rows('shortcut', shortcut, c)
        rows = b * pixels
        if shortcut_planes is not None and (shortcut is not None or shortcut_planes.numel() != self.lib.um_planes_bytes(rows + 1, c, self.CONV_MODE)):
            raise ValueError('nhwc_norm: shortcut_planes must be operand planes of [b * pixels + 1, c] (and exclude shortcut)')
        planes = (torch.empty(self.lib.um_planes_bytes(rows + 1, c, self.CONV_MODE), dtype=torch.uint8, device=x.device)
                  if want_planes else None)
        f32 = torch.empty_like(x) if want_f32 else None
        ws = self._ws(self.lib.um_nhwc_norm_workspace_bytes(b, pixels, c), x.device) if normalize else None
        code = self._launch('instance_norm', lambda: self.lib.um_nhwc_instance_norm(
            _ptr(x), _ptr(shortcut) if shortcut is not None else None,
            _ptr(shortcut_planes) if shortcut_planes is not None else None, _ptr(planes) if planes is not None else None,
            _ptr(f32) if f32 is not None else None, b, pixels, c, float(eps), int(bool(normalize)), int(bool(relu)),
            _ptr(conv_stats[0]) if conv_stats is not None else None, conv_stats[1] if conv_stats is not None else 0,
            _ptr(ws) if ws is not None else None, ws.numel() if ws is not None else 0, self.CONV_MODE, _stream()))
        _abi.check(code, 'um_nhwc_instance_norm')
        return planes, f32

    def nchw_to_nhwc(self, x, want_planes=True, want_f32=False):
        if not (x.is_cuda and x.dtype == torch.float32 and x.dim() == 4 and x.is_contiguous()):
            raise ValueError('nchw_to_nhwc: expected a contiguous CUDA float32 NCHW tensor')
        b, c, h, w = x.shape
        rows = b * h * w
        planes = (torch.empty(self.lib.um_planes_bytes(rows + 1, c, self.CONV_MODE), dtype=torch.uint8, device=x.device)
                  if want_planes else None)
        f32 = torch.empty((rows, c), dtype=torch.float32, device=x.device) if want_f32 else None
        code = self._launch('instance_norm', lambda: self.lib.um_nchw_to_nhwc(
            _ptr(x), _ptr(planes) if planes is not None else None, _ptr(f32) if f32 is not None else None, b, c, h * w,
            self.CONV_MODE, _stream()))
        _abi.check(code, 'um_nchw_to_nhwc')
        return planes, f32

    def global_corr_softmax_flow(self, f0, f1, h, w, bidir=False):
        b, l, c = f0.shape
        _check_tokens('f0', f0, tokens=h * w)
        _check_tokens('f1', f1, b, l)
        out = torch.empty((2 * b if bidir else b, 2, h, w), dtype=torch.float32, device=f0.device)
        ws = self._ws(self.lib.um_global_corr_workspace_bytes(b, l, c, self.mode), f0.device)
        meta = {'flops': (2.0 if bidir else 1.0) * b * (2.0 * l * l * c + 4.0 * l * l),
                'bytes': 2.0 * 4 * b * l * c + 8.0 * b * l}
        code = self._launch('global_corr_flow', lambda: self.lib.um_global_corr_softmax_flow(
            _ptr(f0), _ptr(f1), _ptr(out), b, h, w, c, int(bool(bidir)), self.mode,
            _ptr(ws), ws.numel(), _stream()), meta)
        _abi.check(code, 'um_global_corr_softmax_flow')
        return out

    def global_corr_softmax_stereo(self, f0, f1, h, w):
        b, l, c = f0.shape
        _check_tokens('f0', f0, tokens=h * w)
        _check_tokens('f1', f1, b, l)
        out = torch.empty((b, 1, h, w), dtype=torch.float32, device=f0.device)
        ws = self._ws(self.lib.um_global_corr_workspace_bytes(b, l, c, self.mode), f0.device)
        code = self._launch('global_corr_stereo', lambda: self.lib.um_global_corr_softmax_stereo(
            _ptr(f0), _ptr(f1), _ptr(out), b, h, w, c, self.mode, _ptr(ws), ws.numel(), _stream()))
        _abi.check(code, 'um_global_corr_softmax_stereo')
        return out

    def prop_global(self, q, k, value, h, w):
        b, l, c = q.shape
        _check_tokens('q', q, tokens=h * w)
        _check_tokens('k', k, b, l)
        _check_map('value', value, b, h, w)
        out = torch.empty_like(value)
        ws = self._ws(self.lib.um_global_corr_workspace_bytes(b, l, c, self.mode), q.device)
        vch = value.shape[1]
        meta = {'flops': b * (2.0 * l * l * c + 2.0 * l * l * vch), 'bytes': 2.0 * 4 * b * l * c + 8.0 * b * l * vch}
        code = self._launch('prop_global', lambda: self.lib.um_prop_global_attn(
            _ptr(q), _ptr(k), _ptr(value), _ptr(out), b, h, w, c, vch, self.mode,
            _ptr(ws), ws.numel(), _stream()), meta)
        _abi.check(code, 'um_prop_global_attn')
        return out

    def linear_bias(self, a, weight, bias, out_mul=1.0, bias_mul=1.0, planes=False, a_planes_k=None):
        wp, n, k = self.weight_planes((weight,))
        if a_planes_k is not None:
            m = a.numel() // (2 * self.nplanes * a_planes_k)
            src = (None, _ptr(a))
        else:
            m = a.shape[0]
            self._check_rows('a', a, k)
            src = (_ptr(a), None)
        bias = bias.detach()
        if not (bias.is_cuda and bias.dtype == torch.float32 and bias.is_contiguous() and bias.numel() == n):
            raise ValueError(f'linear_bias: expected a contiguous CUDA float32 bias of {n} elements')
        if planes:
            out = torch.empty(self.lib.um_planes_bytes(m, n, self.mode), dtype=torch.uint8, device=a.device)
            dst = (_ptr(out), None)
        else:
            out = torch.empty((m, n), dtype=torch.float32, device=a.device)
            dst = (None, _ptr(out))
        code = self._launch('linear', lambda: self.lib.um_linear_bias_fwd(
            src[0], src[1], _ptr(wp), _ptr(bias), m, n, k, self.WSHIFT, float(out_mul), float(bias_mul), dst[0], dst[1],
            self.mode, _stream()), {'flops': 2.0 * m * n * k})
        _abi.check(code, 'um_linear_bias_fwd')
        return out

    def prop_global_projected(self, tokens, q_proj, k_proj, value, h, w):
        b, l, c = tokens.shape
        _check_tokens('tokens', tokens, tokens=h * w)
        _check_map('value', value, b, h, w)
        ps = self.lib.um_global_corr_plane_scale(c)
        x = tokens.reshape(b * l, c)
        qp = self.linear_bias(x, q_proj.weight, q_proj.bias, out_mul=ps, bias_mul=ps, planes=True)
        kp = self.linear_bias(qp, k_proj.weight, k_proj.bias, out_mul=1.0, bias_mul=ps, planes=True, a_planes_k=c)
        out = torch.empty_like(value)
        ws = self._ws(self.lib.um_global_corr_workspace_bytes(b, l, c, self.mode), tokens.device)
        vch = value.shape[1]
        meta = {'flops': b * (2.0 * l * l * c + 2.0 * l * l * vch), 'bytes': 2.0 * 4 * b * l * c + 8.0 * b * l * vch}
        code = self._launch('prop_global', lambda: self.lib.um_prop_global_attn_planes(
            _ptr(qp), _ptr(kp), _ptr(value), _ptr(out), b, h, w, c, vch, self.mode, _ptr(ws), ws.numel(), _stream()), meta)
        _abi.check(code, 'um_prop_global_attn_planes')
        return out

    def local_corr_softmax(self, f0, f1, h, w, radius, one_d=False):
        b, l, c = f0.shape
        _check_tokens('f0', f0, tokens=h * w)
        _check_tokens('f1', f1, b, l)
        out = torch.empty((b, 1 if one_d else 2, h, w), dtype=torch.float32, device=f0.device)
        if not one_d and self.k4_mfma and self.lib.um_local_corr_with_flow_feat_supported(h, w, c, radius):
            ws = self._ws(self.lib.um_local_corr_feat_planes_bytes(b, h, w, c), f0.device)
            code = self._launch('local_corr_softmax', lambda: self.lib.um_local_corr_softmax_mfma(
                _ptr(f0), _ptr(f1), _ptr(out), b, h, w, c, radius, _ptr(ws), ws.numel(), _stream()))
            _abi.check(code, 'um_local_corr_softmax_mfma')
            return out
        code = self._launch('local_corr_softmax', lambda: self.lib.um_local_corr_softmax(
            _ptr(f0), _ptr(f1), _ptr(out), b, h, w, c, radius, int(bool(one_d)), _stream()))
        _abi.check(code, 'um_local_corr_softmax')
        return out

    def local_corr_with_flow(self, f0, f1, flow, h, w, radius, dilation=1):
        b, l, c = f0.shape
        _check_tokens('f0', f0, tokens=h * w)
        _check_tokens('f1', f1, b, l)
        _check_map('flow', flow, b, h, w)
        if flow.shape[1] != 2:
            raise ValueError('flow must have 2 channels')
        k = 2 * radius + 1
        out = torch.empty((b, k * k, h, w), dtype=torch.float32, device=f0.device)
        meta = {'flops': 2.0 * b * l * (k + 1) ** 2 * c, 'bytes': 2.0 * 4 * b * l * c + 8.0 * b * l + 4.0 * k * k * b * l}
        if dilation != 1:
            code = self._launch('local_corr_with_flow', lambda: self.lib.um_local_corr_with_flow_dilated(
                _ptr(f0), _ptr(f1), _ptr(flow.contiguous()), _ptr(out), b, h, w, c, radius, int(dilation), _stream()), meta)
            _abi.check(code, 'um_local_corr_with_flow_dilated')
            return out
        feat = self._k4_feat_planes(f0, f1, h, w, radius)
        if feat is not None:
            code = self._launch('local_corr_with_flow', lambda: self.lib.um_local_corr_with_flow_feat(
                _ptr(f0), _ptr(f1), _ptr(feat), _ptr(flow), _ptr(out), None, 0, 0, b, h, w, c, radius, self.k4_flags,
                None, _stream()), meta)
            _abi.check(code, 'um_local_corr_with_flow_feat')
            return out
        code = self._launch('local_corr_with_flow', lambda: self.lib.um_local_corr_with_flow(
            _ptr(f0), _ptr(f1), _ptr(flow), _ptr(out), b, h, w, c, radius, _stream()), meta)
        _abi.check(code, 'um_local_corr_with_flow')
        return out

    def prop_local(self, q, k, value, h, w, radius):
        b, l, c = q.shape
        _check_tokens('q', q, tokens=h * w)
        _check_tokens('k', k, b, l)
        _check_map('value', value, b, h, w)
# ... 22 lines not shown
```

Before: 911.3.

## Fuse residual-block epilogue norm into next downsampling conv with projection shortcut

Adds a conv_entry kernel that takes the previous block's raw conv output plus its stats and shortcut planes. It applies instance norm, residual add and ReLU while loading each tile, then runs the 3x3 stride-2 conv and the 1x1 projection conv together, reusing the centre-tap activation tile. A second new norm kernel normalizes the shortcut with its own stats, so the separate shortcut norm pass is dropped. Together these remove an instance-norm launch, a planes write and reread, and a separate projection conv at layer boundaries. The cost is extra registers for a second accumulator set and more LDS, so a build-time guard checks that the new kernel has no scratch and keeps occupancy of at least 2.

After: 929.9, median of 6. +2.1%, better.

```diff
diff --git a/include/unimatch_hip.h b/include/unimatch_hip.h
--- a/include/unimatch_hip.h
+++ b/include/unimatch_hip.h
@@ -154,12 +154,23 @@
                           int batch, int pixels, int channels, float eps, int normalize, int relu, const float* conv_stats,
                           int conv_stats_parts, void* workspace, size_t workspace_bytes, int mode, void* stream);
 
+size_t um_nhwc_norm_sc_workspace_bytes(int batch, int pixels, int channels);
+int um_nhwc_instance_norm_sc(const float* x, const float* shortcut, const void* shortcut_planes, void* planes_out, float* f32_out,
+                             int batch, int pixels, int channels, float eps, int normalize, int relu, const float* conv_stats,
+                             int conv_stats_parts, void* workspace, size_t workspace_bytes, int mode, void* stream,
+                             const float* sc_conv_stats, int sc_conv_stats_parts);
+
 int um_nhwc_stats_finalize(const float* conv_stats, int conv_stats_parts, float* stats_out, int batch, int pixels, int channels,
                            float eps, void* stream);
 int um_conv2d_norm_supported(int hi, int wi, int cin, int cout, int kh, int kw, int stride, int pad_h, int pad_w, int mode);
 int um_conv2d_norm_fwd(const float* x, const float* norm_stats, int norm_relu, const void* w_planes, const float* bias, float* out,
                        float* stats_out, int batch, int hi, int wi, int cin, int cout, int kh, int kw, int stride, int pad_h,
                        int pad_w, int relu, int wshift, int mode, void* stream);
+
+int um_conv2d_entry_supported(int hi, int wi, int cin, int cout, int kh, int kw, int stride, int pad_h, int pad_w, int mode);
+int um_conv2d_entry_fwd(const float* u, const float* ustats, const void* s_planes, const void* w_planes, const void* w2_planes,
+                        const float* bias2, float* out_t, float* out_d, float* stats_t, float* stats_d, int batch, int hi, int wi,
+                        int cin, int cout, int kh, int kw, int stride, int pad_h, int pad_w, int wshift, int mode, void* stream);
 
 int um_nhwc_gate(int mode, const float* src, int src_ld, const float* zr, float* hbuf, void* planes_out, int ld, int coff,
                  long plane_rows, long rows, int channels, void* stream);
diff --git a/unimatch_amd/_abi.py b/unimatch_amd/_abi.py
--- a/unimatch_amd/_abi.py
+++ b/unimatch_amd/_abi.py
@@ -50,6 +50,11 @@
                                         _c_int, _c_void_p, _c_int, _c_void_p, _c_int, _c_int, ctypes.c_long] + [_c_int] * 11 + [_c_void_p]),
     'um_conv2d_norm_supported': (_c_int, [_c_int] * 10),
     'um_conv2d_norm_fwd': (_c_int, [_c_void_p, _c_void_p, _c_int] + [_c_void_p] * 4 + [_c_int] * 13 + [_c_void_p]),
+    'um_conv2d_entry_supported': (_c_int, [_c_int] * 10),
+    'um_conv2d_entry_fwd': (_c_int, [_c_void_p] * 10 + [_c_int] * 12 + [_c_void_p]),
+    'um_nhwc_norm_sc_workspace_bytes': (_c_size_t, [_c_int] * 3),
+    'um_nhwc_instance_norm_sc': (_c_int, [_c_void_p] * 5 + [_c_int] * 3 + [ctypes.c_float, _c_int, _c_int, _c_void_p, _c_int, _c_void_p,
+                                          _c_size_t, _c_int, _c_void_p, _c_void_p, _c_int]),
     'um_nhwc_stats_finalize': (_c_int, [_c_void_p, _c_int, _c_void_p] + [_c_int] * 3 + [ctypes.c_float, _c_void_p]),
     'um_conv_stats_bytes': (_c_size_t, [_c_int] * 3),
     'um_conv_stats_parts': (_c_int, [_c_int] * 8),
diff --git a/unimatch_amd/build.py b/unimatch_amd/build.py
--- a/unimatch_amd/build.py
+++ b/unimatch_amd/build.py
@@ -1,4 +1,5 @@
 import os
+import re
 import shutil
 import subprocess
 import sys
@@ -15,6 +16,7 @@
                'video.hip': ['-ffp-contract=off'],
                'metrics.hip': ['-ffp-contract=off', '-fhip-fp32-correctly-rounded-divide-sqrt'],
                'prepost.hip': ['-ffp-contract=off', '-fhip-fp32-correctly-rounded-divide-sqrt']}
+RESOURCE_GUARDS = {'conv.hip': {'conv_entry_kernel': 2}}
 FLAGS = ['--offload-arch=gfx950', '-O3', '-std=c++17', '-fPIC', '-fno-gpu-rdc', '-Wno-unused-result']
 
 
@@ -23,6 +25,30 @@
         if cand and os.path.exists(cand):
             return cand
     raise RuntimeError('hipcc not found: the HIP extension cannot be built')
+
+
+def parse_resource_report(text):
+    out, cur = {}, None
+    for line in text.splitlines():
+        m = re.search(r'remark: .*?Function Name: (\S+)', line)
+        if m:
+            cur = out.setdefault(m.group(1), {})
+            continue
+        m = re.search(r'remark: .*?\s{2,}([A-Za-z ]+?)(?: \[[^\]]*\])?: (\d+)', line)
+        if m and cur is not None:
+            cur[m.group(1).strip()] = int(m.group(2))
+    return out
+
+
+def check_resources(src, report):
+    for key, min_occ in RESOURCE_GUARDS.get(src, {}).items():
+        hits = {k: v for k, v in report.items() if key in k}
+        if not hits:
+            raise RuntimeError(f'{src}: no resource report for {key}: the guard of unimatch_amd/build.py has nothing to check')
+        for name, r in hits.items():
+            if r.get('ScratchSize', -1) != 0 or r.get('Occupancy', 0) < min_occ:
+                raise RuntimeError(f'{src}: {name} needs scratch {r.get("ScratchSize")} B/lane at occupancy {r.get("Occupancy")} '
+                                   f'({r.get("VGPRs")} VGPRs): it was written for no scratch at {min_occ} waves per SIMD')
 
 
 def _stale(target, deps):
@@ -41,11 +67,25 @@
     for src in SOURCES:
         s = os.path.join(CSRC, src)
         o = os.path.join(objdir, src.replace('.hip', '.o'))
-        if force or _stale(o, [s] + hdrs):
+        if force or _stale(o, [s] + hdrs) or (src in RESOURCE_GUARDS and not os.path.exists(o[:-2] + '.resources.txt')):
             cmd = [hipcc] + FLAGS + EXTRA_FLAGS.get(src, []) + ['-c', s, '-o', o]
             if verbose:
                 print(' '.join(cmd))
-            subprocess.run(cmd, check=True, cwd=CSRC)
+            if src in RESOURCE_GUARDS:
+                done = subprocess.run(cmd + ['-Rpass-analysis=kernel-resource-usage', '-fno-caret-diagnostics'], cwd=CSRC, stderr=subprocess.PIPE, text=True)
+                remarks = [ln for ln in done.stderr.splitlines() if 'kernel-resource-usage' in ln]
+                sys.stderr.write('\n'.join(ln for ln in done.stderr.splitlines() if 'kernel-resource-usage' not in ln))
+                if done.returncode != 0:
+                    raise subprocess.CalledProcessError(done.returncode, cmd)
+                try:
+                    check_resources(src, parse_resource_report('\n'.join(remarks)))
+                except RuntimeError:
+                    os.remove(o)
+                    raise
+                with open(o[:-2] + '.resources.txt', 'w') as f:
+                    f.write('\n'.join(remarks) + '\n')
+            else:
+                subprocess.run(cmd, check=True, cwd=CSRC)
         objs.append(o)
     if force or _stale(LIB, objs):
         cmd = [hipcc, '--offload-arch=gfx950', '-shared', '-fPIC', '-o', LIB] + objs + ['-ldl']
diff --git a/unimatch_amd/csrc/conv.hip b/unimatch_amd/csrc/conv.hip
--- a/unimatch_amd/csrc/conv.hip
+++ b/unimatch_amd/csrc/conv.hip
@@ -265,14 +265,34 @@
                                                               lane, half);
 }
 
-template <typename T, int NS, int NT>
-__global__ __launch_bounds__(256, 2) void conv_kernel(ConvArgs a) {
-    constexpr int TILE = 128 * 64;
-    constexpr int WTILE = 32 * NT * 64;
-    constexpr int STAGE = NS * (TILE + WTILE);
-    constexpr int EPI = 4 * 32 * (32 * NT * 4);
-    constexpr int RING = (2 * STAGE > EPI) ? 2 * STAGE : EPI;
-    __shared__ __attribute__((aligned(16))) unsigned char lds[RING + 8 * 2 * 32 * NT * 4 + 64];
+struct ConvEntryArgs {
+    const float* u;
+    const float* ustats;
+    const unsigned short* sp;
+    long s_plane_stride;
+    const unsigned short* wp2;
+    long w2_plane_stride;
+    const float* bias2;
+    float* out2;
+    float* stats2;
+};
+
+template <int NS, int NT>
+struct ConvLds {
+    static constexpr int TILE = 128 * 64;
+    static constexpr int WTILE = 32 * NT * 64;
+    static constexpr int STAGE = NS * (TILE + WTILE);
+    static constexpr int EPI = 4 * 32 * (32 * NT * 4);
+    static constexpr int RING = (2 * STAGE > EPI) ? 2 * STAGE : EPI;
+    static constexpr int TOTAL = RING + 8 * 2 * 32 * NT * 4 + 64;
+    static constexpr int ENTRY_CIN = 128;
+    static constexpr int ENTRY_TOTAL = TOTAL + 2 * ENTRY_CIN * 4;
+};
+
+template <typename T, int NS, int NT, bool ENTRY>
+__device__ __forceinline__ void conv_body(const ConvArgs& a, const ConvEntryArgs& e, unsigned char* lds) {
+    using L = ConvLds<NS, NT>;
+    constexpr int TILE = L::TILE, WTILE = L::WTILE, STAGE = L::STAGE, RING = L::RING;
 
     const int tid = threadIdx.x, lane = tid & 63;
     const int wave = __builtin_amdgcn_readfirstlane(tid >> 6);
@@ -307,19 +327,25 @@
         for (int i = 0; i < 2; ++i) {
             const int iy = py[i] + ky, ix = px[i] + kx;
             const bool ok = pok[i] && (unsigned)iy < (unsigned)a.Hi && (unsigned)ix < (unsigned)a.Wi;
-            const unsigned row = ok ? (unsigned)(pbase[i] + iy * a.Wi + ix) : zero_row;
-            rowoff[i] = row * a.row_stride;
+            if constexpr (ENTRY) {
+                rowoff[i] = ok ? (unsigned)(pbase[i] + iy * a.Wi + ix) : ~0u;
+            } else {
+                const unsigned row = ok ? (unsigned)(pbase[i] + iy * a.Wi + ix) : zero_row;
+                rowoff[i] = row * a.row_stride;
+            }
         }
     };
     int ky = 0, kx = 0, cc = 0;
     auto stage_async = [&](int c0, int kglob, unsigned char* buf) {
-#pragma unroll
-        for (int i = 0; i < 2; ++i) {
-            const int r = 32 * wave + 16 * i + (lane >> 2);
-            const int sc = dcp ^ ((r >> 2) & 3);
-            const unsigned off = rowoff[i] + (unsigned)((c0 + 8 * sc) * 2);
-#pragma unroll
-            for (int pl = 0; pl < NS; ++pl) conv_dma16(a.ap + pl * a.a_plane_stride, off, buf + pl * TILE + (32 * wave + 16 * i) * 64);
+        if constexpr (!ENTRY) {
+#pragma unroll
+            for (int i = 0; i < 2; ++i) {
+                const int r = 32 * wave + 16 * i + (lane >> 2);
+                const int sc = dcp ^ ((r >> 2) & 3);
+                const unsigned off = rowoff[i] + (unsigned)((c0 + 8 * sc) * 2);
+#pragma unroll
+                for (int pl = 0; pl < NS; ++pl) conv_dma16(a.ap + pl * a.a_plane_stride, off, buf + pl * TILE + (32 * wave + 16 * i) * 64);
+            }
         }
 #pragma unroll
         for (int i = 0; i < (2 * NT + 3) / 4; ++i) {
@@ -335,20 +361,97 @@
             }
         }
     };
+    const int esc = dcp ^ ((lane >> 4) & 3);
+    float* sstat = reinterpret_cast<float*>(lds + L::TOTAL);
+    f32x4 eu[2][2];
+    u32x4 esh[2], esl[2];
+    bool eok[2];
+    int ec0 = 0;
+    auto entry_load = [&](int c0) {
+        ec0 = c0 + 8 * esc;
+#pragma unroll
+        for (int i = 0; i < 2; ++i) {
+            eok[i] = rowoff[i] != ~0u;
+            const unsigned el = (eok[i] ? rowoff[i] : 0u) * (unsigned)a.Cin + (unsigned)ec0;
+            const unsigned char* pu = reinterpret_cast<const unsigned char*>(e.u) + el * 4u;
+            eu[i][0] = *reinterpret_cast<const f32x4*>(pu);
+            eu[i][1] = *reinterpret_cast<const f32x4*>(pu + 16);
+            const unsigned char* ps = reinterpret_cast<const unsigned char*>(e.sp) + el * 2u;
+            esh[i] = *reinterpret_cast<const u32x4*>(ps);
+            if (NS == 2) esl[i] = *reinterpret_cast<const u32x4*>(ps + e.s_plane_stride * 2);
+        }
+    };
+    auto entry_store = [&](unsigned char* buf) {
+        float mu[8], rs[8];
+        {
+            const f32x4 m0 = *reinterpret_cast<const f32x4*>(sstat + ec0), m1 = *reinterpret_cast<const f32x4*>(sstat + ec0 + 4);
+            const f32x4 r0 = *reinterpret_cast<const f32x4*>(sstat + a.Cin + ec0), r1 = *reinterpret_cast<const f32x4*>(sstat + a.Cin + ec0 + 4);
+#pragma unroll
+            for (int k = 0; k < 4; ++k) {
+                mu[k] = m0[k];
+                mu[4 + k] = m1[k];
+                rs[k] = r0[k];
+                rs[4 + k] = r1[k];
+            }
+        }
+#pragma unroll
+        for (int i = 0; i < 2; ++i) {
+            float v[8], none[8];
+#pragma unroll
+            for (int k = 0; k < 4; ++k) {
+                v[k] = eu[i][0][k];
+                v[4 + k] = eu[i][1][k];
+            }
+#pragma unroll
+            for (int k = 0; k < 8; ++k) none[k] = 0.f;
+            u32x4 h, l = {0u, 0u, 0u, 0u};
+            um_norm_value8<T, NS>(v, true, mu, rs, true, 2, none, false, none, none, esh[i], NS == 2 ? esl[i] : l, true, h, l);
+            unsigned char* dst = buf + (32 * wave + 16 * i) * 64 + lane * 16;
+#pragma unroll
+            for (int k = 0; k < 4; ++k) {
+                h[k] = eok[i] ? h[k] : 0u;
+                l[k] = eok[i] ? l[k] : 0u;
+            }
+            *reinterpret_cast<u32x4*>(dst) = h;
+            if (NS == 2) *reinterpret_cast<u32x4*>(dst + TILE) = l;
+        }
+    };
 
     f32x16 acc[NT];
 #pragma unroll
     for (int nt = 0; nt < NT; ++nt)
 #pragma unroll
         for (int r = 0; r < 16; ++r) acc[nt][r] = 0.f;
+    f32x16 acc2[ENTRY ? NT : 1];
+    if constexpr (ENTRY) {
+#pragma unroll
+        for (int nt = 0; nt < NT; ++nt)
+#pragma unroll
+            for (int r = 0; r < 16; ++r) acc2[nt][r] = 0.f;
+    }
 
     const int fr = lane & 31;
     int foff[2];
 #pragma unroll
     for (int ks = 0; ks < 2; ++ks) foff[ks] = fr * 64 + (((2 * ks + half) ^ ((fr >> 2) & 3)) << 4);
 
+    i16x8 pwh[ENTRY ? NT : 1], pwl[ENTRY ? NT : 1];
+    auto proj_load = [&](int pcc, int ks) {
+#pragma unroll
+        for (int nt = 0; nt < NT; ++nt) {
+            const int n = min(n0 + 32 * nt + fr, a.Cout - 1);
+            const unsigned short* pw = e.wp2 + (unsigned)(n * a.Cin + pcc * 32 + (2 * ks + half) * 8);
+            pwh[nt] = *reinterpret_cast<const i16x8*>(pw);
+            if (NS == 2) pwl[nt] = *reinterpret_cast<const i16x8*>(pw + e.w2_plane_stride);
+        }
+    };
+
     set_tap(0, 0);
     stage_async(0, 0, lds);
+    if constexpr (ENTRY) {
+        entry_load(0);
+        for (int k = tid; k < 2 * a.Cin; k += 256) sstat[k] = e.ustats[(long)bt * 2 * a.Cin + k];
+    }
     auto advance = [&]() {
         if (++cc == cpt) {
             cc = 0;
@@ -360,14 +463,24 @@
         }
     };
     advance();
+    if constexpr (ENTRY) {
+        __syncthreads();
+        entry_store(lds);
+    }
     asm volatile("s_waitcnt vmcnt(0)" ::: "memory");
     __syncthreads();
 
+    int ptap = 0, pcc = 0;
     for (int s = 0; s < nstage; ++s) {
         unsigned char* cur = lds + (s & 1) * STAGE;
         unsigned char* nxt = lds + ((s & 1) ^ 1) * STAGE;
+        const bool centre = ENTRY && ptap == 4;
+        if constexpr (ENTRY) {
+            if (centre) proj_load(pcc, 0);
+        }
         if (s + 1 < nstage) {
             stage_async(cc * 32, (s + 1) * 32, nxt);
+            if constexpr (ENTRY) entry_load(cc * 32);
             advance();
         }
         const unsigned char* at = cur + 32 * wave * 64;
@@ -388,8 +501,28 @@
                 }
                 acc[nt] = T::mfma(wh, bh, acc[nt]);
             }
+            if constexpr (ENTRY) {
+                if (centre) {
+#pragma unroll
+                    for (int nt = 0; nt < NT; ++nt) {
+                        if (NS == 2) {
+                            if (UM_CONV_2P != 1) acc2[nt] = T::mfma(pwl[nt], bh, acc2[nt]);
+                            if (UM_CONV_2P != 2) acc2[nt] = T::mfma(pwh[nt], bl, acc2[nt]);
+                        }
+                        acc2[nt] = T::mfma(pwh[nt], bh, acc2[nt]);
+                    }
+                    if (ks == 0) proj_load(pcc, 1);
+                }
+            }
         }
         __builtin_amdgcn_s_setprio(0);
+        if constexpr (ENTRY) {
+            if (s + 1 < nstage) entry_store(nxt);
+            if (++pcc == cpt) {
+                pcc = 0;
+                ++ptap;
+            }
+        }
         asm volatile("s_waitcnt vmcnt(0)" ::: "memory");
         __syncthreads();
     }
@@ -398,7 +531,28 @@
         const int rloc0 = pl0 + 32 * wave;
         conv_epilogue<T, NS, NT>(a, acc, lds, lds + RING, bt, rloc0, min(32, max(0, P - rloc0)), bt * ((P + 127) / 128) + pl0 / 128, false,
                                  n0, tid, wave, lane, half);
-    }
+        if constexpr (ENTRY) {
+            ConvArgs a2 = a;
+            a2.bias = e.bias2;
+            a2.out = e.out2;
+            a2.stats = e.stats2;
+            __syncthreads();
+            conv_epilogue<T, NS, NT>(a2, acc2, lds, lds + RING, bt, rloc0, min(32, max(0, P - rloc0)), bt * ((P + 127) / 128) + pl0 / 128,
+                                     false, n0, tid, wave, lane, half);
+        }
+    }
+}
+
+template <typename T, int NS, int NT>
+__global__ __launch_bounds__(256, 2) void conv_kernel(ConvArgs a) {
+    __shared__ __attribute__((aligned(16))) unsigned char lds[ConvLds<NS, NT>::TOTAL];
+    conv_body<T, NS, NT, false>(a, ConvEntryArgs{}, lds);
+}
+
+template <typename T, int NS, int NT>
+__global__ __launch_bounds__(256, 2) void conv_entry_kernel(ConvArgs a, ConvEntryArgs e) {
+    __shared__ __attribute__((aligned(16))) unsigned char lds[ConvLds<NS, NT>::ENTRY_TOTAL];
+    conv_body<T, NS, NT, true>(a, e, lds);
 }
 
 template <int NS, int NT, int KW, int NSLOT>
@@ -828,6 +982,18 @@
     return hipGetLastError();
 }
 
+template <int NT>
+static hipError_t launch_conv_entry(const ConvArgs& a, const ConvEntryArgs& e, int mode, hipStream_t stream) {
+    dim3 grid(a.B * ((a.Ho * a.Wo + 127) / 128) * ((a.Cout + 32 * NT - 1) / (32 * NT))), block(256);
+    ScopedKernelTimer timer(UM_K_CONV, stream);
+    um_census_hit(UM_V_CONV_GENERIC);
+    if (mode == 0)
+        hipLaunchKernelGGL((conv_entry_kernel<Fp16, 2, NT>), grid, block, 0, stream, a, e);
+    else
+        hipLaunchKernelGGL((conv_entry_kernel<Bf16, 1, NT>), grid, block, 0, stream, a, e);
+    return hipGetLastError();
+}
+
 template <int NT, int KW, int NSLOT>
 static hipError_t launch_conv_rows(const ConvArgs& a, int mode, hipStream_t stream) {
     static bool configured[2] = {false, false};
@@ -920,6 +1086,19 @@
     int nt;
     if (conv_pick(hi, wi, ho, wo, cout, kh, kw, stride, pad_h, pad_w, &nt) != CONV_PATCH) return 0;
     return nt >= 2 && nt <= 4 && kNormOnLoad[nt] ? 1 : 0;
+}
+
+static constexpr bool kEntryConv[5] = {false, false, false, true, true};
+
+extern "C" int um_conv2d_entry_supported(int hi, int wi, int cin, int cout, int kh, int kw, int stride, int pad_h, int pad_w, int mode) {
+    if (hi <= 0 || wi <= 0 || cin <= 0 || cin % 32 != 0 || cin > ConvLds<2, 4>::ENTRY_CIN || cout <= 0 || cout % 4 != 0 ||
+        (mode != 0 && mode != 1))
+        return 0;
+    if (kh != 3 || kw != 3 || stride != 2 || pad_h != 1 || pad_w != 1) return 0;
+    const int ho = (hi - 1) / 2 + 1, wo = (wi - 1) / 2 + 1;
+    int nt;
+    if (conv_pick(hi, wi, ho, wo, cout, 3, 3, 2, 1, 1, &nt) != CONV_GENERIC) return 0;
+    return nt >= 3 && nt <= 4 && kEntryConv[nt] ? 1 : 0;
 }
 
 extern "C" int um_conv_stats_parts(int hi, int wi, int cout, int kh, int kw, int stride, int pad_h, int pad_w) {
@@ -1122,6 +1301,71 @@
                        norm_stats, norm_relu ? 1 : 0);
 }
 
+extern "C" int um_conv2d_entry_fwd(const float* u, const float* ustats, const void* s_planes, const void* w_planes, const void* w2_planes,
+                                   const float* bias2, float* out_t, float* out_d, float* stats_t, float* stats_d, int batch, int hi, int wi,
+                                   int cin, int cout, int kh, int kw, int stride, int pad_h, int pad_w, int wshift, int mode, void* stream_) {
+    if (!u || !ustats || !s_planes || !w_planes || !w2_planes || !out_t || !out_d || batch <= 0 || wshift < 0 || wshift > 14) {
+        um_set_error("um_conv2d_entry_fwd: bad argument (a null input / output, batch=%d, wshift=%d)", batch, wshift);
+        return -1;
+    }
+    if (!um_conv2d_entry_supported(hi, wi, cin, cout, kh, kw, stride, pad_h, pad_w, mode)) {
+        um_set_error("um_conv2d_entry_fwd: no entry kernel for this geometry (hi=%d wi=%d cin=%d cout=%d k=%dx%d stride=%d pad=%d,%d mode=%d): "
+                     "ask um_conv2d_entry_supported() first", hi, wi, cin, cout, kh, kw, stride, pad_h, pad_w, mode);
+        return -2;
+    }
+    if ((((unsigned long)u | (unsigned long)s_planes | (unsigned long)w_planes | (unsigned long)w2_planes | (unsigned long)bias2 |
+          (unsigned long)out_t | (unsigned long)out_d) & 15) != 0 || (((unsigned long)ustats | (unsigned long)stats_t | (unsigned long)stats_d) & 3) != 0) {
+        um_set_error("um_conv2d_entry_fwd: inputs, planes, bias and outputs must be 16-byte aligned");
+        return -1;
+    }
+    const int ho = (hi - 1) / 2 + 1, wo = (wi - 1) / 2 + 1;
+    const long rows_in = (long)batch * hi * wi, m = (long)batch * ho * wo;
+    if (rows_in * cin * 4 >= (1L << 32) - 1 || (long)cout * 9 * cin * 2 >= (1L << 32) || m >= (1L << 31)) {
+        um_set_error("um_conv2d_entry_fwd: an input beyond 4 GiB is not addressable by this kernel");
+        return -4;
+    }
+    ConvArgs a;
+    memset(&a, 0, sizeof(a));
+    a.wp = (const unsigned short*)w_planes;
+    a.w_plane_stride = (long)cout * 9 * cin;
+    a.out = out_t;
+    a.out_ld = cout;
+    a.stats = stats_t;
+    a.B = batch;
+    a.Hi = hi;
+    a.Wi = wi;
+    a.Cin = cin;
+    a.Ho = ho;
+    a.Wo = wo;
+    a.Cout = cout;
+    a.KH = a.KW = 3;
+    a.stride = 2;
+    a.pad_h = a.pad_w = 1;
+    a.M = (int)m;
+    a.gate_c = cout;
+    a.out_scale = ldexpf(1.f, -wshift);
+    a.xcd = conv_xcd_enabled();
+    ConvEntryArgs e;
+    e.u = u;
+    e.ustats = ustats;
+    e.sp = (const unsigned short*)s_planes;
+    e.s_plane_stride = (rows_in + 1) * cin;
+    e.wp2 = (const unsigned short*)w2_planes;
+    e.w2_plane_stride = (long)cout * cin;
+    e.bias2 = bias2;
+    e.out2 = out_d;
+    e.stats2 = stats_d;
+    int nt;
+    conv_pick(hi, wi, ho, wo, cout, 3, 3, 2, 1, 1, &nt);
+    hipStream_t st = (hipStream_t)stream_;
+    const hipError_t err = nt == 3 ? launch_conv_entry<3>(a, e, mode, st) : launch_conv_entry<4>(a, e, mode, st);
+    if (err != hipSuccess) {
+        um_set_error("um_conv2d_entry_fwd: launch failed: %s", hipGetErrorString(err));
+        return (int)err;
+    }
+    return 0;
+}
+
 template <int CPP>
 __global__ __launch_bounds__(256) void pack7_kernel(const float* img, unsigned short* planes, long plane_stride, int B, int C,
                                                     int H, int W, int Hp, int Wp, int normalize, float m0, float m1, float m2,
diff --git a/unimatch_amd/csrc/nhwc_ops.hip b/unimatch_amd/csrc/nhwc_ops.hip
--- a/unimatch_amd/csrc/nhwc_ops.hip
+++ b/unimatch_amd/csrc/nhwc_ops.hip
@@ -126,7 +126,7 @@
 }
 
 template <typename T, int NS>
-__global__ __launch_bounds__(256) void nhwc_apply_kernel(const float* x, const float* stats, const float* shortcut,
+__global__ __launch_bounds__(256) void nhwc_apply_kernel(const float* x, const float* stats, const float* shortcut, const float* sc_stats,
                                                          const unsigned short* shortcut_planes, unsigned short* planes,
                                                          float* outf, long rows, int P, int C, int relu) {
     const int c8n = C >> 3;
@@ -142,7 +142,9 @@
         for (int pl = 0; pl < NS; ++pl) *reinterpret_cast<u32x4*>(planes + pl * plane_stride + row * C + c) = z;
         return;
     }
-    float v[8];
+    float v[8], mu[8], rs[8], s[8], smu[8], srs[8];
+#pragma unroll
+    for (int i = 0; i < 8; ++i) mu[i] = rs[i] = s[i] = smu[i] = srs[i] = 0.f;
     {
         const f32x4 a0 = __builtin_nontemporal_load(reinterpret_cast<const f32x4*>(x + row * C + c));
         const f32x4 a1 = __builtin_nontemporal_load(reinterpret_cast<const f32x4*>(x + row * C + c + 4));
@@ -152,54 +154,46 @@
             v[4 + i] = a1[i];
         }
     }
+    const int b = (int)(row / P);
     if (stats) {
-        const int b = (int)(row / P);
-        const float* mu = stats + ((long)b * 2) * C + c;
-        const float* rs = mu + C;
-#pragma unroll
-        for (int i = 0; i < 8; ++i) v[i] = (v[i] - mu[i]) * rs[i];
-    }
-    if (relu) {
-#pragma unroll
-        for (int i = 0; i < 8; ++i) v[i] = fmaxf(v[i], 0.f);
-    }
+        const float* m = stats + ((long)b * 2) * C + c;
+#pragma unroll
+        for (int i = 0; i < 8; ++i) {
+            mu[i] = m[i];
+            rs[i] = m[C + i];
+        }
+    }
+    u32x4 sh = {0u, 0u, 0u, 0u}, sl = sh;
     if (shortcut) {
         const f32x4 s0 = *reinterpret_cast<const f32x4*>(shortcut + row * C + c);
         const f32x4 s1 = *reinterpret_cast<const f32x4*>(shortcut + row * C + c + 4);
 #pragma unroll
         for (int i = 0; i < 4; ++i) {
-            v[i] = fmaxf(v[i] + s0[i], 0.f);
-            v[4 + i] = fmaxf(v[4 + i] + s1[i], 0.f);
+            s[i] = s0[i];
+            s[4 + i] = s1[i];
+        }
+        if (sc_stats) {
+            const float* m = sc_stats + ((long)b * 2) * C + c;
+#pragma unroll
+            for (int i = 0; i < 8; ++i) {
+                smu[i] = m[i];
+                srs[i] = m[C + i];
+            }
         }
     } else if (shortcut_planes) {
-        const u32x4 sh = *reinterpret_cast<const u32x4*>(shortcut_planes + row * C + c);
-        u32x4 sl = {0u, 0u, 0u, 0u};
+        sh = *reinterpret_cast<const u32x4*>(shortcut_planes + row * C + c);
         if (NS == 2) sl = *reinterpret_cast<const u32x4*>(shortcut_planes + plane_stride + row * C + c);
-#pragma unroll
-        for (int i = 0; i < 4; ++i) {
-            const f32x2 uh = T::unpack2(sh[i]);
-            f32x2 ul = {0.f, 0.f};
-            if (NS == 2) ul = T::unpack2(sl[i]);
-            v[2 * i] = fmaxf(v[2 * i] + (uh[0] + ul[0]), 0.f);
-            v[2 * i + 1] = fmaxf(v[2 * i + 1] + (uh[1] + ul[1]), 0.f);
-        }
-    }
+    }
+    u32x4 h, l;
+    um_norm_value8<T, NS>(v, stats != nullptr, mu, rs, relu != 0, shortcut ? 1 : shortcut_planes ? 2 : 0, s, sc_stats != nullptr, smu, srs,
+                          sh, sl, planes != nullptr, h, l);
     if (outf) {
         *reinterpret_cast<f32x4*>(outf + row * C + c) = f32x4{v[0], v[1], v[2], v[3]};
         *reinterpret_cast<f32x4*>(outf + row * C + c + 4) = f32x4{v[4], v[5], v[6], v[7]};
     }
     if (planes) {
-        const u32x4 h = {T::pack2(v[0], v[1]), T::pack2(v[2], v[3]), T::pack2(v[4], v[5]), T::pack2(v[6], v[7])};
         *reinterpret_cast<u32x4*>(planes + row * C + c) = h;
-        if (NS == 2) {
-            u32x4 l;
-#pragma unroll
-            for (int i = 0; i < 4; ++i) {
-                const f32x2 u = T::unpack2(h[i]);
-                l[i] = T::pack2(v[2 * i] - u[0], v[2 * i + 1] - u[1]);
-            }
-            *reinterpret_cast<u32x4*>(planes + plane_stride + row * C + c) = l;
-        }
+        if (NS == 2) *reinterpret_cast<u32x4*>(planes + plane_stride + row * C + c) = l;
     }
 }
 
@@ -304,29 +298,36 @@
 
 static bool nhwc_channels_ok(int c) { return c > 0 && c % 8 == 0 && c <= 256; }
 
-extern "C" int um_nhwc_instance_norm(const float* x, const float* shortcut, const void* shortcut_planes, void* planes_out, float* f32_out, int batch,
-                                     int pixels, int channels, float eps, int normalize, int relu, const float* conv_stats, int conv_stats_parts,
-                                     void* workspace, size_t workspace_bytes, int mode, void* stream_) {
+static int nhwc_instance_norm_impl(const char* who, const float* x, const float* shortcut, const void* shortcut_planes, void* planes_out,
+                                   float* f32_out, int batch, int pixels, int channels, float eps, int normalize, int relu,
+                                   const float* conv_stats, int conv_stats_parts, const float* sc_conv_stats, int sc_conv_stats_parts,
+                                   void* workspace, size_t workspace_bytes, int mode, void* stream_) {
     hipStream_t stream = (hipStream_t)stream_;
     if (!x || (!planes_out && !f32_out) || batch <= 0 || pixels <= 0 || !nhwc_channels_ok(channels) || (mode != 0 && mode != 1)) {
-        um_set_error("um_nhwc_instance_norm: bad argument (batch=%d pixels=%d channels=%d: channels must be a multiple of 8, <= 256)",
-                     batch, pixels, channels);
+        um_set_error("%s: bad argument (batch=%d pixels=%d channels=%d: channels must be a multiple of 8, <= 256)", who, batch, pixels,
+                     channels);
+        return -1;
+    }
+    if (sc_conv_stats && (!shortcut || !normalize || sc_conv_stats_parts <= 0)) {
+        um_set_error("%s: shortcut statistics go with an fp32 shortcut, normalize = 1 and sc_conv_stats_parts = um_conv_stats_parts() of "
+                     "the shortcut's convolution", who);
         return -1;
     }
     const long rows = (long)batch * pixels;
     const int nchunk = (pixels + NHWC_CHUNK_ROWS - 1) / NHWC_CHUNK_ROWS;
     float* partial = (float*)workspace;
-    float* stats = nullptr;
+    float *stats = nullptr, *sc_stats = nullptr;
     ScopedKernelTimer timer(UM_K_INSTANCE_NORM, stream);
     if (normalize) {
-        if (!workspace || workspace_bytes < um_nhwc_norm_workspace_bytes(batch, pixels, channels)) {
-            um_set_error("um_nhwc_instance_norm: workspace too small");
+        const size_t need = um_nhwc_norm_workspace_bytes(batch, pixels, channels) + (sc_conv_stats ? (size_t)batch * 2 * channels * sizeof(float) : 0);
+        if (!workspace || workspace_bytes < need) {
+            um_set_error("%s: workspace too small", who);
             return -3;
         }
         stats = partial + (long)batch * nchunk * 3 * channels;
         if (conv_stats) {
             if (conv_stats_parts <= 0) {
-                um_set_error("um_nhwc_instance_norm: conv_stats needs conv_stats_parts = um_conv_stats_parts() of the convolution");
+                um_set_error("%s: conv_stats needs conv_stats_parts = um_conv_stats_parts() of the convolution", who);
                 return -1;
             }
             hipLaunchKernelGGL(nhwc_stats_finalize_kernel, dim3(channels / 8, batch), dim3(256), 0, stream, conv_stats, stats, pixels, channels,
@@ -336,21 +337,51 @@
             hipLaunchKernelGGL(nhwc_stats_finalize_kernel, dim3(channels / 8, batch), dim3(256), 0, stream, partial, stats, pixels, channels,
                                nchunk, NHWC_CHUNK_ROWS, eps);
         }
+        if (sc_conv_stats) {
+            sc_stats = stats + (long)batch * 2 * channels;
+            hipLaunchKernelGGL(nhwc_stats_finalize_kernel, dim3(channels / 8, batch), dim3(256), 0, stream, sc_conv_stats, sc_stats, pixels,
+                               channels, sc_conv_stats_parts, 0, eps);
+        }
     }
     const long total = (rows + (planes_out ? 1 : 0)) * (channels / 8);
     const dim3 grid((unsigned)((total + 255) / 256));
     if (mode == 0)
-        hipLaunchKernelGGL((nhwc_apply_kernel<Fp16, 2>), grid, dim3(256), 0, stream, x, stats, shortcut,
+        hipLaunchKernelGGL((nhwc_apply_kernel<Fp16, 2>), grid, dim3(256), 0, stream, x, stats, shortcut, sc_stats,
                            (const unsigned short*)shortcut_planes, (unsigned short*)planes_out, f32_out, rows, pixels, channels, relu);
     else
-        hipLaunchKernelGGL((nhwc_apply_kernel<Bf16, 1>), grid, dim3(256), 0, stream, x, stats, shortcut,
+        hipLaunchKernelGGL((nhwc_apply_kernel<Bf16, 1>), grid, dim3(256), 0, stream, x, stats, shortcut, sc_stats,
                            (const unsigned short*)shortcut_planes, (unsigned short*)planes_out, f32_out, rows, pixels, channels, relu);
     const hipError_t e = hipGetLastError();
     if (e != hipSuccess) {
-        um_set_error("um_nhwc_instance_norm: launch failed: %s", hipGetErrorString(e));
+        um_set_error("%s: launch failed: %s", who, hipGetErrorString(e));
         return (int)e;
     }
     return 0;
+}
+
+extern "C" int um_nhwc_instance_norm(const float* x, const float* shortcut, const void* shortcut_planes, void* planes_out, float* f32_out, int batch,
+                                     int pixels, int channels, float eps, int normalize, int relu, const float* conv_stats, int conv_stats_parts,
+                                     void* workspace, size_t workspace_bytes, int mode, void* stream_) {
+    return nhwc_instance_norm_impl("um_nhwc_instance_norm", x, shortcut, shortcut_planes, planes_out, f32_out, batch, pixels, channels, eps,
+                                   normalize, relu, conv_stats, conv_stats_parts, nullptr, 0, workspace, workspace_bytes, mode, stream_);
+}
+
+extern "C" size_t um_nhwc_norm_sc_workspace_bytes(int batch, int pixels, int channels) {
+    if (batch <= 0 || pixels <= 0 || channels <= 0) return 0;
+    return um_nhwc_norm_workspace_bytes(batch, pixels, channels) + (size_t)batch * 2 * channels * sizeof(float);
+}
+
+extern "C" int um_nhwc_instance_norm_sc(const float* x, const float* shortcut, const void* shortcut_planes, void* planes_out, float* f32_out,
+                                        int batch, int pixels, int channels, float eps, int normalize, int relu, const float* conv_stats,
+                                        int conv_stats_parts, void* workspace, size_t workspace_bytes, int mode, void* stream_,
+                                        const float* sc_conv_stats, int sc_conv_stats_parts) {
+    if (!sc_conv_stats) {
+        um_set_error("um_nhwc_instance_norm_sc: no shortcut statistics (um_nhwc_instance_norm is the entry without them)");
+        return -1;
+    }
+    return nhwc_instance_norm_impl("um_nhwc_instance_norm_sc", x, shortcut, shortcut_planes, planes_out, f32_out, batch, pixels, channels,
+                                   eps, normalize, relu, conv_stats, conv_stats_parts, sc_conv_stats, sc_conv_stats_parts, workspace,
+                                   workspace_bytes, mode, stream_);
 }
 
 extern "C" int um_nhwc_stats_finalize(const float* conv_stats, int conv_stats_parts, float* stats_out, int batch, int pixels, int channels,
diff --git a/unimatch_amd/csrc/planes.h b/unimatch_amd/csrc/planes.h
--- a/unimatch_amd/csrc/planes.h
+++ b/unimatch_amd/csrc/planes.h
@@ -36,6 +36,48 @@
     um_range_note<T>(range_flag, mx, UM_RANGE_PLANES);
 }
 
+template <class T, int NS>
+__device__ __forceinline__ void um_norm_value8(float (&v)[8], bool norm, const float (&mu)[8], const float (&rs)[8], bool relu, int sc,
+                                               float (&s)[8], bool sc_norm, const float (&smu)[8], const float (&srs)[8], u32x4 sh,
+                                               u32x4 sl, bool split, u32x4& h, u32x4& l) {
+#pragma clang fp contract(off)
+    if (norm) {
+#pragma unroll
+        for (int i = 0; i < 8; ++i) v[i] = (v[i] - mu[i]) * rs[i];
+    }
+    if (relu) {
+#pragma unroll
+        for (int i = 0; i < 8; ++i) v[i] = fmaxf(v[i], 0.f);
+    }
+    if (sc == 1) {
+        if (sc_norm) {
+#pragma unroll
+            for (int i = 0; i < 8; ++i) s[i] = (s[i] - smu[i]) * srs[i];
+        }
+#pragma unroll
+        for (int i = 0; i < 8; ++i) v[i] = fmaxf(v[i] + s[i], 0.f);
+    } else if (sc == 2) {
+#pragma unroll
+        for (int i = 0; i < 4; ++i) {
+            const f32x2 uh = T::unpack2(sh[i]);
+            f32x2 ul = {0.f, 0.f};
+            if (NS == 2) ul = T::unpack2(sl[i]);
+            v[2 * i] = fmaxf(v[2 * i] + (uh[0] + ul[0]), 0.f);
+            v[2 * i + 1] = fmaxf(v[2 * i + 1] + (uh[1] + ul[1]), 0.f);
+        }
+    }
+    if (split) {
+        h = u32x4{T::pack2(v[0], v[1]), T::pack2(v[2], v[3]), T::pack2(v[4], v[5]), T::pack2(v[6], v[7])};
+        if (NS == 2) {
+#pragma unroll
+            for (int i = 0; i < 4; ++i) {
+                const f32x2 u = T::unpack2(h[i]);
+                l[i] = T::pack2(v[2 * i] - u[0], v[2 * i + 1] - u[1]);
+            }
+        }
+    }
+}
+
 static inline hipError_t launch_split_elems(const float* src, unsigned short* dst, long n_elems, float scale,
                                             int mode, hipStream_t stream);
 
diff --git a/unimatch_amd/encoder.py b/unimatch_amd/encoder.py
--- a/unimatch_amd/encoder.py
+++ b/unimatch_amd/encoder.py
@@ -1,3 +1,5 @@
+
+import collections
 
 import torch
 import torch.nn as nn
@@ -6,6 +8,9 @@
 
 def _conv3(cin, cout, stride=1):
     return nn.Conv2d(cin, cout, 3, stride=stride, padding=1, bias=False)
+
+
+_Deferred = collections.namedtuple('_Deferred', 'u stats shortcut_planes')
 
 
 class _Residual(nn.Module):
@@ -29,24 +34,44 @@
         return F.relu((x if self.downsample is None else self.downsample(x)) + y)
 
 
-    def forward_nhwc(self, act, ops, want_f32):
+    def entry_fusable(self, ops, h, w, cin):
+        return (getattr(ops, 'fused_entry', False) and self.downsample is not None and self.conv1.stride[0] == 2 and
+                ops.conv2d_entry_supported(h, w, cin, self.conv1.weight, self.downsample[0].weight))
+
+    def forward_nhwc(self, act, ops, want_f32, defer=False):
         planes, f32, b, h, w, c = act
         stride = self.conv1.stride[0]
         cout = self.conv1.out_channels
-        t, ho, wo = ops.conv2d_nhwc((planes, b, h, w, c), self.conv1.weight, None, stride, (1, 1), stats=True)
+        fused = getattr(ops, 'fused_entry', False)
+        d = dstats = None
+        if isinstance(planes, _Deferred):
+            proj = self.downsample[0]
+            t, d, ho, wo, tstats, dstats = ops.conv2d_entry(planes.u, planes.stats, planes.shortcut_planes, (b, h, w, c), self.conv1.weight,
+                                                            proj.weight, proj.bias)
+        else:
+            t, ho, wo = ops.conv2d_nhwc((planes, b, h, w, c), self.conv1.weight, None, stride, (1, 1), stats=True)
+            tstats = ops.last_conv_stats
         if getattr(ops, 'norm_on_load', False) and ops.conv2d_norm_supported(ho, wo, cout, self.conv2.weight):
-            u, _, _ = ops.conv2d_nhwc_normed(t, ops.last_conv_stats, (b, ho, wo, cout), self.conv2.weight, stats=True)
+            u, _, _ = ops.conv2d_nhwc_normed(t, tstats, (b, ho, wo, cout), self.conv2.weight, stats=True)
         else:
-            tp, _ = ops.nhwc_norm(t, b, ho * wo, relu=True, want_planes=True, conv_stats=ops.last_conv_stats)
+            tp, _ = ops.nhwc_norm(t, b, ho * wo, relu=True, want_planes=True, conv_stats=tstats)
             u, _, _ = ops.conv2d_nhwc((tp, b, ho, wo, cout), self.conv2.weight, None, 1, (1, 1), stats=True)
         ustats = ops.last_conv_stats
         sc = scp = None
         if self.downsample is None:
             sc, scp = (f32, None) if f32 is not None else (None, planes)
+            if defer and scp is not None:
+                return _Deferred(u, ustats, scp), None, b, ho, wo, cout
         else:
-            proj = self.downsample[0]
-            d, _, _ = ops.conv2d_nhwc((planes, b, h, w, c), proj.weight, proj.bias, stride, (0, 0), stats=True)
-            _, sc = ops.nhwc_norm(d, b, ho * wo, relu=False, want_planes=False, want_f32=True, conv_stats=ops.last_conv_stats)
+            if d is None:
+                proj = self.downsample[0]
+                d, _, _ = ops.conv2d_nhwc((planes, b, h, w, c), proj.weight, proj.bias, stride, (0, 0), stats=True)
+                dstats = ops.last_conv_stats
+            if fused:
+                op, of = ops.nhwc_norm(u, b, ho * wo, relu=True, shortcut=d, shortcut_stats=dstats, want_planes=True, want_f32=want_f32,
+                                       conv_stats=ustats)
+                return op, of, b, ho, wo, cout
+            _, sc = ops.nhwc_norm(d, b, ho * wo, relu=False, want_planes=False, want_f32=True, conv_stats=dstats)
         op, of = ops.nhwc_norm(u, b, ho * wo, relu=True, shortcut=sc, shortcut_planes=scp, want_planes=True, want_f32=want_f32,
                                conv_stats=ustats)
         return op, of, b, ho, wo, cout
@@ -114,6 +139,12 @@
 
     shortcut_f32 = False
 
+    @staticmethod
+    def _out_geometry(blk, act):
+        _, _, _, h, w, _ = act
+        s = blk.conv1.stride[0]
+        return (h - 1) // s + 1, (w - 1) // s + 1, blk.conv1.out_channels
+
     def _forward_nhwc(self, x, ops, input_norm=None):
         b = x.shape[0]
         y, h, w = ops.stem_conv(x.contiguous(), self.conv1.weight, input_norm, stats=True)
@@ -124,7 +155,8 @@
         blocks = [blk for layer in (self.layer1, self.layer2, self.layer3) for blk in layer]
         for i, blk in enumerate(blocks):
             nxt = blocks[i + 1] if i + 1 < len(blocks) else None
-            act = blk.forward_nhwc(act, ops, want_f32=keep_f32 and nxt is not None and nxt.downsample is None)
+            defer = nxt is not None and blk.downsample is None and nxt.entry_fusable(ops, *self._out_geometry(blk, act))
+            act = blk.forward_nhwc(act, ops, want_f32=keep_f32 and nxt is not None and nxt.downsample is None, defer=defer)
         planes, _, b, h, w, c = act
         out, _, _ = ops.conv2d_nhwc((planes, b, h, w, c), self.conv2.weight, self.conv2.bias, 1, (0, 0))
         if self.num_branch == 1:
diff --git a/unimatch_amd/ops.py b/unimatch_amd/ops.py
--- a/unimatch_amd/ops.py
+++ b/unimatch_amd/ops.py
@@ -128,6 +128,7 @@
     fused_kv = True
     fused_conv = True
     norm_on_load = True
+    fused_entry = True
     CONV_MODE = 0
     WSHIFT = 10
 
@@ -645,6 +646,41 @@
             _stream()), meta)
         _abi.check(code, 'um_conv2d_norm_fwd')
         return out, h, w
+
+    def conv2d_entry_supported(self, h, w, cin, weight, proj_weight, stride=2, padding=(1, 1)):
+        cout, wcin, kh, kw = weight.shape
+        ph, pw = (padding, padding) if isinstance(padding, int) else padding
+        return (wcin == cin and tuple(proj_weight.shape) == (cout, cin, 1, 1) and
+                bool(self.lib.um_conv2d_entry_supported(h, w, cin, cout, kh, kw, stride, ph, pw, self.CONV_MODE)))
+
+    def conv2d_entry(self, u, conv_stats, shortcut_planes, geom, weight, proj_weight, proj_bias, eps=1e-5):
+        b, h, w, cin = geom
+        self._check_rows('u', u, cin)
+        if u.shape[0] != b * h * w:
+            raise ValueError('conv2d_entry: u must have b * h * w rows')
+        if shortcut_planes.numel() != self.lib.um_planes_bytes(b * h * w + 1, cin, self.CONV_MODE):
+            raise ValueError('conv2d_entry: shortcut_planes must be operand planes of [b * h * w + 1, cin]')
+        wp, cout, wcin, kh, kw = self.conv_weight_planes(weight)
+        wp2, cout2, wcin2, kh2, kw2 = self.conv_weight_planes(proj_weight)
+        if wcin != cin or (cout2, wcin2, kh2, kw2) != (cout, cin, 1, 1):
+            raise ValueError('conv2d_entry: the weights do not fit the activation / each other')
+        nstats = torch.empty((b, 2, cin), dtype=torch.float32, device=u.device)
+        _abi.check(self._launch('instance_norm', lambda: self.lib.um_nhwc_stats_finalize(
+            _ptr(conv_stats[0]), conv_stats[1], _ptr(nstats), b, h * w, cin, float(eps), _stream())), 'um_nhwc_stats_finalize')
+        ho, wo = (h - 1) // 2 + 1, (w - 1) // 2 + 1
+        t = torch.empty((b * ho * wo, cout), dtype=torch.float32, device=u.device)
+        d = torch.empty_like(t)
+        parts = self.lib.um_conv_stats_parts(h, w, cout, 3, 3, 2, 1, 1)
+        nst = self.lib.um_conv_stats_bytes(b, parts, cout) // 4
+        st_t = torch.empty(nst, dtype=torch.float32, device=u.device)
+        st_d = torch.empty(nst, dtype=torch.float32, device=u.device)
+        meta = {'flops': 2.0 * b * ho * wo * cout * 10 * cin}
+        code = self._launch('conv', lambda: self.lib.um_conv2d_entry_fwd(
+            _ptr(u), _ptr(nstats), _ptr(shortcut_planes), _ptr(wp), _ptr(wp2), _ptr(proj_bias) if proj_bias is not None else None, _ptr(t), _ptr(d), _ptr(st_t), _ptr(st_d),
+            b, h, w, cin, cout, 3, 3, 2, 1, 1, self.WSHIFT, self.CONV_MODE, _stream()), meta)
+        _abi.check(code, 'um_conv2d_entry_fwd')
+        self.last_conv_stats = (st_t, parts)
+        return t, d, ho, wo, (st_t, parts), (st_d, parts)
 
     def nhwc_planes_from(self, pieces, pad_to=32):
         rows = pieces[0].shape[0]
@@ -837,7 +873,7 @@
         return out, ho, wo
 
     def nhwc_norm(self, x, b, pixels, normalize=True, relu=True, shortcut=None, want_planes=True, want_f32=False, eps=1e-5,
-                  conv_stats=None, shortcut_planes=None):
+                  conv_stats=None, shortcut_planes=None, shortcut_stats=None):
         self._check_rows('x', x, x.shape[1])
         c = x.shape[1]
         if x.shape[0] != b * pixels:
@@ -850,6 +886,17 @@
         planes = (torch.empty(self.lib.um_planes_bytes(rows + 1, c, self.CONV_MODE), dtype=torch.uint8, device=x.device)
                   if want_planes else None)
         f32 = torch.empty_like(x) if want_f32 else None
+        if shortcut_stats is not None:
+            if shortcut is None or not normalize:
+                raise ValueError('nhwc_norm: shortcut_stats go with an fp32 shortcut and normalize=True')
+            ws = self._ws(self.lib.um_nhwc_norm_sc_workspace_bytes(b, pixels, c), x.device)
+            code = self._launch('instance_norm', lambda: self.lib.um_nhwc_instance_norm_sc(
+                _ptr(x), _ptr(shortcut), None, _ptr(planes) if planes is not None else None,
+                _ptr(f32) if f32 is not None else None, b, pixels, c, float(eps), 1, int(bool(relu)),
+                _ptr(conv_stats[0]) if conv_stats is not None else None, conv_stats[1] if conv_stats is not None else 0,
+                _ptr(ws), ws.numel(), self.CONV_MODE, _stream(), _ptr(shortcut_stats[0]), shortcut_stats[1]))
+            _abi.check(code, 'um_nhwc_instance_norm_sc')
+            return planes, f32
         ws = self._ws(self.lib.um_nhwc_norm_workspace_bytes(b, pixels, c), x.device) if normalize else None
         code = self._launch('instance_norm', lambda: self.lib.um_nhwc_instance_norm(
             _ptr(x), _ptr(shortcut) if shortcut is not None else None,
```
